# JGI-Bioinformatics/Kmernator

Hardware: AMD Instinct MI355X
Metric: total k-mers/sec at k=31, 150 bp reads (spectrum build, inputs resident in HBM) (higher is better)
Workload: dtype u64

## Files before the change

kmernator_amd/csrc/kmr_api.hip:

```cpp
#include <hip/hip_runtime.h>
#include <dlfcn.h>
#include <unistd.h>
#include <rccl/rccl.h>

#include <algorithm>
#include <atomic>
#include <cmath>
#include <cstdio>
#include <cstdlib>
#include <cstring>
#include <cctype>
#include <memory>
#include <mutex>
#include <string>
#include <type_traits>
#include <vector>

#include "kmr_host.hpp"
#include "kmr_runs.hpp"
#include "kmr_image_layout.hpp"
#include "kmr_kernels.hpp"
#include "kmr_partition.hpp"
#include "kmr_superkmer.hpp"
#include "kmr_buckets.hpp"
// ... 38 lines not shown

namespace {

template <int W, class F> auto with_win(uint32_t win, F &&f) {
	if (W > 1 && win == 32) return f(int_c<(W > 1 ? 32 : 16)>());
	return win == 16 ? f(int_c<16>()) : (win == 8 ? f(int_c<8>()) : f(int_c<4>()));
}

size_t slot_bytes(kmr_handle *h) { return with_w(h, [](auto W) { return sizeof(Slot<W()>); }); }

ReadsView reads_view(const void *bases, const void *quals, const void *offsets, uint64_t n_reads, const void *discarded = nullptr, uint64_t stream_base = 0, uint64_t first_read_idx = 0) {
	ReadsView rv{};
	rv.bases = (const uint8_t *)bases; rv.quals = (const uint8_t *)quals; rv.offsets = (const uint64_t *)offsets; rv.discarded = (const uint8_t *)discarded;
	rv.n_reads = n_reads; rv.stream_base = stream_base; rv.first_read_idx = first_read_idx;
	return rv;
}
ReadsView reads_slice(const ReadsView &all, uint64_t r, uint64_t m) {
	ReadsView rv = all;
	rv.offsets = all.offsets + r; rv.n_reads = m; rv.discarded = all.discarded ? all.discarded + r : nullptr; rv.first_read_idx = all.first_read_idx + r;
	return rv;
}
FinalizeParams finalize_params(kmr_handle *h, uint32_t min_depth) {
	FinalizeParams f{};
	f.kb = h->hkb; f.ext_min_q = h->cfg.ext_min_quality; f.min_depth = min_depth; f.has_singletons = h->cfg.separate_singletons ? 1 : 0; f.nb_weak = h->nb_weak; f.nb_sing = h->nb_sing;
	return f;
}

DevParams dev_params(kmr_handle *h) {
	DevParams p;
	p.k = h->k; p.kb = h->hkb; p.min_weight = h->cfg.min_weight; p.fastq_start = h->cfg.fastq_start_char; p.ext_min_q = h->cfg.ext_min_quality;
	p.qzero = h->cfg.fastq_start_char + std::max<uint32_t>(1u, h->cfg.min_quality_score);
	p.subsample = h->cfg.kmer_subsample; p.rank = h->cfg.rank; p.world = h->cfg.world_size; p.num_parts = h->cfg.num_parts; p.part_idx = h->cfg.part_idx;
	p.count_sender_bad = 0u;
	p.P = h->dP.get<double>(); p.stats = h->dstats.get<DevStats>(); p.err = h->derr.get<uint32_t>();
	p.sub_wstart = p.sub_wkeys = p.sub_sstart = p.sub_skeys = nullptr; p.sub_wvals = nullptr; p.sub_sweight = nullptr; p.sub_wnb = p.sub_snb = 0; p.sub_vw = 0;
	if (h->subtract) {
		const kmr_handle *o = h->subtract;
		if (o->weak.present && o->weak.n) { p.sub_wstart = o->weak.start.get<uint64_t>(); p.sub_wkeys = o->weak.keys.get<uint64_t>(); p.sub_wvals = o->weak.vals.get<uint32_t>(); p.sub_wnb = o->weak.nb; p.sub_vw = o->ext ? 15 : 3; }
		if (o->sing.present && o->sing.n) { p.sub_sstart = o->sing.start.get<uint64_t>(); p.sub_skeys = o->sing.keys.get<uint64_t>(); p.sub_sweight = o->sing.sweight.get<uint8_t>(); p.sub_snb = o->sing.nb; }
	}
	return p;
}


template <int W> Table<W> table_of(kmr_handle *h) { Table<W> t; t.slots = h->slots.get<Slot<W>>(); t.ext = h->extslots.get<ExtSlot>(); t.log2cap = h->log2cap; return t; }

template <int W> int clear_table(kmr_handle *h, void *slots, ExtSlot *ext, uint32_t log2cap) {
	hipLaunchKernelGGL(table_clear_kernel<W>, dim3(grid_for(1ull << log2cap)), dim3(256), 0, h->stream, (Slot<W> *)slots, ext, 1ull << log2cap);
	HIPCHK(h, hipGetLastError());
	return 0;
}
int clear_table_any(kmr_handle *h, void *slots, ExtSlot *ext, uint32_t log2cap) { return with_w(h, [&](auto W) { return clear_table<W()>(h, slots, ext, log2cap); }); }

int alloc_table(kmr_handle *h, uint32_t log2cap, DevBuf &slots, DevBuf &ext) {
	DevBuf s, x;
	HIPCHK(h, s.alloc(slot_bytes(h) << log2cap));
	if (h->ext) HIPCHK(h, x.alloc(sizeof(ExtSlot) << log2cap));
	const int rc = clear_table_any(h, s.get(), x.get<ExtSlot>(), log2cap);
	if (rc) return rc;
	slots = std::move(s); ext = std::move(x);
	return 0;
}

int sync_state(kmr_handle *h, bool with_pool_head = false) {
	h->l1_head_seen = 0;
	if (with_pool_head && h->l1.head) HIPCHK(h, hipMemcpyAsync(&h->l1_head_seen, h->l1.head.get<unsigned int>(), 4, hipMemcpyDeviceToHost, h->stream));
	HIPCHK(h, hipStreamSynchronize(h->stream));
	for (int which = 0; which < KMR_TIME_GROUPS; which++) {
		for (auto &pr : h->pending_events[which]) {
			float ms = 0; hipEventElapsedTime(&ms, pr.first, pr.second);
			h->ms[which] += ms; h->launches[which]++;
			hipEventDestroy(pr.first); hipEventDestroy(pr.second);
		}
		h->pending_events[which].clear();
	}
	uint32_t e = 0; DevStats s;
	HIPCHK(h, hipMemcpy(&e, h->derr.get<uint32_t>(), sizeof(e), hipMemcpyDeviceToHost));
	HIPCHK(h, hipMemcpy(&s, h->dstats.get<DevStats>(), sizeof(s), hipMemcpyDeviceToHost));
#ifdef KMR_DEBUG_HOOKS
	if (h->superkmer_mode) { if (dbg()) fprintf(stderr, "sk_extract windows: %llu general, %llu fast\n", s.claimed, s.inserted); s.claimed = 0; s.inserted = 0; }
#endif
	h->stats.raw_kmers = s.raw + s.inserted + s.sender_bad; h->stats.raw_good_kmers = s.good + s.inserted; h->stats.discarded = s.raw - s.good + s.sender_bad;
	h->occupied = s.claimed; h->pending_kmers = 0; h->subtracted = s.subtracted;
	if (e & ERR_READ_TOO_LONG) return fail(h, KMR_ERR_UNSUPPORTED, "a read is longer than the per-wavefront LDS tile (" + std::to_string(TILE_SPAN) + " bases)");
	if (e & ERR_TABLE_FULL) return fail(h, KMR_ERR_CAPACITY, "device k-mer table is full; raise kmr_config.max_table_entries / estimated_raw_kmers");
	if (e & ERR_SEGMENT_OVERFLOW) return fail(h, KMR_ERR_CAPACITY, "an owner segment overflowed seg_capacity");
	if (e & ERR_POOL_FULL) return fail(h, KMR_ERR_CAPACITY, "record pool overflow (internal sizing error)");
	if (e & ERR_ENTRIES_FULL) return fail(h, KMR_ERR_CAPACITY, "entry buffer overflow (internal sizing error)");
	return 0;
}

template <int W, bool EXT> int grow_table_t(kmr_handle *h, uint32_t newlog) {
	DevBuf ns, ne;
	int rc = alloc_table(h, newlog, ns, ne);
	if (rc) return rc;
	Table<W> src = table_of<W>(h), dst; dst.slots = ns.get<Slot<W>>(); dst.ext = ne.get<ExtSlot>(); dst.log2cap = newlog;
	hipLaunchKernelGGL((rehash_kernel<W, EXT>), dim3(grid_for(1ull << h->log2cap)), dim3(256), 0, h->stream, src, dst, h->hkb, h->derr.get<uint32_t>());
	HIPCHK(h, hipGetLastError());
	HIPCHK(h, hipStreamSynchronize(h->stream));
	h->slots = std::move(ns); h->extslots = std::move(ne); h->log2cap = newlog;
	return 0;
}
int grow_table(kmr_handle *h, uint32_t newlog) { return with_w_ext(h, [&](auto W, auto EXT) { return grow_table_t<W(), EXT()>(h, newlog); }); }

int ensure_capacity(kmr_handle *h, uint64_t incoming) {
	const uint64_t cap = 1ull << h->log2cap;
	if ((double)(h->occupied + h->pending_kmers + incoming) <= 0.85 * (double)cap) { h->pending_kmers += incoming; return 0; }
	int rc = sync_state(h);
	if (rc) return rc;
	if ((double)(h->occupied + incoming) > 0.85 * (double)cap) {
		uint32_t nl = h->log2cap;
		while ((double)(h->occupied + incoming) > 0.6 * (double)(1ull << nl)) nl++;
		rc = grow_table(h, nl);
		if (rc) return rc;
	}
	h->pending_kmers = incoming;
	return 0;
}

const size_t EXTRACT_SMEM = (size_t)WAVES_PER_BLOCK * 2 * TILE_BUF;

int prepare_units(kmr_handle *h, ReadsView &rv, uint32_t span = (uint32_t)TILE_SPAN, const unsigned int *longest = nullptr) {
	rv.u_start = rv.u_end = rv.u_read = nullptr; rv.n_units = 0;
	const uint64_t n = rv.n_reads;
	if (n == 0) return 0;
	int rc = 0;
	unsigned int mx = 0;
	if (longest) mx = *longest;
	else {
		rc = h->umax.reserve(h, "umax", 4); if (rc) return rc;
		HIPCHK(h, hipMemsetAsync(h->umax.get<unsigned int>(), 0, 4, h->stream));
		hipLaunchKernelGGL(unit_max_kernel, dim3(grid_for(n)), dim3(256), 0, h->stream, rv.offsets, n, h->umax.get<unsigned int>());
		HIPCHK(h, hipGetLastError());
		HIPCHK(h, hipMemcpyAsync(&mx, h->umax.get<unsigned int>(), 4, hipMemcpyDeviceToHost, h->stream));
		HIPCHK(h, hipStreamSynchronize(h->stream));
	}
	if (mx <= span) return 0;
	h->unit_batches++;
	rc = h->ucnt.reserve(h, "ucnt", 4 * (n + 1)); if (rc) return rc;
	hipLaunchKernelGGL(unit_count_kernel, dim3(grid_for(n)), dim3(256), 0, h->stream, rv.offsets, n, h->k, span, h->ucnt.get<uint32_t>());
	HIPCHK(h, hipGetLastError());
	rc = h->ufirst.reserve(h, "ufirst", 8 * (n + 1)); if (rc) return rc;
	rc = exclusive_scan_queue(h, h->ucnt.get<uint32_t>(), n, h->ufirst.get<uint64_t>()); if (rc) return rc;
	uint64_t U = 0;
	HIPCHK(h, hipMemcpyAsync(&U, h->ufirst.get<uint64_t>() + n, 8, hipMemcpyDeviceToHost, h->stream));
	HIPCHK(h, hipStreamSynchronize(h->stream));
	if (h->u_read.cap() < 8 * U) {
		h->u_start.reset(); h->u_end.reset(); h->u_read.reset();
		HIPCHK(h, h->u_start.alloc(8 * U)); HIPCHK(h, h->u_end.alloc(8 * U)); HIPCHK(h, h->u_read.alloc(8 * U));
	}
	hipLaunchKernelGGL(unit_fill_kernel, dim3(grid_for(n)), dim3(256), 0, h->stream, rv.offsets, n, h->k, span, h->ufirst.get<uint64_t>(), h->u_start.get<uint64_t>(), h->u_end.get<uint64_t>(), h->u_read.get<uint64_t>());
	HIPCHK(h, hipGetLastError());
	rv.u_start = h->u_start.get<uint64_t>(); rv.u_end = h->u_end.get<uint64_t>(); rv.u_read = h->u_read.get<uint64_t>(); rv.n_units = U;
	return 0;
}

template <int W, bool EXT, class Op> int launch_extract(kmr_handle *h, const ReadsView &rv, const DevParams &dp, const Op &op, uint64_t max_blocks = 0) {
	const bool sub = Op::NEEDS_WEIGHT && (dp.sub_wnb | dp.sub_snb) != 0;
	auto kern = sub ? extract_kernel<W, EXT, Op, true> : extract_kernel<W, EXT, Op, false>;
	HIPCHK(h, hipFuncSetAttribute((const void *)kern, hipFuncAttributeMaxDynamicSharedMemorySize, (int)EXTRACT_SMEM));
	if (dbg()) { int nb = 0; hipOccupancyMaxActiveBlocksPerMultiprocessor(&nb, (const void *)kern, WAVES_PER_BLOCK * 64, EXTRACT_SMEM); fprintf(stderr, "extract: %d blocks of %d waves per CU (dynamic LDS %zu)\n", nb, WAVES_PER_BLOCK, EXTRACT_SMEM);
		for (size_t tr : {(size_t)79872, (size_t)65536, (size_t)52000, (size_t)38000}) { hipOccupancyMaxActiveBlocksPerMultiprocessor(&nb, (const void *)kern, WAVES_PER_BLOCK * 64, tr); fprintf(stderr, "   with %zu bytes: %d blocks\n", tr, nb); } }
	const uint64_t tiles = ((rv.u_start ? rv.n_units : rv.n_reads) + 63) / 64;
	uint64_t blocks = (tiles + WAVES_PER_BLOCK - 1) / WAVES_PER_BLOCK;
	if (blocks == 0) return 0;
	if (max_blocks && blocks > max_blocks) blocks = max_blocks;
// ... 1047 lines not shown
		uint32_t sh = 0; while ((1u << sh) < h->cfg.world_size) sh++;
		if (bits >= 6 + sh) { h->sk_fine_shift = sh; bits -= sh; }
	}
	h->sk_bits = bits;
	if (h->cfg.world_size <= 1 && !h->sk_exchange && h->tune.target_list == 2048 && !h->tune.pow2_lists) {
		const uint64_t aim = h->tune.list_aim ? h->tune.list_aim : (W == 1 ? (h->ext ? 800 : (lean ? 1450 : 1700)) : per_list * 19 / 20);
		const uint64_t nlists = (est / aim + 63) & ~63ull;
		if (nlists > 64 && (nlists < (1ull << bits) || h->tune.list_aim) && nlists < (1ull << 31)) h->sk_bits = (uint32_t)nlists;
	}
	const uint64_t nl0 = sk_list_count(h->sk_bits);
	HIPCHK(h, h->sk_state.alloc(8 * nl0));
	hipLaunchKernelGGL(sk_state_init_kernel, dim3(grid_for(nl0)), dim3(256), 0, h->stream, h->sk_state.get<unsigned long long>(), nl0);
	HIPCHK(h, hipGetLastError());
	return 0;
}
void sk_presize_pool(kmr_handle *h, uint64_t call_bases, uint64_t total_bases, uint64_t avg, bool lean) {
	if (h->l1.base || h->cfg.world_size > 1 || h->sk_exchange || !(h->cfg.estimated_raw_kmers || call_bases > total_bases)) return;
	const double job_bases = h->cfg.estimated_raw_kmers ? (double)h->cfg.estimated_raw_kmers * (double)avg / (double)(avg > h->k ? avg - h->k + 1 : 1) : (double)call_bases;
	const double rest = job_bases - (double)total_bases;
	size_t fr = 0, tot = 0;
	if (rest > 0 && hipMemGetInfo(&fr, &tot) == hipSuccess) {
		const uint64_t want = (uint64_t)(rest * (h->ext ? 2.0 : 1.0) * (lean ? 0.3 : 0.65) / SK_CHUNK_G);
		h->l1.presize = std::min<uint64_t>(want, (uint64_t)(fr / 4) / ((size_t)CH * rec_bytes(h)));
	}
}
uint64_t sk_launch_chunks(kmr_handle *h, uint64_t bases) { return (h->ext ? 2 : 1) * bases / SK_CHUNK_G + ((h->l1.base && !h->sk_exchange) ? 0 : sk_list_count(h->sk_bits)) + (uint64_t)num_cus(h) * SK_EXTRACT_WAVES_PER_CU * 130 + 64; }
template <int W> int sk_launch_extraction(kmr_handle *h, const ReadsView &rv, const SkParams &sp, const DevParams &dp, bool filt, bool lean, float wK, const SkPacked *packed, uint64_t r) {
	if (packed) {
		SkPacked pkd = *packed; pkd.off += r; if (pkd.mk_off) pkd.mk_off += r;
		return with_win<W>(h->sk_win, [&](auto WIN) { return launch_sk_extract_lean<W, WIN(), true>(h, rv, sp, dp, wK, pkd); });
	}
	return with_win<W>(h->sk_win, [&](auto WIN) {
		if (h->ext) return filt ? launch_sk_extract<W, WIN(), true, true>(h, rv, sp, dp) : launch_sk_extract<W, WIN(), false, true>(h, rv, sp, dp);
		if (filt) return launch_sk_extract<W, WIN(), true>(h, rv, sp, dp);
		return lean ? launch_sk_extract_lean<W, WIN()>(h, rv, sp, dp, wK) : launch_sk_extract<W, WIN(), false>(h, rv, sp, dp);
	});
}
template <int W> int sk_track_call(kmr_handle *h, const ReadsView &rvAll, const DevParams &dp) {
	const uint64_t n = rvAll.n_reads;
	std::vector<SkTrackRec> recs(n);
	HIPCHK(h, hipMemcpyAsync(recs.data(), h->trk.get<SkTrackRec>(), n * sizeof(SkTrackRec), hipMemcpyDeviceToHost, h->stream));
	HIPCHK(h, hipStreamSynchronize(h->stream));
	std::vector<SkBoundary> bd; std::vector<uint64_t> good_before;
	const bool walkable = (dp.sub_wnb | dp.sub_snb) == 0;
	for (uint64_t r = 0; r < n; r++) {
		while ((uint64_t)h->trk_next <= h->trk_raw + recs[r].raw) {
			SkBoundary b; b.read = r; b.t = (uint32_t)((uint64_t)h->trk_next - h->trk_raw); b.good = 0; b.ordinal = 0;
			if (!walkable) { b.t = recs[r].raw; b.good = recs[r].good; b.ordinal = recs[r].end_ordinal; }
			bd.push_back(b); good_before.push_back(h->trk_good);
			h->trk_snap_raw.push_back(walkable ? (uint64_t)h->trk_next : h->trk_raw + recs[r].raw);
			h->trk_next = (long)((double)h->trk_next * 1.05);
			if (!walkable) break;
		}
		if (!walkable) while ((uint64_t)h->trk_next <= h->trk_raw + recs[r].raw) h->trk_next = (long)((double)h->trk_next * 1.05);
		h->trk_raw += recs[r].raw; h->trk_good += recs[r].good;
	}
	if (h->trk_bounds.size() + bd.size() > SK_TRACK_MAX) return fail(h, KMR_ERR_UNSUPPORTED, "size tracker: more than 512 elements");
	if (!bd.empty() && walkable) {
		DevBuf dbdb; HIPCHK(h, dbdb.alloc(bd.size() * sizeof(SkBoundary)));
		SkBoundary *dbd = dbdb.get<SkBoundary>();
		auto chk = [&](hipError_t e) { return e == hipSuccess ? 0 : fail(h, KMR_ERR_HIP, std::string("size tracker boundaries: ") + hipGetErrorString(e)); };
		int rc = chk(hipMemcpyAsync(dbd, bd.data(), bd.size() * sizeof(SkBoundary), hipMemcpyHostToDevice, h->stream)); if (rc) return rc;
		ReadsView rv = rvAll; rv.u_start = rv.u_end = rv.u_read = nullptr; rv.n_units = 0;
		hipLaunchKernelGGL(sk_track_boundary_kernel<W>, dim3((unsigned)((bd.size() + 63) / 64)), dim3(64), 0, h->stream, rv, dp, dbd, (uint32_t)bd.size());
		rc = chk(hipGetLastError()); if (rc) return rc;
		rc = chk(hipMemcpyAsync(bd.data(), dbd, bd.size() * sizeof(SkBoundary), hipMemcpyDeviceToHost, h->stream)); if (rc) return rc;
		rc = chk(hipStreamSynchronize(h->stream)); if (rc) return rc;
	}
	for (size_t i = 0; i < bd.size(); i++) { h->trk_bounds.push_back(bd[i].ordinal); h->trk_snap_good.push_back(good_before[i] + bd[i].good); }
	return 0;
}
template <int W> int add_reads_superkmer_t(kmr_handle *h, const ReadsView &rvAll, uint64_t total_bases, const FeedHints &hints) {
	const uint64_t n = rvAll.n_reads;
	const DevParams dp = dev_params(h);
	const bool filt = sk_build_filters(h, dp), tracking = h->cfg.size_tracker && n;
	bool lean = false; float wK = 1.0f; int rc = 0;
	const uint64_t avg = n ? std::max<uint64_t>(1, total_bases / n) : 1;
	const uint64_t sub_bases = h->tune.sub_batch_bases ? h->tune.sub_batch_bases : (1ull << 31);
	const uint64_t chunk = std::max<uint64_t>(64, (sub_bases / avg) & ~63ull);
	unsigned int longest = 0; bool have_longest = false;
	if (!filt && !h->ext && !sp_debug_extract(h)) { rc = sk_uniform_weight(h, rvAll, hints, lean, wK, n <= chunk ? &longest : nullptr, &have_longest); if (rc) return rc; }
	if (hints.packed && (!lean || h->cfg.size_tracker)) return fail(h, KMR_ERR_STATE, "internal: a packed batch handed to an extraction that wants text");
	if (n) sk_note_call_weight(h, lean, wK);
	if (!h->sk_state) { rc = sk_size_lists<W>(h, std::max<uint64_t>(total_bases, hints.call_bases), lean); if (rc) return rc; }
	if (tracking) { h->trk_n = 0; rc = h->trk.reserve(h, "trk", n * sizeof(SkTrackRec)); if (rc) return rc; HIPCHK(h, hipMemsetAsync(h->trk.get<SkTrackRec>(), 0, n * sizeof(SkTrackRec), h->stream)); }
	for (uint64_t r = 0; r < n; r += chunk) {
		const uint64_t m = std::min(chunk, n - r);
		ReadsView rv = reads_slice(rvAll, r, m);
		rc = prepare_units(h, rv, hints.packed ? SK_PACKED_SPAN : (uint32_t)TILE_SPAN, have_longest ? &longest : nullptr); if (rc) return rc;
		if (r == 0) sk_presize_pool(h, hints.call_bases, total_bases, avg, lean);
		rc = pool_reserve(h, h->l1, sk_launch_chunks(h, m * avg + avg), true); if (rc) return rc;
		TimeSpan tb(h, KMR_TIME_BUILD), te(h, KMR_TIME_EXTRACT);
		SkParams sp = sk_params(h);
		if (h->cfg.size_tracker) sp.track = h->trk.get<SkTrackRec>() + r;
		rc = sk_launch_extraction<W>(h, rv, sp, dp, filt, lean, wK, hints.packed, r);
		te.end(); tb.end();
		if (rc) return rc;
	}
	return tracking ? sk_track_call<W>(h, rvAll, dp) : 0;
}
int add_reads_superkmer(kmr_handle *h, const ReadsView &rv, uint64_t total_bases, const FeedHints &hints) { return with_w(h, [&](auto W) { return add_reads_superkmer_t<W()>(h, rv, total_bases, hints); }); }
static const uint64_t SAT_BATCH_BYTES = 1ull << 30;
static const uint64_t SAT_BATCH_KEYS = (1ull << 23) - 1;
static const uint64_t SAT_PAIR_BYTES = 24;
template <int W> int saturated_fix_t(kmr_handle *h, const uint64_t *ls, const uint64_t *lc, uint64_t nl, unsigned long long n_clamped, unsigned long long n_sightings, uint32_t has_singletons) {
	DevMap &wm = h->weak;
	h->last_saturated_keys = 0; h->last_saturated_batches = 0;
	if (!n_clamped || !wm.n) return 0;
	uint32_t list_bits = 0; while ((1ull << list_bits) < nl) list_bits++;
	if ((1ull << list_bits) != nl) list_bits = (uint32_t)nl;
	auto no_mem = [&](const char *what, size_t bytes) { return fail(h, KMR_ERR_OOM, std::string("saturated-key pass (weights of k-mers seen 256 times or more): no device memory for ") + what + " (" + std::to_string(bytes) + " bytes)"); };
	auto dalloc = [](DevBuf &b, size_t bytes) { return b.alloc(std::max<size_t>(bytes, 256)); };
	DevBuf bfound, bentry, blist;
	if (dalloc(bfound, 8) != hipSuccess) return no_mem("a counter", 8);
	unsigned long long *dfound = bfound.get<unsigned long long>(); uint64_t *d_entry = nullptr; uint32_t *d_list = nullptr;
	uint64_t cap = std::min<uint64_t>(wm.n, 4 * n_clamped + 1024);
	unsigned long long found = 0;
	for (;;) {
		if (dalloc(bentry, 8 * cap) != hipSuccess || dalloc(blist, 4 * cap) != hipSuccess) return no_mem("the key list", 12 * cap);
		d_entry = bentry.get<uint64_t>(); d_list = blist.get<uint32_t>();
		HIPCHK(h, hipMemsetAsync(dfound, 0, 8, h->stream));
		hipLaunchKernelGGL(sat_find_kernel<W>, dim3(grid_for(wm.n)), dim3(256), 0, h->stream, (const uint64_t *)wm.keys.get<uint64_t>(), (const uint32_t *)wm.vals.get<uint32_t>(), wm.n, h->sk_m, h->sk_off, h->sk_win, list_bits, dfound, cap, d_entry, d_list, h->ext ? 15u : 3u);
		HIPCHK(h, hipGetLastError());
		HIPCHK(h, hipMemcpyAsync(&found, dfound, 8, hipMemcpyDeviceToHost, h->stream)); HIPCHK(h, hipStreamSynchronize(h->stream));
		if (found <= cap) break;
		cap = found;
	}
	if (!found) return 0;
	std::vector<uint64_t> entry(found); std::vector<uint32_t> lst(found);
	HIPCHK(h, hipMemcpy(entry.data(), d_entry, 8 * found, hipMemcpyDeviceToHost)); HIPCHK(h, hipMemcpy(lst.data(), d_list, 4 * found, hipMemcpyDeviceToHost));
	std::vector<uint64_t> order(found);
	for (uint64_t i = 0; i < found; i++) order[i] = i;
	std::sort(order.begin(), order.end(), [&](uint64_t a, uint64_t b) { return lst[a] != lst[b] ? lst[a] < lst[b] : entry[a] < entry[b]; });
	std::vector<uint64_t> sentry(found); std::vector<uint32_t> dl; std::vector<uint64_t> le0, le1;
	for (uint64_t i = 0; i < found; i++) {
		sentry[i] = entry[order[i]];
		const uint32_t l = lst[order[i]];
		if (dl.empty() || dl.back() != l) { dl.push_back(l); le0.push_back(i); le1.push_back(i + 1); } else le1.back() = i + 1;
	}
	std::vector<uint64_t>().swap(entry); std::vector<uint32_t>().swap(lst); std::vector<uint64_t>().swap(order);
	HIPCHK(h, hipMemcpy(d_entry, sentry.data(), 8 * found, hipMemcpyHostToDevice));
	HIPCHK(h, hipMemcpy(d_list, dl.data(), 4 * dl.size(), hipMemcpyHostToDevice));
	std::vector<uint64_t> c0(dl.size()), c1(dl.size());
	{
		DevBuf bc0, bc1;
		if (dalloc(bc0, 8 * dl.size()) != hipSuccess || dalloc(bc1, 8 * dl.size()) != hipSuccess) return no_mem("the chunk ranges", 16 * dl.size());
		hipLaunchKernelGGL(sat_gather_kernel, dim3(grid_for(dl.size())), dim3(256), 0, h->stream, ls, (const uint32_t *)d_list, (uint64_t)dl.size(), bc0.get<uint64_t>(), bc1.get<uint64_t>());
		HIPCHK(h, hipGetLastError());
		HIPCHK(h, hipMemcpy(c0.data(), bc0.get<uint64_t>(), 8 * dl.size(), hipMemcpyDeviceToHost)); HIPCHK(h, hipMemcpy(c1.data(), bc1.get<uint64_t>(), 8 * dl.size(), hipMemcpyDeviceToHost));
	}
	blist = DevBuf();
	struct Seg { uint32_t li; uint64_t e0, e1, est; };
	std::vector<Seg> segs;
	uint64_t all_chunks = 0;
	for (size_t i = 0; i < dl.size(); i++) all_chunks += c1[i] - c0[i];
	const double per_chunk = all_chunks ? (double)n_sightings / (double)all_chunks : 0.0;
	for (size_t i = 0; i < dl.size(); i++)
		for (uint64_t a = le0[i]; a < le1[i]; a += SAT_BATCH_KEYS) {
			const uint64_t b = std::min<uint64_t>(le1[i], a + SAT_BATCH_KEYS);
			const double share = (double)(b - a) / (double)(le1[i] - le0[i]);
			segs.push_back(Seg{(uint32_t)i, a, b, (uint64_t)(per_chunk * (double)(c1[i] - c0[i]) * share) + 1});
		}
	const uint64_t budget = h->tune.saturated_batch_bytes ? h->tune.saturated_batch_bytes : SAT_BATCH_BYTES;
	uint64_t batches = 0;
	for (size_t s0 = 0; s0 < segs.size(); ) {
		size_t s1 = s0 + 1; uint64_t est = segs[s0].est;
		while (s1 < segs.size() && segs[s1].e1 - segs[s0].e0 <= SAT_BATCH_KEYS && (est + segs[s1].est) * SAT_PAIR_BYTES <= budget) est += segs[s1++].est;
		const uint64_t k0 = segs[s0].e0, nk = segs[s1 - 1].e1 - k0;
		std::vector<uint64_t> items;
		for (size_t g = s0; g < s1; g++)
			for (uint64_t a = c0[segs[g].li]; a < c1[segs[g].li]; a += 256) { items.push_back(a); items.push_back(std::min(c1[segs[g].li], a + 256)); items.push_back(segs[g].e0 - k0); items.push_back(segs[g].e1 - k0); }
		const size_t ni = items.size() / 4;
		std::vector<uint64_t> soa(4 * ni);
		for (size_t i = 0; i < ni; i++) for (int q = 0; q < 4; q++) soa[q * ni + i] = items[4 * i + q];
		uint64_t pcap = est + est / 4 + 1024;
		for (int attempt = 0; ni; attempt++) {
			DevBuf bitems, bk_in, bk_out, bv_in, bv_out, btmp;
			if (dalloc(bitems, 32 * ni) != hipSuccess) return no_mem("its work items", 32 * ni);
			uint64_t *d_items = bitems.get<uint64_t>();
			HIPCHK(h, hipMemcpy(d_items, soa.data(), 32 * ni, hipMemcpyHostToDevice));
			if (dalloc(bk_in, 8 * pcap) != hipSuccess || dalloc(bk_out, 8 * pcap) != hipSuccess || dalloc(bv_in, 4 * pcap) != hipSuccess || dalloc(bv_out, 4 * pcap) != hipSuccess)
				return no_mem("the sightings of one batch", SAT_PAIR_BYTES * pcap);
			unsigned long long *pk_in = bk_in.get<unsigned long long>(), *pk_out = bk_out.get<unsigned long long>(); uint32_t *pv_in = bv_in.get<uint32_t>(), *pv_out = bv_out.get<uint32_t>();
			HIPCHK(h, hipMemsetAsync(dfound, 0, 8, h->stream));
			int rc = zero_work_counter(h); if (rc) return rc;
			hipLaunchKernelGGL(sat_collect_kernel<W>, dim3((unsigned)std::min<uint64_t>(ni, (uint64_t)num_cus(h) * 4)), dim3(256), 0, h->stream, pool_view(h, h->l1), lc, h->k, (const uint64_t *)wm.keys.get<uint64_t>(), (const uint64_t *)(d_entry + k0),
			                   (const uint64_t *)d_items, (const uint64_t *)(d_items + ni), (const uint64_t *)(d_items + 2 * ni), (const uint64_t *)(d_items + 3 * ni), (uint64_t)ni, dfound, pcap, pk_in, pv_in, h->work_counter.get<unsigned int>());
			HIPCHK(h, hipGetLastError());
			unsigned long long n_pairs = 0;
			HIPCHK(h, hipMemcpyAsync(&n_pairs, dfound, 8, hipMemcpyDeviceToHost, h->stream)); HIPCHK(h, hipStreamSynchronize(h->stream));
			if (n_pairs > pcap) {
				if (attempt) return fail(h, KMR_ERR_CAPACITY, "saturated-key pass: sightings of a batch changed between two passes (internal error)");
				pcap = n_pairs;
				continue;
			}
			size_t tmp_bytes = 0;
			if (kmr::sort_pairs_u64_u32(nullptr, &tmp_bytes, pk_in, pk_out, pv_in, pv_out, n_pairs, h->stream) != 0) return fail(h, KMR_ERR_HIP, "saturated-key pass: radix sort (size query)");
			if (dalloc(btmp, tmp_bytes) != hipSuccess) return no_mem("the sort's temporary storage", tmp_bytes);
			if (kmr::sort_pairs_u64_u32(btmp.get(), &tmp_bytes, pk_in, pk_out, pv_in, pv_out, n_pairs, h->stream) != 0) return fail(h, KMR_ERR_HIP, "saturated-key pass: radix sort");
			hipLaunchKernelGGL(sat_reduce_kernel, dim3((unsigned)std::min<uint64_t>(nk, 4096)), dim3(256), 0, h->stream, (const unsigned long long *)pk_out, (const uint32_t *)pv_out, (uint64_t)n_pairs, (const uint64_t *)(d_entry + k0), (uint64_t)nk, has_singletons, wm.vals.get<uint32_t>(), h->ext ? 15u : 3u);
			HIPCHK(h, hipGetLastError());
			HIPCHK(h, hipStreamSynchronize(h->stream));
			break;
		}
		batches++;
		s0 = s1;
	}
	h->last_saturated_keys = found; h->last_saturated_batches = batches;
	return 0;
}


template <int W> int sk_count_uniform(kmr_handle *h, bool tracking, bool &uni, uint32_t &uni_wbits) {
	uni = false; uni_wbits = 0;
	if (tracking || h->ext || h->sk_uni_mixed || h->tune.no_uniform_count) return 0;
	if (W > 1 && (h->k & 31u) == 0) return 0;
	uint32_t w = h->sk_uni_w; bool mixed = false;
	if (h->peer_uni_mixed) mixed = true;
	else if (h->peer_uni_w != SK_UNI_NONE) { if (w == SK_UNI_NONE) w = h->peer_uni_w; else if (w != h->peer_uni_w) mixed = true; }
	if (h->d_uni) {
		uint32_t dv[2] = {SK_UNI_NONE, 0u};
		HIPCHK(h, hipMemcpy(dv, h->d_uni.get<uint32_t>(), 8, hipMemcpyDeviceToHost));
		if (dv[1]) mixed = true;
		else if (dv[0] != SK_UNI_NONE) { if (w == SK_UNI_NONE) w = dv[0]; else if (w != dv[0]) mixed = true; }
	}
	if (!mixed && w != SK_UNI_NONE) { uni = true; uni_wbits = w; }
	return 0;
}
template <int W> SkLong<W> sk_own_lists(kmr_handle *h, bool refined) {
	SkLong<W> lg{};
	lg.list_first = 0; lg.list_stride = 1;
	if (h->sk_exchange && h->cfg.world_size > 1 && !refined) { lg.list_first = h->cfg.rank; lg.list_stride = h->cfg.world_size; }
	return lg;
}
template <int W> struct SkCountLaunch {
	void (*kern)(const uint4 *, const uint64_t *, const uint64_t *, uint64_t, uint32_t, SkCountHot, unsigned int *, uint32_t, const SkCountArgs<W> *);
	size_t smem;
	int blocks;
};
static const int SK_COUNT_BLOCKS_DEFAULT = 5;
template <int W> int sk_count_blocks(kmr_handle *h, bool ext, bool tracking, bool uni, bool item) {
	if (W != 1 || ext || tracking || !uni || item) return 4;
	return h->tune.count_blocks ? h->tune.count_blocks : SK_COUNT_BLOCKS_DEFAULT;
}
template <int W, int LOG2S, bool TRACK, bool EXT, bool UNI, bool ITEM, int BLOCKS = 0> SkCountLaunch<W> sk_count_form() { return {sk_count_kernel<W, LOG2S, TRACK, EXT, UNI, ITEM, BLOCKS>, sk_count_smem_bytes<W, LOG2S, TRACK, EXT, UNI>(), BLOCKS ? BLOCKS : 4}; }
template <int W, bool ITEM> SkCountLaunch<W> sk_count_forms(bool ext, bool tracking, bool uni, int blocks) {
	if constexpr (!ITEM) { if (tracking && !ext) return sk_count_form<W, COUNT_LOG2S, true, false, false, false>(); }
	if constexpr (W == 1 && !ITEM) { if (blocks == 5) return sk_count_form<1, COUNT_LOG2S, false, false, true, false, 5>(); }
	return ext ? sk_count_form<W, COUNT_LOG2S_EXT, false, true, false, ITEM>() :
	    (uni ? sk_count_form<W, COUNT_LOG2S, false, false, true, ITEM>() : sk_count_form<W, COUNT_LOG2S, false, false, false, ITEM>());
}
template <int W> int sk_count_select(kmr_handle *h, bool ext, bool tracking, bool uni, bool item, const CountOut &out, const SkLong<W> &lg, SkCountLaunch<W> &k) {
	if (item && tracking) return fail(h, KMR_ERR_STATE, "internal: the size tracker's count pass has no long-list items");
	if (item != (lg.item_c0 != nullptr) || (item && (!lg.item_c1 || !lg.merge.slots || !lg.merge_used))) return fail(h, KMR_ERR_STATE, "internal: count pass and its work items disagree");
	if (ext ? (!out.wkeys || !out.wvals || !out.weakCount) : !out.wentries) return fail(h, KMR_ERR_STATE, "internal: count pass and its entry buffers disagree");
	const int blocks = sk_count_blocks<W>(h, ext, tracking, uni, item);
	k = item ? sk_count_forms<W, true>(ext, tracking, uni, blocks) : sk_count_forms<W, false>(ext, tracking, uni, blocks);
	if (k.blocks != blocks) return fail(h, KMR_ERR_STATE, "internal: count pass and its blocks per CU disagree");
	if (!item) h->last_count_blocks = k.blocks;
	const auto kern = k.kern; const size_t smem = k.smem;
	HIPCHK(h, hipFuncSetAttribute((const void *)kern, hipFuncAttributeMaxDynamicSharedMemorySize, (int)smem));
	return 0;
}
template <int W> int sk_count_launch(kmr_handle *h, const SkCountLaunch<W> &k, int grid, const uint64_t *ls, const uint64_t *lc, uint64_t nl, const CountOut &out, const FinalizeParams &f, const SkTrackView &tv, const SkLong<W> &lg) {
	SkCountArgs<W> a{out, f, tv, lg};
	SkCountArgs<W> *d = nullptr;
	int rc = arena_get(h, &d, 1); if (rc) return rc;
	hipLaunchKernelGGL(sk_count_args_kernel<W>, dim3(1), dim3(64), 0, h->stream, a, d);
	hipLaunchKernelGGL(k.kern, dim3(grid), dim3(SKC_THREADS), k.smem, h->stream, (const uint4 *)pool_view(h, h->l1).base, ls, lc, nl, h->k, sk_count_hot<W>(a), h->work_counter.get<unsigned int>(), sk_dbg_flags("KMR_SK_COUNT_DBG"), (const SkCountArgs<W> *)d);
	return 0;
}

template <int W> struct SkFinalize : CountPass {
	bool tracking = false, refined = false, uni = false;
	uint64_t nl = 1; uint64_t *ls = nullptr, *lc = nullptr; uint32_t nch = 0;
	SkTrackView tv{};
	SkLong<W> lgMain{}, lgItems{}; uint64_t n_items = 0;
	uint64_t early_slots = 0; FinalizeCounters early_c{};
};

int sk_refine_lists(kmr_handle *h, uint64_t &nl) {
	const uint32_t fine_bits = h->sk_bits + h->sk_fine_shift;
	const uint64_t nlf = 1ull << fine_bits;
	unsigned int head = 0;
	HIPCHK(h, hipStreamSynchronize(h->stream));
	HIPCHK(h, hipMemcpy(&head, h->l1.head.get<unsigned int>(), 4, hipMemcpyDeviceToHost));
	if (head > h->l1.cap) head = h->l1.cap;
	int rc = h->sk_fine_state.reserve(h, "sk_fine_state", 8 * nlf); if (rc) return rc;
	hipLaunchKernelGGL(sk_state_init_kernel, dim3(grid_for(nlf)), dim3(256), 0, h->stream, h->sk_fine_state.get<unsigned long long>(), nlf);
	const int rgrid = (int)std::min<uint64_t>(((uint64_t)head + SK_REFINE_WAVES - 1) / SK_REFINE_WAVES + 1, (uint64_t)num_cus(h) * 8);
	rc = pool_reserve(h, h->l1, (uint64_t)head * 2 + nlf / h->cfg.world_size + (uint64_t)rgrid * SK_REFINE_WAVES * 130 + 64, true); if (rc) return rc;
	if (head) hipLaunchKernelGGL(sk_refine_kernel, dim3(rgrid), dim3(SK_REFINE_WAVES * 64), 0, h->stream, pool_view(h, h->l1), head, fine_bits, h->sk_fine_state.get<unsigned long long>());
	hipLaunchKernelGGL(sk_close_kernel, dim3(grid_for(nlf)), dim3(256), 0, h->stream, h->sk_fine_state.get<unsigned long long>(), nlf, h->l1.chunk_count.get<uint32_t>(), h->l1.cap);
	HIPCHK(h, hipGetLastError());
	nl = nlf;
	return 0;
}
int sk_track_view(kmr_handle *h, SkTrackView &tv) {
	const std::vector<unsigned long long> &bounds = h->trk_bounds;
	if (bounds.size() > SK_TRACK_MAX) return fail(h, KMR_ERR_UNSUPPORTED, "size tracker: more than 512 elements");
	unsigned long long *db = nullptr; unsigned int *dd = nullptr;
	int rc = arena_get(h, &db, bounds.size() + 1); if (rc) return rc;
	rc = arena_get(h, &dd, 2 * (bounds.size() + 1)); if (rc) return rc;
	if (!bounds.empty()) HIPCHK(h, hipMemcpyAsync(db, bounds.data(), 8 * bounds.size(), hipMemcpyHostToDevice, h->stream));
	tv.bounds = db; tv.n = (uint32_t)bounds.size(); tv.d_unique = dd; tv.d_single = dd + bounds.size() + 1;
	return 0;
}
int sk_track_elements(kmr_handle *h, const SkTrackView &tv, uint32_t has_singletons) {
	std::vector<unsigned int> dd(2 * (tv.n + 1), 0);
	HIPCHK(h, hipMemcpy(dd.data(), tv.d_unique, 8 * (tv.n + 1), hipMemcpyDeviceToHost));
	h->trk_elems.clear();
	uint64_t uniq = 0; int64_t single = 0;
	const uint64_t sub = h->cfg.kmer_subsample > 1 ? h->cfg.kmer_subsample : 1;
	for (uint32_t i = 0; i < tv.n; i++) {
		uniq += dd[i]; single += (int32_t)dd[tv.n + 1 + i];
		h->trk_elems.push_back(h->trk_snap_raw[i] * sub); h->trk_elems.push_back(h->trk_snap_good[i] * sub);
		h->trk_elems.push_back(uniq * sub); h->trk_elems.push_back(has_singletons ? (uint64_t)single * sub : 0);
	}
	return 0;
}
template <int W> int sk_early_takeover(kmr_handle *h, SkFinalize<W> &p, uint32_t min_depth, bool &device_error) {
	device_error = false;
	FinalizeCounters &early_c = p.early_c;
	h->last_early_hi = 0; h->last_early_entries = 0; h->last_early_overflowed = false;
	if (!h->early.active) return 0;
	uint32_t eerr = 0;
	HIPCHK(h, hipMemcpy(&eerr, h->early.err.get<uint32_t>(), 4, hipMemcpyDeviceToHost));
	unsigned long long ecur = 0;
	HIPCHK(h, hipMemcpy(&ecur, h->early.cursor.get<unsigned long long>(), 8, hipMemcpyDeviceToHost)); HIPCHK(h, hipMemcpy(&early_c, h->early.fc.get(), sizeof(early_c), hipMemcpyDeviceToHost));
	if (eerr & ~(uint32_t)ERR_ENTRIES_FULL) {
		uint32_t e = 0; HIPCHK(h, hipMemcpy(&e, h->derr.get<uint32_t>(), 4, hipMemcpyDeviceToHost)); e |= eerr & ~(uint32_t)ERR_ENTRIES_FULL;
		HIPCHK(h, hipMemcpy(h->derr.get<uint32_t>(), &e, 4, hipMemcpyHostToDevice)); h->early.active = false;
		device_error = true;
		return 0;
	}
	const bool overflowed = (eerr & ERR_ENTRIES_FULL) || ecur > packed_entries(h, h->early.ue);
	const bool ok = !overflowed && h->early.min_depth == min_depth && !p.tracking && !p.ext && !p.keepSing && !p.refined;
	h->last_early_overflowed = overflowed;
	if (ok) {
		p.early_slots = ecur;
		h->last_early_hi = h->early.hi; h->last_early_entries = early_c.weak_kept;
		const uint64_t stride0 = p.lgMain.list_stride, first0 = p.lgMain.list_first;
		uint64_t first = h->early.hi;
		if (stride0 > 1) first += (first0 + stride0 - first % stride0) % stride0;
		p.lgMain.list_first = first;
	} else { h->early.active = false; memset(&early_c, 0, sizeof(early_c)); }
	return 0;
}
template <int W> int sk_long_items(kmr_handle *h, SkFinalize<W> &p) {
	p.lgItems = p.lgMain; p.n_items = 0;
	const uint64_t LONG_CHUNKS = p.ext ? std::min<uint64_t>(h->tune.long_list_chunks ? h->tune.long_list_chunks : SK_EXT_LONG_CHUNKS, SK_EXT_LONG_CHUNKS) : (h->tune.long_list_chunks ? h->tune.long_list_chunks : 1024), PIECE = std::max<uint64_t>(1, LONG_CHUNKS / 2);
	if (p.tracking || p.nch <= LONG_CHUNKS) return 0;
	const uint64_t cap = (uint64_t)p.nch / PIECE + 2 * 1024 + 16;
	uint64_t *ic0 = nullptr, *ic1 = nullptr; unsigned long long *dn = nullptr;
	int rc = arena_get(h, &ic0, cap); if (rc) return rc; rc = arena_get(h, &ic1, cap); if (rc) return rc; rc = arena_get(h, &dn, 1); if (rc) return rc;
	HIPCHK(h, hipMemsetAsync(dn, 0, 8, h->stream));
	hipLaunchKernelGGL(sk_long_items_kernel, dim3(grid_for(p.nl)), dim3(256), 0, h->stream, p.ls, p.nl, LONG_CHUNKS, PIECE, ic0, ic1, cap, dn);
	HIPCHK(h, hipGetLastError());
	unsigned long long hn = 0;
	HIPCHK(h, hipMemcpyAsync(&hn, dn, 8, hipMemcpyDeviceToHost, h->stream)); HIPCHK(h, hipStreamSynchronize(h->stream));
	if (hn > cap) return fail(h, KMR_ERR_CAPACITY, "long-list work items (internal sizing error)");
	p.n_items = hn;
	if (p.n_items) {
		p.lgMain.long_threshold = LONG_CHUNKS;
		p.lgItems.item_c0 = ic0; p.lgItems.item_c1 = ic1; p.lgItems.n_items = p.n_items; p.lgItems.merge_used = dn;
	}
	return 0;
}
CountOut count_out(kmr_handle *h, bool packed, unsigned long long *cursors, uint32_t *wc, uint32_t *sc, FinalizeCounters *fc) {
	CountOut out{};
	if (packed) { out.wentries = h->ue.get<uint64_t>(); out.wcap = packed_entries(h, h->ue); }
	else { out.wkeys = h->uw_keys.get<uint64_t>(); out.wvals = h->uw_vals.get<uint32_t>(); out.wcap = key_entries(h, h->uw_keys); out.spkt = h->us_pkt.get<uint32_t>(); out.weakCount = wc; }
	out.wcursor = cursors; out.scursor = cursors + 1;
	out.skeys = h->us_keys.get<uint64_t>(); out.sweight = h->us_b8.get<uint8_t>(); out.scap = key_entries(h, h->us_keys);
	out.singCount = sc; out.fc = fc; out.err = h->derr.get<uint32_t>();
	return out;
}
template <int W> int sk_count_pass(kmr_handle *h, SkFinalize<W> &p) {
	const uint64_t nl = p.nl, n_items = p.n_items; const SkTrackView &tv = p.tv;
	uint32_t merge_log2 = 16;
	DevBuf mslots, mext;
	return count_attempts(h, p, [&]() -> int { mslots.reset(); mext.reset(); return 0; }, [&](const CountOut &out, bool repeated, uint32_t &repeat_on) -> int {
		if (repeated) merge_log2 += 3;
		int rc = 0;
		SkCountLaunch<W> k;
		rc = sk_count_select<W>(h, p.ext, p.tracking, p.uni, false, out, p.lgMain, k); if (rc) return rc;
		const int grid = (int)std::min<uint64_t>((uint64_t)num_cus(h) * k.blocks, (nl / p.lgMain.list_stride + SK_LBATCH) / SK_LBATCH);
		if (p.tracking) HIPCHK(h, hipMemsetAsync(tv.d_unique, 0, 8 * (tv.n + 1), h->stream));
		if (dbg()) { int nb = 0; hipOccupancyMaxActiveBlocksPerMultiprocessor(&nb, (const void *)k.kern, SKC_THREADS, k.smem); fprintf(stderr, "sk_count<W=%d>: %d blocks per CU (LDS %zu), %llu lists, %u chunks\n", W, nb, k.smem, (unsigned long long)nl, p.nch); }
		rc = sk_count_launch<W>(h, k, grid, p.ls, p.lc, nl, out, p.f, tv, p.lgMain); if (rc) return rc;
		HIPCHK(h, hipGetLastError());
		if (!n_items) return 0;
		SkLong<W> &lgItems = p.lgItems;
		if (mslots.alloc(sizeof(Slot<W>) << merge_log2) != hipSuccess) return fail(h, KMR_ERR_OOM, "merge table of the long lists");
		if (p.ext && mext.alloc(sizeof(ExtSlot) << merge_log2) != hipSuccess) return fail(h, KMR_ERR_OOM, "merge table of the long lists");
		hipLaunchKernelGGL(table_clear_kernel<W>, dim3(grid_for(1ull << merge_log2)), dim3(256), 0, h->stream, mslots.get<Slot<W>>(), mext.get<ExtSlot>(), 1ull << merge_log2);
		lgItems.merge.slots = mslots.get<Slot<W>>(); lgItems.merge.ext = mext.get<ExtSlot>(); lgItems.merge.log2cap = merge_log2;
		HIPCHK(h, hipMemsetAsync(lgItems.merge_used, 0, 8, h->stream));
		rc = zero_work_counter(h); if (rc) return rc;
		rc = sk_count_select<W>(h, p.ext, p.tracking, p.uni, true, out, lgItems, k); if (rc) return rc;
		const int grid2 = (int)std::min<uint64_t>((uint64_t)num_cus(h) * k.blocks, n_items);
		rc = sk_count_launch<W>(h, k, grid2, p.ls, p.lc, nl, out, p.f, tv, lgItems); if (rc) return rc;
		hipLaunchKernelGGL(sk_merge_emit_kernel<W>, dim3(grid_for(1ull << merge_log2)), dim3(256), 0, h->stream, lgItems.merge, out, p.f);
		if (hipGetLastError() != hipSuccess) return fail(h, KMR_ERR_HIP, "long-list launches");
		if (merge_log2 < 30) repeat_on = ERR_TABLE_FULL;
		return 0;
	});
}
template <int W> int sk_append_early(kmr_handle *h, SkFinalize<W> &p) {
	FinalizeCounters &c = p.c; const FinalizeCounters &early_c = p.early_c; unsigned long long *cur = p.cur; const uint64_t early_slots = p.early_slots;
	const size_t eb = 8ull * (W + 1);
	if (cur[0] + early_slots > packed_entries(h, h->ue)) {
		DevBuf bigger;
		HIPCHK(h, bigger.alloc(eb * (cur[0] + early_slots + 4096)));
		HIPCHK(h, hipMemcpyAsync(bigger.get(), h->ue.get(), eb * cur[0], hipMemcpyDeviceToDevice, h->stream)); HIPCHK(h, hipStreamSynchronize(h->stream));
		h->ue = std::move(bigger);
	}
	HIPCHK(h, hipMemcpyAsync((uint8_t *)h->ue.get<uint64_t>() + eb * cur[0], h->early.ue.get<uint64_t>(), eb * early_slots, hipMemcpyDeviceToDevice, h->stream));
	cur[0] += early_slots;
	c.unique += early_c.unique; c.singletons += early_c.singletons; c.weak_kept += early_c.weak_kept; c.sing_kept += early_c.sing_kept;
	c.saturated += early_c.saturated; c.sat_sightings += early_c.sat_sightings;
	h->stats.unique_kmers = c.unique; h->stats.singleton_kmers = p.f.has_singletons ? c.singletons : 0;
	return 0;
}

template <int W> int finalize_superkmer_t(kmr_handle *h, uint32_t min_depth) {
	int rc = sync_state(h, true);
	if (rc) return rc;
	TimeSpan whole(h, KMR_TIME_FINALIZE);
	const uint64_t G = h->stats.raw_good_kmers;
	SkFinalize<W> p;
	p.f = finalize_params(h, min_depth);
	p.keepSing = p.f.has_singletons && min_depth <= 1;
	p.ext = h->ext; p.packed = !p.ext;
	p.tracking = h->cfg.size_tracker != 0;
	if (!h->l1.head) { rc = pool_reserve(h, h->l1, 0, false); if (rc) return rc; }
	rc = arena_reset(h); if (rc) return rc;
	p.nl = h->sk_state ? sk_list_count(h->sk_bits) : 1;
	if (h->sk_state) {
		hipLaunchKernelGGL(sk_close_kernel, dim3(grid_for(p.nl)), dim3(256), 0, h->stream, h->sk_state.get<unsigned long long>(), p.nl, h->l1.chunk_count.get<uint32_t>(), h->l1.cap);
		HIPCHK(h, hipGetLastError());
	}
	p.refined = h->sk_state && h->sk_fine_shift > 0;
	if (p.refined) { rc = sk_refine_lists(h, p.nl); if (rc) return rc; }
	rc = build_csr(h, h->l1, p.nl, 0, &p.ls, &p.lc, &p.nch, p.refined ? nullptr : &h->l1_head_seen); if (rc) return rc;
	rc = sk_count_uniform<W>(h, p.tracking, p.uni, p.f.uni_wbits); if (rc) return rc;
	h->last_count_uniform = p.uni;
	rc = count_entry_buffers(h, p, G, sk_entry_slack(h, sk_count_blocks<W>(h, p.ext, p.tracking, p.uni, false)), G / (p.f.has_singletons ? 8 : 3), G / 3, h->sk_exchange && h->cfg.world_size > 1); if (rc) return rc;
	if (p.tracking) { rc = sk_track_view(h, p.tv); if (rc) return rc; }
	p.lgMain = sk_own_lists<W>(h, p.refined);
	bool device_error = false;
	rc = sk_early_takeover<W>(h, p, min_depth, device_error); if (rc) return rc;
	if (device_error) { whole.end(); return sync_state(h); }
	rc = sk_long_items<W>(h, p); if (rc) return rc;
	uint32_t *overflow = nullptr;
	auto count_and_bucket = [&](bool fixed_bins) -> int {
		int rc2 = sk_count_pass<W>(h, p); if (rc2) return rc2;
		h->stats.unique_kmers = p.c.unique; h->stats.singleton_kmers = p.f.has_singletons ? p.c.singletons : 0;
		if (p.tracking && !h->last_bb_fallback) { rc2 = sk_track_elements(h, p.tv, p.f.has_singletons); if (rc2) return rc2; }
		if (p.early_slots) { rc2 = sk_append_early<W>(h, p); if (rc2) return rc2; }
		h->early.active = false;
		TimeSpan t(h, KMR_TIME_BUCKETS);
		return finish_maps_from_entries(h, p.wc, p.sc, p.cur[0], p.cur[1], p.c.weak_kept, p.c.sing_kept, p.keepSing, overflow, p.packed, fixed_bins);
	};
	h->last_bb_fallback = false;
	rc = count_and_bucket(h->tune.bb_fixed_bins); if (rc) return rc;
	if (overflow) {
		uint32_t ovf = 0;
		HIPCHK(h, hipMemcpyAsync(&ovf, overflow, 4, hipMemcpyDeviceToHost, h->stream)); HIPCHK(h, hipStreamSynchronize(h->stream));
		if (ovf) {
			if (dbg()) fprintf(stderr, "bucket build: a bin of the radix partition overflowed its capacity, again with measured bins\n");
			h->last_bb_fallback = true;
			rc = count_and_bucket(false); if (rc) return rc;
		}
	}
	h->last_saturated_keys = 0; h->last_saturated_batches = 0;
	if (p.c.saturated) { rc = saturated_fix_t<W>(h, p.ls, p.lc, p.nl, p.c.saturated, p.c.sat_sightings, p.f.has_singletons); if (rc) return rc; }
	whole.end();
	return publish_maps(h, p.keepSing);
}
template <int W> int count_prefix_superkmer_t(kmr_handle *h, uint32_t min_depth, uint64_t hi) {
	int rc = sync_state(h, true); if (rc) return rc;
	FinalizeParams f = finalize_params(h, min_depth);
	const bool keepSing = f.has_singletons && min_depth <= 1;
	h->early.active = false;
	if (h->ext || h->cfg.size_tracker || keepSing || (h->sk_state && h->sk_fine_shift > 0) || !h->sk_state) return KMR_OK;
	const uint64_t nl = sk_list_count(h->sk_bits);
	if (hi > nl) hi = nl;
	if (hi == 0) return KMR_OK;
	rc = arena_reset(h); if (rc) return rc;
	hipLaunchKernelGGL(sk_close_kernel, dim3(grid_for(nl)), dim3(256), 0, h->stream, h->sk_state.get<unsigned long long>(), nl, h->l1.chunk_count.get<uint32_t>(), h->l1.cap);
	HIPCHK(h, hipGetLastError());
	uint64_t *ls = nullptr, *lc = nullptr; uint32_t nch = 0;
	rc = build_csr(h, h->l1, nl, 0, &ls, &lc, &nch, &h->l1_head_seen); if (rc) return rc;
	const uint64_t G = h->stats.raw_good_kmers;
	bool uni = false;
	if (!h->peer_uni_mixed) { rc = sk_count_uniform<W>(h, false, uni, f.uni_wbits); if (rc) return rc; }
	uint64_t want = (uint64_t)((double)G * ((double)hi / (double)nl) / (f.has_singletons ? 6.0 : 2.5)) + sk_entry_slack(h, sk_count_blocks<W>(h, false, false, uni, false));
	if (h->tune.early_entry_share >= 0) { want = (uint64_t)((double)G * h->tune.early_entry_share) + 16384; h->early.ue.reset(); }
	rc = h->early.ue.reserve(h, "early count ue", 8ull * (W + 1) * want); if (rc) return rc;
	rc = h->early.cursor.reserve(h, "early count cursor", 16); if (rc) return rc;
	rc = h->early.fc.reserve(h, "early count fc", sizeof(FinalizeCounters)); if (rc) return rc;
	rc = h->early.err.reserve(h, "early count error word", 4); if (rc) return rc;
	HIPCHK(h, hipMemsetAsync(h->early.cursor.get<unsigned long long>(), 0, 16, h->stream)); HIPCHK(h, hipMemsetAsync(h->early.fc.get(), 0, sizeof(FinalizeCounters), h->stream));
	HIPCHK(h, hipMemsetAsync(h->early.err.get<uint32_t>(), 0, 4, h->stream));
	const SkTrackView tv{};
	SkLong<W> lg = sk_own_lists<W>(h, false);
	lg.long_threshold = h->tune.long_list_chunks ? h->tune.long_list_chunks : 1024;
	uint32_t *sc = nullptr;
	rc = arena_get(h, &sc, h->nb_sing); if (rc) return rc;
	HIPCHK(h, hipMemsetAsync(sc, 0, 4 * h->nb_sing, h->stream));
	CountOut out{};
	out.wentries = h->early.ue.get<uint64_t>(); out.wcursor = h->early.cursor.get<unsigned long long>(); out.wcap = packed_entries(h, h->early.ue);
	out.scursor = h->early.cursor.get<unsigned long long>() + 1;
	out.singCount = sc; out.fc = (FinalizeCounters *)h->early.fc.get(); out.err = h->early.err.get<uint32_t>();
	rc = zero_work_counter(h); if (rc) return rc;
	const uint64_t n_work = hi > lg.list_first ? (hi - lg.list_first + lg.list_stride - 1) / lg.list_stride : 0;
	if (n_work) {
		SkCountLaunch<W> k;
		rc = sk_count_select<W>(h, false, false, uni, false, out, lg, k); if (rc) return rc;
		const int grid = (int)std::min<uint64_t>((uint64_t)num_cus(h) * k.blocks, (n_work + SK_LBATCH) / SK_LBATCH);
		TimeSpan t(h, KMR_TIME_COUNT);
		rc = sk_count_launch<W>(h, k, grid, ls, lc, hi, out, f, tv, lg);
		t.end();
		if (rc) return rc;
		HIPCHK(h, hipGetLastError());
	}
	h->early.active = true; h->early.hi = hi; h->early.min_depth = min_depth;
	return KMR_OK;
}
int count_prefix_superkmer(kmr_handle *h, uint32_t min_depth, uint64_t hi) { return with_w(h, [&](auto W) { return count_prefix_superkmer_t<W()>(h, min_depth, hi); }); }
int finalize_superkmer(kmr_handle *h, uint32_t min_depth) { return with_w(h, [&](auto W) { return finalize_superkmer_t<W()>(h, min_depth); }); }

template <class M> void release(kmr_handle *h) { static_cast<M &>(*h) = M(); }

void free_partition_state(kmr_handle *h) {
	release<BuildMem>(h);
	if (h->tb_copy_stream) { hipStreamDestroy(h->tb_copy_stream); h->tb_copy_stream = nullptr; for (int a = 0; a < 2; a++) { hipEventDestroy(h->tb_ready[a]); hipEventDestroy(h->tb_consumed[a]); h->tb_set_used[a] = false; } }
}

}

extern "C" {

uint32_t kmr_abi_version(void) { return KMR_ABI_VERSION; }

int kmr_config_init(kmr_config *c) {
	if (!c) return KMR_ERR_INVALID_ARG;
	memset(c, 0, sizeof(*c));
	c->struct_size = sizeof(*c);
	c->value_kind = KMR_VALUE_COUNT_DIR; c->min_weight = 0.10f; c->min_quality_score = 3; c->fastq_start_char = 33;
	c->ext_min_quality = 20; c->separate_singletons = 1; c->kmer_subsample = 1; c->device = -1; c->rank = 0; c->world_size = 1;
	c->estimated_depth = 20.0; c->estimated_error_rate = 0.35; c->kmers_per_bucket = 32; c->num_parts = 1; c->part_idx = 0;
	return KMR_OK;
}

const char *kmr_last_error(const kmr_handle *h) { return h ? h->err.c_str() : g_create_error.c_str(); }

int kmr_create(const kmr_config *cfg, kmr_handle **out) {
	if (!cfg || !out) return fail(nullptr, KMR_ERR_INVALID_ARG, "null argument");
	*out = nullptr;
	if (cfg->struct_size != sizeof(kmr_config)) return fail(nullptr, KMR_ERR_INVALID_ARG, "kmr_config.struct_size mismatch (ABI)");
	if (cfg->k < 1 || cfg->k > 128) return fail(nullptr, KMR_ERR_INVALID_ARG, "k must be in 1..128");
	if (cfg->world_size < 1 || cfg->rank >= cfg->world_size) return fail(nullptr, KMR_ERR_INVALID_ARG, "bad rank/world_size");
	if (cfg->value_kind > KMR_VALUE_EXT) return fail(nullptr, KMR_ERR_INVALID_ARG, "bad value_kind");
	if (cfg->hash_kind > KMR_HASH_LOOKUP8) return fail(nullptr, KMR_ERR_INVALID_ARG, "bad hash_kind");
	int ndev = 0;
	if (hipGetDeviceCount(&ndev) != hipSuccess || ndev == 0) return fail(nullptr, KMR_ERR_NO_DEVICE, "no HIP device: this library has no CPU path");
	kmr_handle *h = new kmr_handle();
	h->cfg = *cfg;
	if (h->cfg.kmer_subsample == 0) h->cfg.kmer_subsample = 1;
	if (h->cfg.num_parts == 0) h->cfg.num_parts = 1;
	h->k = cfg->k; h->kb = (cfg->k + 3) / 4; h->W = (h->kb + 7) / 8; h->ext = cfg->value_kind == KMR_VALUE_EXT;
	h->hkb = h->kb | (cfg->hash_kind << 16);
	memset(&h->stats, 0, sizeof(h->stats));
	int rc = 0;
	do {
		if (cfg->device >= 0) { if (hipSetDevice(cfg->device) != hipSuccess) { rc = fail(nullptr, KMR_ERR_NO_DEVICE, "hipSetDevice failed"); break; } }
		if (hipGetDevice(&h->device) != hipSuccess) { rc = fail(nullptr, KMR_ERR_NO_DEVICE, "hipGetDevice failed"); break; }
		if (hipStreamCreate(&h->stream) != hipSuccess) { rc = fail(nullptr, KMR_ERR_HIP, "hipStreamCreate failed"); break; }
		uint64_t w = cfg->num_buckets_weak, s = cfg->num_buckets_singleton;
		const double depth = cfg->estimated_depth > 0 ? cfg->estimated_depth : 20.0;
		const uint32_t kpb = cfg->kmers_per_bucket ? cfg->kmers_per_bucket : 32;
		const uint64_t raw = cfg->estimated_raw_kmers / (cfg->world_size > 1 ? cfg->world_size : 1);
		if (w == 0) { unsigned long est = (unsigned long)(int)(raw / depth); w = est / kpb + 1; }
		if (s == 0) { unsigned long est = cfg->separate_singletons ? (unsigned long)(raw * cfg->estimated_error_rate) : 1; s = est / kpb + 1; }
		h->nb_weak = resize_buckets(w); h->nb_sing = resize_buckets(s);
		h->has_singletons = cfg->separate_singletons != 0;
		uint64_t want = cfg->max_table_entries ? (uint64_t)(cfg->max_table_entries / 0.7) : (uint64_t)(cfg->estimated_raw_kmers * 0.45 / 0.6);
		if (cfg->world_size > 1 && !cfg->max_table_entries) want /= cfg->world_size;
		uint32_t lg = 16; while ((1ull << lg) < want && lg < 40) lg++;
		h->log2cap = lg;
		double P[256]; quality_table(P, cfg->min_quality_score, cfg->fastq_start_char);
		if (h->dP.alloc(sizeof(P)) != hipSuccess || h->dstats.alloc(sizeof(DevStats)) != hipSuccess || h->derr.alloc(4) != hipSuccess) { rc = fail(nullptr, KMR_ERR_OOM, "hipMalloc failed"); break; }
		hipMemcpy(h->dP.get<double>(), P, sizeof(P), hipMemcpyHostToDevice); hipMemset(h->dstats.get<DevStats>(), 0, sizeof(DevStats)); hipMemset(h->derr.get<uint32_t>(), 0, 4);
		if (cfg->build_mode > 3) { rc = fail(nullptr, KMR_ERR_INVALID_ARG, "bad build_mode"); break; }
		h->partition_mode = cfg->build_mode != 1;
		uint32_t wish_w = 0, wish_m = 0, wish_o = 0;
		const bool sk_auto = cfg->build_mode == 0 && cfg->world_size <= 1 && sk_geometry(h->k, 0, wish_w, wish_m, wish_o);
		h->auto_mode = cfg->build_mode == 0;
		const bool sk_ready = sk_geometry(h->k, 0, wish_w, wish_m, wish_o);
		if (cfg->build_mode == 3 || sk_auto || sk_ready) {
			if (!sk_geometry(h->k, 0, h->sk_win, h->sk_m, h->sk_off)) { rc = fail(nullptr, KMR_ERR_UNSUPPORTED, "build_mode 3 (super-k-mer lists) needs k >= 13"); break; }
			h->superkmer_mode = cfg->build_mode == 3 || sk_auto;
			double Pk[256];
			for (int cidx = 0; cidx < 256; cidx++) { double wv = 1.0; for (uint32_t jj = 0; jj < h->k; jj++) wv *= P[cidx]; Pk[cidx] = wv; }
			memcpy(h->hPk, Pk, sizeof(Pk)); memcpy(h->hP, P, sizeof(h->hP));
			if (h->dPk.alloc(2 * sizeof(Pk)) != hipSuccess) { rc = fail(nullptr, KMR_ERR_OOM, "hipMalloc failed"); break; }
			hipMemcpy(h->dPk.get<double>(), Pk, sizeof(Pk), hipMemcpyHostToDevice);
			double Rp[256]; bool fast = true;
			for (int cidx = 0; cidx < 256; cidx++) Rp[cidx] = P[cidx] != 0.0 ? 1.0 / P[cidx] : 0.0;
			for (int a = 0; a < 256 && fast; a++) for (int b = 0; b < 256; b++) {
				if (P[a] == 0.0 || P[b] == 0.0) continue;
				const double q0 = P[a] * Rp[b];
				if (std::fma(std::fma(-q0, P[b], P[a]), Rp[b], q0) != P[a] / P[b]) { fast = false; break; }
			}
			h->sk_fast_div = fast;
			hipMemcpy(h->dPk.get<double>() + 256, Rp, sizeof(Rp), hipMemcpyHostToDevice);
		}
		if (cfg->size_tracker && (!h->superkmer_mode || h->ext || cfg->world_size > 1)) { rc = fail(nullptr, KMR_ERR_UNSUPPORTED, "size_tracker: kept by the super-k-mer build (build_mode 0 / 3, direction-counting values, k >= 13) of a single partition"); break; }
		if (!h->partition_mode) {
			rc = alloc_table(h, h->log2cap, h->slots, h->extslots);
			if (rc) { g_create_error = h->err; break; }
		}
		if (hipStreamSynchronize(h->stream) != hipSuccess) { rc = fail(nullptr, KMR_ERR_HIP, std::string("table clear failed: ") + hipGetErrorString(hipGetLastError())); break; }
	} while (0);
	if (rc) { kmr_destroy(h); return rc; }
	*out = h;
	return KMR_OK;
}

static void exchange_destroy_comm(kmr_handle *h);
void kmr_destroy(kmr_handle *h) {
	if (!h) return;
	if (h->stream) hipStreamSynchronize(h->stream);
	for (int which = 0; which < KMR_TIME_GROUPS; which++) for (auto &pr : h->pending_events[which]) { hipEventDestroy(pr.first); hipEventDestroy(pr.second); }
	release<HandleMem>(h);
	free_partition_state(h);
	exchange_destroy_comm(h);
	release<ExchangeMem>(h);
	if (h->stream) hipStreamDestroy(h->stream);
	delete h;
}

int kmr_num_buckets(const kmr_handle *h, int which, uint64_t *out) {
	if (!h || !out) return KMR_ERR_INVALID_ARG;
	if (which == KMR_MAP_WEAK) *out = h->finalized && h->weak.present ? h->weak.nb : h->nb_weak;
	else if (which == KMR_MAP_SINGLETON) *out = h->finalized && h->sing.present ? h->sing.nb : h->nb_sing;
	else return KMR_ERR_UNSUPPORTED;
	return KMR_OK;
}

int kmr_reset(kmr_handle *h) {
	if (!h) return KMR_ERR_INVALID_ARG;
	hipSetDevice(h->device);
	HIPCHK(h, hipStreamSynchronize(h->stream));
	clear_map(h->weak); clear_map(h->sing);
	int rc = 0;
	if (h->partition_mode) {
		if (h->l1.head) HIPCHK(h, hipMemsetAsync(h->l1.head.get<unsigned int>(), 0, 4, h->stream));
		h->l1.used_ub = 0;
		h->inserted_records = 0;
		h->qual_mixed = false;
		h->sk_uni_w = SK_UNI_NONE; h->sk_uni_mixed = false; h->peer_uni_w = SK_UNI_NONE; h->peer_uni_mixed = false; h->peers_declare = false;
		h->xr_lo = 0; h->xr_hi = ~0ull; h->early.active = false;
		if (h->d_uni) { const uint32_t init[2] = {SK_UNI_NONE, 0u}; HIPCHK(h, hipMemcpyAsync(h->d_uni.get<uint32_t>(), init, 8, hipMemcpyHostToDevice, h->stream)); HIPCHK(h, hipStreamSynchronize(h->stream)); }
		if (h->sk_state) hipLaunchKernelGGL(sk_state_init_kernel, dim3(grid_for(sk_list_count(h->sk_bits))), dim3(256), 0, h->stream, h->sk_state.get<unsigned long long>(), sk_list_count(h->sk_bits));
		if (h->l1_state) {
			hipLaunchKernelGGL(partition_state_init_kernel, dim3(partition_blocks(h)), dim3(256), 0, h->stream, h->l1_state.get<uint8_t>(),
			                   h->l1_state.cap() / (size_t)partition_blocks(h), h->bits1, (uint32_t)partition_blocks(h));
			h->l1_state_dirty = false;
		}
	} else {
		if (!h->slots) rc = alloc_table(h, h->log2cap, h->slots, h->extslots);
		else rc = clear_table_any(h, h->slots.get(), h->extslots.get<ExtSlot>(), h->log2cap);
		if (rc) return rc;
	}
	HIPCHK(h, hipMemsetAsync(h->dstats.get<DevStats>(), 0, sizeof(DevStats), h->stream));
	HIPCHK(h, hipMemsetAsync(h->derr.get<uint32_t>(), 0, 4, h->stream));
	memset(&h->stats, 0, sizeof(h->stats));
	h->occupied = h->pending_kmers = 0; h->stream_base = 0; h->reads = 0; h->subtracted = 0; h->xc_job_bases = 0; h->xc_bytes_to_peers = 0;
	h->trk_n = 0; h->trk_elems.clear();
	h->trk_next = 128; h->trk_raw = h->trk_good = 0; h->trk_bounds.clear(); h->trk_snap_raw.clear(); h->trk_snap_good.clear();
	h->finalized = false; h->map_gen++; h->has_singletons = h->cfg.separate_singletons != 0;
	return KMR_OK;
}
int kmr_release_table(kmr_handle *h) {
	if (!h) return KMR_ERR_INVALID_ARG;
	if (!h->finalized) return fail(h, KMR_ERR_STATE, "kmr_release_table before kmr_finalize");
	hipSetDevice(h->device);
	h->slots.reset(); h->extslots.reset();
	if (h->partition_mode) free_partition_state(h);
	return KMR_OK;
}

void *kmr_stream(kmr_handle *h) { return h ? (void *)h->stream : nullptr; }

int kmr_set_stream_origin(kmr_handle *h, uint64_t ordinal) {
	if (!h) return KMR_ERR_INVALID_ARG;
	if (h->finalized) return fail(h, KMR_ERR_STATE, "kmr_set_stream_origin after kmr_finalize");
	if (ordinal > MAX_STREAM_ORDINAL) return fail(h, KMR_ERR_CAPACITY, "stream ordinals have 40 bits");
	h->stream_base = ordinal;
	return KMR_OK;
}

int kmr_tune(kmr_handle *h, const char *knob, double value) {
	if (!h || !knob) return KMR_ERR_INVALID_ARG;
	const std::string k(knob);
	if (k == "target_list_records") h->tune.target_list = value >= 1 ? (uint64_t)value : 2048;
	else if (k == "sub_batch_bases") h->tune.sub_batch_bases = value >= 1 ? (uint64_t)value : 0;
	else if (k == "recycle_chunks") h->tune.recycle = value < 0 ? -1 : (value != 0 ? 1 : 0);
	else if (k == "partition_blocks") h->tune.part_blocks = value >= 1 ? (int)value : 0;
	else if (k == "entry_share") h->tune.entry_share = value;
	else if (k == "early_entry_share") h->tune.early_entry_share = value;
	else if (k == "saturated_batch_bytes") h->tune.saturated_batch_bytes = value >= 1 ? (uint64_t)value : 0;
	else if (k == "lookup_table") h->tune.no_lut = value == 0;
	else if (k == "stream_lookups") h->tune.no_stream_lookups = value == 0;
	else if (k == "long_list_chunks") h->tune.long_list_chunks = value < 2 ? 2 : (uint64_t)value;
	else if (k == "lean_extract") h->tune.no_lean_extract = value == 0;
	else if (k == "uniform_count") h->tune.no_uniform_count = value == 0;
	else if (k == "count_blocks") { if (value != 0 && value != 4 && value != 5) return fail(h, KMR_ERR_INVALID_ARG, "count_blocks is 0 (default), 4 or 5"); h->tune.count_blocks = (int)value; }
	else if (k == "packed_direct") h->tune.no_packed_direct = value == 0;
	else if (k == "pow2_lists") h->tune.pow2_lists = value != 0;
	else if (k == "list_aim") h->tune.list_aim = value >= 1 ? (uint64_t)value : 0;
	else if (k == "twobit_piece_bases") h->tune.twobit_piece_bases = (uint64_t)value;
	else if (k == "exchange_fail_once") h->tune.exchange_fail_once = value != 0;
	else if (k == "binned_buckets_min") h->tune.binned_min = value >= 0 ? (uint64_t)value : ~0ull;
	else if (k == "bb_fixed_bins") h->tune.bb_fixed_bins = value != 0;
	else if (k == "bb_slack_bins") h->tune.bb_slack_bins = value;
	else if (k == "bb_slack_groups") h->tune.bb_slack_groups = value;
	else if (k == "bb_reload") h->tune.bb_reload = value != 0;
	else if (k == "coarse_lists") h->tune.no_coarse_lists = value == 0;
	else if (k == "select_timing") h->tune.select_timing = value != 0;
	else if (k == "dump_timing") h->tune.dump_timing = value != 0;
	else if (k == "pairs_timing") h->tune.pairs_timing = value != 0;
	else if (k == "dedup_timing") h->tune.dedup_timing = value != 0;
	else if (k == "bimodal_window") h->tune.bimodal_window = value >= 0 && value <= BM_CAP ? (int)value : -1;
	else if (k == "partition_units") h->tune.partition_units = value >= 1 && value <= 8192 ? (uint32_t)value : 0;
	else if (k == "artifact_report_lds") h->tune.artifact_report_lds = value == 0 ? 0 : value == 1 ? 1 : -1;
	else if (k == "pair_hash_bits") h->tune.pair_hash_bits = value >= 1 && value < 64 ? (uint32_t)value : 64;
	else if (k == "dump_piece_bytes") h->tune.dump_piece_bytes = value >= 1 ? (uint64_t)value : 0;
	else if (k == "dump_tiles_per_block") h->tune.dump_tiles_per_block = value >= 1 ? (uint64_t)std::min(value, 4294967296.0) : 0;
	else if (k == "narrow_tallies") h->tune.no_narrow = value == 0;
	else if (k == "keep_level1_state") h->tune.no_l1_state = value == 0;
	else if (k == "csr_partition") h->tune.csr_partition = value != 0;
	else if (k == "compare_lds_kmers") h->tune.compare_lds_kmers = value >= 0 && value <= CMP_CAP_MOST ? (int)value : -1;
	else if (k == "compare_stage_kmers") h->tune.compare_stage_kmers = value >= 1 ? std::min<uint64_t>((uint64_t)value, 1ull << 31) : 0;
	else if (k == "tnf_piece_bases") h->tune.tnf_piece_bases = value >= 1 ? (uint32_t)std::min<double>(value, 1u << 30) : 0;
	else if (k == "match_hit_capacity") h->tune.match_hit_capacity = value >= 1 ? (uint64_t)std::min<double>(value, 4294967294.0) : 0;
	else if (k == "extend_stage_kmers") h->tune.extend_stage_kmers = value >= 1 ? std::min<uint64_t>((uint64_t)value, 1ull << 31) : 0;
	else if (k == "extend_timing") h->tune.extend_timing = value != 0;
	else if (k == "superkmer_window") {
		if (h->superkmer_mode && !h->sk_state) { uint32_t w, m, o; if (!sk_geometry(h->k, 0, w, m, o, (uint32_t)value)) return fail(h, KMR_ERR_INVALID_ARG, "no minimizer geometry under that window"); h->sk_win = w; h->sk_m = m; h->sk_off = o; }
	}
	else if (k == "superkmer_minimizer") {
		if (h->superkmer_mode && !h->sk_state) { uint32_t w, m, o; if (!sk_geometry(h->k, (uint32_t)value, w, m, o)) return fail(h, KMR_ERR_INVALID_ARG, "no minimizer geometry for that length"); h->sk_win = w; h->sk_m = m; h->sk_off = o; }
	}
	else return fail(h, KMR_ERR_INVALID_ARG, "unknown tuning knob '" + k + "'");
	return KMR_OK;
}

int kmr_build_info(kmr_handle *h, const char *what, double *value) {
	if (!h || !what || !value) return KMR_ERR_INVALID_ARG;
	const std::string k(what);
	if (k == "lists") *value = h->sk_state ? (double)sk_list_count(h->sk_bits) : 0.0;
	else if (k == "uniform_count") *value = h->last_count_uniform ? 1.0 : 0.0;
	else if (k == "count_blocks") *value = (double)h->last_count_blocks;
	else if (k == "chunk_pool_chunks") *value = (double)h->l1.cap;
	else if (k == "superkmer_window") *value = (double)h->sk_win;
	else if (k == "early_lists") *value = (double)h->last_early_hi;
	else if (k == "early_entries") *value = (double)h->last_early_entries;
	else if (k == "early_overflowed") *value = h->last_early_overflowed ? 1.0 : 0.0;
	else if (k == "bb_path") *value = (double)h->last_bb_path;
	else if (k == "bb_fallback") *value = h->last_bb_fallback ? 1.0 : 0.0;
	else if (k == "score_path") *value = (double)h->last_score_path;
	else if (k == "saturated_keys") *value = (double)h->last_saturated_keys;
	else if (k == "saturated_batches") *value = (double)h->last_saturated_batches;
	else if (k == "count_attempts") *value = (double)h->last_count_attempts;
	else if (k == "csr_path") *value = (double)h->last_csr_path;
	else if (k == "csr_chunks") *value = (double)h->last_csr_chunks;
	else if (k == "unit_batches") *value = (double)h->unit_batches;
	else if (k == "match_add_attempts") *value = (double)h->last_match_attempts;
	else if (k == "extend_runs") *value = (double)h->last_extend_runs;
	else if (k == "extend_gather_ms") *value = h->last_extend_ms[0];
	else if (k == "extend_extract_ms") *value = h->last_extend_ms[1];
	else if (k == "extend_sort_ms") *value = h->last_extend_ms[2];
	else if (k == "extend_reduce_ms") *value = h->last_extend_ms[3];
	else if (k == "extend_walk_ms") *value = h->last_extend_ms[4];
	else if (k == "device_blocks_live") *value = (double)g_blocks_live.load();
	else if (k == "filter_score_ms") *value = h->last_score_ms;
	else if (k == "select_ms") *value = h->last_select_ms;
	else if (k == "select_write_ms") *value = h->last_write_ms;
	else if (k == "artifact_report_lds") *value = h->last_artifact_report_lds;
	else if (k == "pairs_ms") *value = h->last_pairs_ms;
	else if (k == "pairs_parse_ms") *value = h->last_pairs_parse_ms;
	else if (k == "pairs_sort_ms") *value = h->last_pairs_sort_ms;
	else if (k == "pair_hash_collisions") *value = (double)h->last_pair_hash_collisions;
	else if (k == "dedup_ms") *value = h->last_dedup_ms;
	else if (k == "dedup_key_ms") *value = h->last_dedup_key_ms;
	else if (k == "dedup_sort_ms") *value = h->last_dedup_sort_ms;
	else if (k == "dedup_consensus_ms") *value = h->last_dedup_consensus_ms;
	else if (k == "dump_size_ms") *value = h->last_dump_size_ms;
	else if (k == "dump_write_ms") *value = h->last_dump_write_ms;
	else if (k == "dump_tiles_per_block") *value = (double)h->last_dump_tiles_per_block;
// ... 843 lines not shown
	return add_reads_superkmer(h, reads_view(nullptr, nullptr, nullptr, 0), 0, FeedHints());
}
int kmr_sk_exchange_counts(kmr_handle *h, uint64_t *chunks, uint64_t *granules) {
	if (!h || !chunks || !granules) return KMR_ERR_INVALID_ARG;
	int rc = sk_exchange_ready(h, "kmr_sk_exchange_counts"); if (rc) return rc;
	hipSetDevice(h->device);
	rc = sk_ensure_state(h); if (rc) return rc;
	rc = sync_state(h); if (rc) return rc;
	const uint32_t world = h->cfg.world_size;
	const uint64_t nl = sk_list_count(h->sk_bits);
	unsigned int head = 0;
	HIPCHK(h, hipMemcpy(&head, h->l1.head.get<unsigned int>(), 4, hipMemcpyDeviceToHost));
	if (head > h->l1.cap) head = h->l1.cap;
	DevBuf db; HIPCHK(h, db.alloc(16 * SK_OWNER_MAX));
	unsigned long long *d = db.get<unsigned long long>();
	HIPCHK(h, hipMemsetAsync(d, 0, 16 * SK_OWNER_MAX, h->stream));
	hipLaunchKernelGGL(sk_close_kernel, dim3(grid_for(nl)), dim3(256), 0, h->stream, h->sk_state.get<unsigned long long>(), nl, h->l1.chunk_count.get<uint32_t>(), h->l1.cap);
	if (head) hipLaunchKernelGGL(sk_owner_count_kernel, dim3(grid_for(head)), dim3(256), 0, h->stream, h->l1.chunk_list.get<uint32_t>(), h->l1.chunk_count.get<uint32_t>(), head, world, d, d + SK_OWNER_MAX, h->xr_lo, h->xr_hi);
	hipError_t e = hipGetLastError();
	std::vector<unsigned long long> hv(2 * SK_OWNER_MAX, 0);
	if (e == hipSuccess) e = hipMemcpyAsync(hv.data(), d, 16 * SK_OWNER_MAX, hipMemcpyDeviceToHost, h->stream);
	if (e == hipSuccess) e = hipStreamSynchronize(h->stream);
	HIPCHK(h, e);
	for (uint32_t r = 0; r < world; r++) { chunks[r] = hv[r]; granules[r] = hv[SK_OWNER_MAX + r]; }
	return KMR_OK;
}
int kmr_sk_exchange_pack_dev(kmr_handle *h, void *dev_data, void *dev_meta, const uint64_t *granule_offset, const uint64_t *chunk_offset) {
	if (!h || !dev_data || !dev_meta || !granule_offset || !chunk_offset) return KMR_ERR_INVALID_ARG;
	int rc = sk_exchange_ready(h, "kmr_sk_exchange_pack_dev"); if (rc) return rc;
	hipSetDevice(h->device);
	const uint32_t world = h->cfg.world_size;
	unsigned int head = 0;
	HIPCHK(h, hipMemcpy(&head, h->l1.head.get<unsigned int>(), 4, hipMemcpyDeviceToHost));
	if (head > h->l1.cap) head = h->l1.cap;
	DevBuf db; HIPCHK(h, db.alloc(32 * SK_OWNER_MAX));
	unsigned long long *d = db.get<unsigned long long>();
	std::vector<unsigned long long> hv(4 * SK_OWNER_MAX, 0);
	for (uint32_t r = 0; r < world; r++) { hv[r] = granule_offset[r]; hv[SK_OWNER_MAX + r] = chunk_offset[r]; }
	hipError_t e = hipMemcpyAsync(d, hv.data(), 32 * SK_OWNER_MAX, hipMemcpyHostToDevice, h->stream);
	if (e == hipSuccess && head) {
		hipLaunchKernelGGL(sk_pack_kernel, dim3(grid_for((uint64_t)head * 64, 256, num_cus(h) * 8)), dim3(256), 0, h->stream, pool_view(h, h->l1), head, world, h->cfg.rank,
		                   d, d + SK_OWNER_MAX, d + 2 * SK_OWNER_MAX, d + 3 * SK_OWNER_MAX, (uint4 *)dev_data, (uint2 *)dev_meta, h->xr_lo, h->xr_hi);
		hipLaunchKernelGGL(sk_state_drop_kernel, dim3(grid_for(sk_list_count(h->sk_bits))), dim3(256), 0, h->stream, h->sk_state.get<unsigned long long>(), sk_list_count(h->sk_bits), world, h->cfg.rank, h->xr_lo, h->xr_hi);
		e = hipGetLastError();
	}
	if (e == hipSuccess) e = hipStreamSynchronize(h->stream);
	HIPCHK(h, e);
	return KMR_OK;
}
int kmr_sk_exchange_range(kmr_handle *h, uint64_t list_lo, uint64_t list_hi) {
	if (!h || list_lo > list_hi) return KMR_ERR_INVALID_ARG;
	h->xr_lo = list_lo; h->xr_hi = list_hi;
	return KMR_OK;
}
int kmr_count_lists_prefix(kmr_handle *h, uint32_t min_depth, uint64_t list_hi) {
	if (!h) return KMR_ERR_INVALID_ARG;
	if (h->finalized) return fail(h, KMR_ERR_STATE, "kmr_count_lists_prefix after kmr_finalize");
	if (!h->superkmer_mode) return KMR_OK;
	hipSetDevice(h->device);
	return count_prefix_superkmer(h, min_depth, list_hi);
}
int kmr_sk_exchange_uniform(kmr_handle *h, uint64_t *state) {
	if (!h || !state) return KMR_ERR_INVALID_ARG;
	*state = h->sk_uni_mixed ? (2ull << 32) : (h->sk_uni_w == SK_UNI_NONE ? 0ull : ((1ull << 32) | h->sk_uni_w));
	return KMR_OK;
}
int kmr_sk_exchange_peer_uniform(kmr_handle *h, uint64_t state) {
	if (!h) return KMR_ERR_INVALID_ARG;
	const uint32_t kind = (uint32_t)(state >> 32), w = (uint32_t)state;
	if (kind > 2) return fail(h, KMR_ERR_INVALID_ARG, "bad uniform-weight state");
	h->peers_declare = true;
	if (kind == 2) h->peer_uni_mixed = true;
	else if (kind == 1) { if (h->peer_uni_w == SK_UNI_NONE) h->peer_uni_w = w; else if (h->peer_uni_w != w) h->peer_uni_mixed = true; }
	return KMR_OK;
}
int kmr_sk_exchange_adopt_dev(kmr_handle *h, const void *dev_data, const void *dev_meta, uint64_t n_chunks, uint64_t n_granules) {
	if (!h || (n_chunks && (!dev_data || !dev_meta))) return KMR_ERR_INVALID_ARG;
	int rc = sk_exchange_ready(h, "kmr_sk_exchange_adopt_dev"); if (rc) return rc;
	const bool declared = h->peers_declare;
	h->peers_declare = false;
	if (n_chunks == 0) return KMR_OK;
	hipSetDevice(h->device);
	rc = sk_ensure_state(h); if (rc) return rc;
	const int grid = (int)std::min<uint64_t>((n_chunks + SK_ADOPT_WAVES * SK_ADOPT_GROUP - 1) / (SK_ADOPT_WAVES * SK_ADOPT_GROUP), (uint64_t)num_cus(h) * 8);
	rc = pool_reserve(h, h->l1, n_chunks + n_granules / SK_CHUNK_G + (sk_list_count(h->sk_bits) / h->cfg.world_size) + (uint64_t)grid * SK_ADOPT_WAVES * 130 + 64, true); if (rc) return rc;
	const size_t need = 8 * (n_chunks + 1) + 4 * (n_chunks + 1) + 256;
	rc = h->adopt_buf.reserve(h, "adopt_buf", need, need + need / 4); if (rc) return rc;
	uint64_t *start = (uint64_t *)h->adopt_buf.get<uint8_t>(); uint32_t *cnt = (uint32_t *)(h->adopt_buf.get<uint8_t>() + 8 * (n_chunks + 1));
	hipLaunchKernelGGL(sk_meta_counts_kernel, dim3(grid_for(n_chunks)), dim3(256), 0, h->stream, (const uint2 *)dev_meta, n_chunks, cnt);
	rc = exclusive_scan(h, cnt, n_chunks, start);
	if (!rc && !h->d_uni && !declared) {
		if (h->d_uni.alloc(8) != hipSuccess) rc = fail(h, KMR_ERR_OOM, "uniform-weight flags");
		else { const uint32_t init[2] = {SK_UNI_NONE, 0u}; if (hipMemcpyAsync(h->d_uni.get<uint32_t>(), init, 8, hipMemcpyHostToDevice, h->stream) != hipSuccess) rc = fail(h, KMR_ERR_HIP, "uniform-weight flags"); else hipStreamSynchronize(h->stream); }
	}
	if (!rc && !declared) hipLaunchKernelGGL(sk_uniform_check_kernel, dim3(grid_for(n_chunks)), dim3(256), 0, h->stream, (const uint4 *)dev_data, start, cnt, n_chunks, h->d_uni.get<uint32_t>());
	if (!rc) {
		hipLaunchKernelGGL(sk_adopt_kernel, dim3(grid), dim3(SK_ADOPT_WAVES * 64), 0, h->stream, (const uint4 *)dev_data, (const uint2 *)dev_meta, start, n_chunks, sk_params(h), pool_view(h, h->l1));
		if (hipGetLastError() != hipSuccess) rc = fail(h, KMR_ERR_HIP, "sk_adopt_kernel launch");
	}
	hipStreamSynchronize(h->stream);
	return rc ? rc : sync_state(h);
}

int kmr_size_tracker(kmr_handle *h, int force_last, uint64_t *elements, uint64_t capacity, uint64_t *n_elements) {
	if (!h || !n_elements) return KMR_ERR_INVALID_ARG;
	if (!h->cfg.size_tracker) return fail(h, KMR_ERR_STATE, "kmr_size_tracker: kmr_config.size_tracker was not set");
	if (!h->finalized) return fail(h, KMR_ERR_STATE, "kmr_size_tracker before kmr_finalize");
	const uint64_t n = h->trk_elems.size() / 4 + (force_last ? 1 : 0);
	*n_elements = n;
	if (!elements) return KMR_OK;
	if (capacity < n) return fail(h, KMR_ERR_CAPACITY, "kmr_size_tracker: element buffer too small");
	if (!h->trk_elems.empty()) memcpy(elements, h->trk_elems.data(), 8 * h->trk_elems.size());
	if (force_last) {
		const uint64_t sub = h->cfg.kmer_subsample > 1 ? h->cfg.kmer_subsample : 1;
		uint64_t *e = elements + h->trk_elems.size();
		e[0] = h->stats.raw_kmers * sub; e[1] = h->stats.raw_good_kmers * sub; e[2] = h->stats.unique_kmers * sub; e[3] = h->stats.singleton_kmers * sub;
	}
	return KMR_OK;
}

#include "kmr_exchange_rccl.hpp"

int kmr_kernel_time(kmr_handle *h, int which, double *ms, uint64_t *launches) {
	if (!h || which < 0 || which >= KMR_TIME_GROUPS) return KMR_ERR_INVALID_ARG;
	hipSetDevice(h->device);
	int rc = sync_state(h); if (rc) return rc;
	if (ms) *ms = h->ms[which];
	if (launches) *launches = h->launches[which];
	return KMR_OK;
}
int kmr_kernel_time_reset(kmr_handle *h) {
	if (!h) return KMR_ERR_INVALID_ARG;
	int rc = sync_state(h); if (rc) return rc;
	for (int i = 0; i < KMR_TIME_GROUPS; i++) { h->ms[i] = 0; h->launches[i] = 0; }
	return KMR_OK;
}

}

namespace {

enum { CMP_B_ACC = 0, CMP_B_NK, CMP_B_KOFF, CMP_B_STAGE, CMP_B_CNT, CMP_B_LOFF, CMP_B_SRC, CMP_B_RID, CMP_B_PERM, CMP_B_HSCAN, CMP_B_START, CMP_B_COUNT };
static_assert(CMP_B_COUNT == sizeof(HandleMem::cmp_buf) / sizeof(DevBuf), "kmr_host.hpp's cmp_buf holds one block per CMP_B_ index");

DevParams own_reads_params(kmr_handle *h, bool whole) {
	DevParams dp = dev_params(h);
	dp.sub_wstart = dp.sub_wkeys = dp.sub_sstart = dp.sub_skeys = nullptr; dp.sub_wvals = nullptr; dp.sub_sweight = nullptr; dp.sub_wnb = dp.sub_snb = 0;
	if (whole) { dp.subsample = 1; dp.world = 1; dp.rank = 0; dp.num_parts = 1; dp.part_idx = 0; }
	return dp;
}

int kmer_slots_queue(kmr_handle *h, const uint64_t *offsets, uint64_t n, uint32_t *nk, uint64_t *koff, unsigned int *most_err) {
	hipLaunchKernelGGL(compare_nk_kernel, dim3(grid_for(n)), dim3(256), 0, h->stream, offsets, n, h->k, nk, most_err, most_err + 1);
	HIPCHK(h, hipGetLastError());
	return exclusive_scan_queue(h, nk, n, koff);
}
int kmer_slot_plan(kmr_handle *h, const uint64_t *offsets, uint64_t n, uint64_t **koff, uint64_t *total, unsigned int *most, const char *refusal) {
	DevBuf *B = h->cmp_buf;
	int rc = B[CMP_B_ACC].reserve(h, "compare counters", 256); if (rc) return rc;
	rc = B[CMP_B_NK].reserve(h, "compare k-mer counts", 4 * std::max<uint64_t>(n, 1)); if (rc) return rc;
	rc = B[CMP_B_KOFF].reserve(h, "compare k-mer offsets", 8 * (n + 1)); if (rc) return rc;
	unsigned int *most_err = (unsigned int *)((unsigned long long *)(B[CMP_B_ACC].get<CompareRec>() + 1) + CMP_T_WORDS), hm[2] = {0, 0};
	*koff = B[CMP_B_KOFF].get<uint64_t>(); *total = 0;
	HIPCHK(h, hipMemsetAsync(most_err, 0, 8, h->stream));
	rc = kmer_slots_queue(h, offsets, n, B[CMP_B_NK].get<uint32_t>(), *koff, most_err); if (rc) return rc;
	HIPCHK(h, hipMemcpyAsync(total, *koff + n, 8, hipMemcpyDeviceToHost, h->stream));
// ... 447 lines not shown
```

kmernator_amd/csrc/kmr_host.hpp:

```cpp
#ifndef KMR_HOST_HPP_
#define KMR_HOST_HPP_

#include <hip/hip_runtime.h>
#include <unistd.h>

#include <algorithm>
#include <atomic>
#include <cstdio>
#include <memory>
#include <string>
#include <type_traits>
#include <utility>
#include <vector>

#include "../../include/kmernator_amd.h"

#define KMR_HIDDEN __attribute__((visibility("hidden")))

namespace kmr { struct SkPacked; }

namespace kmr_host KMR_HIDDEN {

inline std::string g_create_error;

// ... 48 lines not shown
struct DevMap {
	uint64_t nb = 0, n = 0;
	DevBuf start;
	DevBuf keys;
	DevBuf vals;
	DevBuf sweight;
	DevBuf spkt;
	DevBuf image;
	bool present = false;
};

struct HostPool {
	DevBuf base, chunk_list, chunk_count, head;
	uint32_t cap = 0; size_t chunk_bytes = 0;
	uint64_t used_ub = 0;
	uint64_t presize = 0;
};

struct HandleMem {
	DevBuf slots, extslots;
	DevBuf dP, dstats, derr;
	DevMap weak, sing;
	DevBuf ix_start, ix_keys, ix_counts;
	DevBuf scratch_stats;
	DevBuf adopt_buf;
	DevBuf trk;
	DevBuf scan_sums;
	DevBuf score_buf;
	DevBuf bimodal_buf;
	DevBuf fasta_buf[2][3];
	DevBuf lut;
	DevBuf dPk;
	DevBuf d_uni;
	DevBuf qrange;
	DevBuf sk_fine_state;
	struct Early { bool active = false; uint64_t hi = 0; uint32_t min_depth = 0; DevBuf ue, cursor, fc, err; } early;
	DevBuf dedup_tab;
	DevBuf xo_dev;
	DevBuf cmp_buf[11];
	SortBufs cmp_sort;
};
struct BuildMem {
	DevBuf sk_state;
	HostPool l1;
	DevBuf work_counter;
	DevBuf l1_state; bool l1_state_dirty = false;
	DevBuf arena; size_t arena_used = 0, arena_want = 0; std::vector<DevBuf> arena_overflow;
	DevBuf linear;
	DevBuf tile_count, kcap, koff;
	DevBuf ucnt, ufirst, u_start, u_end, u_read, umax;
	DevBuf tb_bases, tb_quals, tb_rel, tb_off, tb_len;
	uint64_t tb_quals_filled = 0; int tb_quals_char = -1;
	DevBuf tb_stage[2][8];
	DevBuf uw_keys, uw_vals, us_keys, us_b8, us_pkt;
	DevBuf ue, ue2;
};
struct ExchangeMem {
	DevBuf xc_small, xc_dcounts;
	DevBuf xc_send, xc_send2, xc_recv, xc_recv2;
};

}
using namespace kmr_host;

struct KMR_HIDDEN Tuning {
	uint64_t target_list = 2048;
	uint64_t sub_batch_bases = 0;
	int recycle = -1;
	int part_blocks = 0;
	double entry_share = -1.0;
	double early_entry_share = -1.0;
	uint64_t saturated_batch_bytes = 0;
	bool no_lut = false, no_narrow = false, no_l1_state = false, no_stream_lookups = false;
	uint64_t long_list_chunks = 0;
	uint64_t binned_min = 1ull << 18;
	bool bb_fixed_bins = true;
	double bb_slack_bins = 1.0, bb_slack_groups = 1.0;
	bool bb_reload = false;
	uint64_t twobit_piece_bases = 0;
	uint64_t list_aim = 0;
	bool pow2_lists = false;
	bool no_packed_direct = false;
	bool no_uniform_count = false;
	int count_blocks = 0;
	bool no_lean_extract = false;
	bool exchange_fail_once = false;
	uint64_t dump_piece_bytes = 0;
	uint64_t dump_tiles_per_block = 0;
	bool dump_timing = false;
	bool select_timing = false;
	bool pairs_timing = false;
	bool dedup_timing = false;
	uint32_t partition_units = 0;
	int artifact_report_lds = -1;
	uint32_t pair_hash_bits = 64;
	int bimodal_window = -1;
	bool csr_partition = true;
	int compare_lds_kmers = -1;
	uint64_t compare_stage_kmers = 0;
	uint32_t tnf_piece_bases = 0;
	uint64_t match_hit_capacity = 0;
	uint64_t extend_stage_kmers = 0;
	bool extend_timing = false;
	bool no_coarse_lists = true;
};

struct KMR_HIDDEN FeedHints {
	const kmr::SkPacked *packed = nullptr;
	int uniform_q = -1;
	uint64_t call_bases = 0;
	uint64_t piece_origin = 0;
};

struct KMR_HIDDEN kmr_handle : HandleMem, BuildMem, ExchangeMem {
	kmr_config cfg;
	Tuning tune;
	uint32_t k = 0, kb = 0, hkb = 0, W = 0;
	bool ext = false;
	int device = 0, ncu = 0;
	hipStream_t stream = nullptr;
	std::string err;
	uint32_t log2cap = 0;
	uint64_t occupied = 0;
	uint64_t pending_kmers = 0;
	uint64_t stream_base = 0, reads = 0;
	uint64_t nb_weak = 0, nb_sing = 0;
	bool finalized = false, has_singletons = true;
	kmr_handle *subtract = nullptr;
	uint64_t subtracted = 0;
	kmr_stats stats;
	bool partition_mode = false;
	bool superkmer_mode = false;
	uint64_t ix_lists = 0, ix_gen = ~0ull;
	uint64_t trk_n = 0; std::vector<uint64_t> trk_elems;
	long trk_next = 128; uint64_t trk_raw = 0, trk_good = 0; std::vector<unsigned long long> trk_bounds; std::vector<uint64_t> trk_snap_raw, trk_snap_good;
	bool sk_fast_div = false;
	bool sk_exchange = false;
	bool auto_mode = false;
	int bits1 = 0;
	uint64_t inserted_records = 0;
	uint32_t lut_log2 = 0;
	uint64_t lut_gen = ~0ull, map_gen = 0;
	hipStream_t tb_copy_stream = nullptr; hipEvent_t tb_ready[2] = {nullptr, nullptr}, tb_consumed[2] = {nullptr, nullptr}; bool tb_set_used[2] = {false, false};
	uint32_t sk_bits = 0, sk_m = 0, sk_off = 0, sk_win = 0;
	double hP[256], hPk[256];
	uint32_t sk_uni_w = 0xffffffffu; bool sk_uni_mixed = false; bool last_count_uniform = false;
	uint32_t peer_uni_w = 0xffffffffu; bool peer_uni_mixed = false, peers_declare = false;
	uint64_t xr_lo = 0, xr_hi = ~0ull;
	uint64_t last_early_hi = 0, last_early_entries = 0;
	int last_bb_path = 0; bool last_bb_fallback = false;
	double bimodal_sigmas = -1.0; uint64_t bimodal_n = ~0ull; bool bimodal_on = false;
	std::vector<uint64_t> sel_bimodal; bool sel_bimodal_set = false;
	int last_score_path = 0;
	bool last_early_overflowed = false;
	double last_score_ms = 0, last_select_ms = 0, last_write_ms = 0;
	int last_artifact_report_lds = 0;
	double last_dump_size_ms = 0, last_dump_write_ms = 0;
	uint64_t last_dump_tiles_per_block = 0, last_dump_blocks = 0;
	double last_pairs_ms = 0, last_pairs_parse_ms = 0, last_pairs_sort_ms = 0;
	double last_dedup_ms = 0, last_dedup_key_ms = 0, last_dedup_sort_ms = 0, last_dedup_consensus_ms = 0;
	uint64_t last_pair_hash_collisions = 0;
	uint64_t last_saturated_keys = 0, last_saturated_batches = 0;
	int last_csr_path = -1; uint32_t last_csr_chunks = 0;
	unsigned int l1_head_seen = 0;
	uint64_t unit_batches = 0;
	int last_match_attempts = 0;
	int last_extend_runs = 0; double last_extend_ms[5] = {0, 0, 0, 0, 0};
	int last_count_blocks = 0;
	int last_count_attempts = 0;
	bool qual_mixed = false;
	uint32_t sk_fine_shift = 0;
	uint64_t xo_segcap = 0; std::vector<uint64_t> xo_counts; const void *xo_batch = nullptr; uint64_t xo_first = 0;
	void *xc_comm = nullptr; kmr_transport xc_tr = {nullptr, nullptr, nullptr};
	uint64_t xc_job_bases = 0, xc_bytes_to_peers = 0;
	hipEvent_t ev0 = nullptr, ev1 = nullptr;
	double ms[KMR_TIME_GROUPS] = {0};
	uint64_t launches[KMR_TIME_GROUPS] = {0};
	std::vector<std::pair<hipEvent_t, hipEvent_t> > pending_events[KMR_TIME_GROUPS];
};

struct OnDevice { int device = 0; };

struct KMR_HIDDEN kmr_picks : OnDevice {
	DevBuf text, picked;
	uint64_t n = 0, n_picked = 0, bytes = 0;
	DevBuf read_seg;
	std::vector<uint64_t> seg_table;
	uint32_t n_rounds = 1, n_inputs = 1;
	float round_depth[33] = {};
	uint8_t round_is_remainder[33] = {};
	bool normalized = false;
	uint64_t norm_info[3] = {};
};

struct KMR_HIDDEN kmr_pairs : OnDevice {
	DevBuf mate, read1, read2;
	uint64_t n = 0, n_pairs = 0, n_full = 0, n_seq = 0, n_conflicts = 0;
};

struct KMR_HIDDEN kmr_text : OnDevice {
	DevBuf text;
	uint64_t kept = 0, bytes = 0;
};

struct KMR_HIDDEN kmr_reads : OnDevice {
	DevBuf bases, quals;
	DevBuf offsets;
	DevBuf name_off, name_len;
// ... 141 lines not shown
```

kmernator_amd/csrc/kmr_instances.hpp:

```cpp
#ifndef KMR_INSTANCES_HPP_
#define KMR_INSTANCES_HPP_

#include "kmr_superkmer.hpp"
#include "kmr_compare.hpp"
#include "kmr_match.hpp"
#include "kmr_extend.hpp"

namespace kmr {

static const int COUNT_LOG2S = 10;
static const int COUNT_LOG2S_EXT = 9;
static const int PD_THREADS = 1024, PD_RPT = 8, PD_LINE = 4;

#ifdef KMR_INSTANCES_EXTERN
#define KMR_T extern template
#else
#define KMR_T template
#endif

#define KMR_SKX(W, WIN, FILT) KMR_T __global__ void sk_extract_kernel<W, WIN, FILT, false>(ReadsView, DevParams, SkParams, PoolView); KMR_T __global__ void sk_extract_kernel<W, WIN, FILT, true>(ReadsView, DevParams, SkParams, PoolView);
#define KMR_SKXL(W, WIN) KMR_T __global__ void sk_extract_lean_kernel<W, WIN, false>(ReadsView, DevParams, SkParams, PoolView, float, SkPacked); KMR_T __global__ void sk_extract_lean_kernel<W, WIN, true>(ReadsView, DevParams, SkParams, PoolView, float, SkPacked);
#define KMR_SKX_W(W) KMR_SKX(W, 16, false) KMR_SKX(W, 16, true) KMR_SKX(W, 8, false) KMR_SKX(W, 8, true) KMR_SKX(W, 4, false) KMR_SKX(W, 4, true) KMR_SKXL(W, 16) KMR_SKXL(W, 8) KMR_SKXL(W, 4)

#define KMR_SKX_W32(W) KMR_SKX(W, 32, false) KMR_SKX(W, 32, true) KMR_SKXL(W, 32)

#define KMR_SKC(W, TRACK) KMR_SKCX(W, TRACK, false)
#define KMR_SKCB(W, TRACK, EXT, UNI, ITEM, BLOCKS) KMR_T __global__ void sk_count_kernel<W, EXT ? COUNT_LOG2S_EXT : COUNT_LOG2S, TRACK, EXT, UNI, ITEM, BLOCKS>(const uint4 *, const uint64_t *, const uint64_t *, uint64_t, uint32_t, SkCountHot, unsigned int *, uint32_t, const SkCountArgs<W> *);
#define KMR_SKCI(W, TRACK, EXT, UNI, ITEM) KMR_SKCB(W, TRACK, EXT, UNI, ITEM, 0)
#define KMR_SKC5 KMR_SKCB(1, false, false, true, false, 5)
#define KMR_SKCX(W, TRACK, EXT) KMR_SKCI(W, TRACK, EXT, false, false)
#define KMR_SKL(W) KMR_T __global__ void sk_lookup_kernel<W>(PoolView, const uint64_t *, const uint64_t *, uint64_t, uint32_t, const uint64_t *, const uint64_t *, const uint32_t *, uint32_t *, uint64_t, unsigned int *, const uint64_t *, const uint64_t *, const uint32_t *, uint64_t, uint64_t);
#define KMR_SKCU(W) KMR_SKCI(W, false, false, true, false)
#define KMR_SKC_W(W) KMR_SKC(W, false) KMR_SKCU(W) KMR_SKC(W, true) KMR_SKCX(W, false, true) \
	KMR_SKCI(W, false, false, false, true) KMR_SKCI(W, false, false, true, true) KMR_SKCI(W, false, true, false, true) KMR_SKL(W)

#define KMR_EX(W, EXT, OP, SUB) KMR_T __global__ void extract_kernel<W, EXT, OP, SUB>(ReadsView, DevParams, OP);
#define KMR_EX_OP(W, EXT, ...) KMR_T __global__ void extract_kernel<W, EXT, __VA_ARGS__, false>(ReadsView, DevParams, __VA_ARGS__); KMR_T __global__ void extract_kernel<W, EXT, __VA_ARGS__, true>(ReadsView, DevParams, __VA_ARGS__);
#define KMR_EX_W(W) \
	KMR_EX_OP(W, false, InsertOp<W, false>) KMR_EX_OP(W, true, InsertOp<W, true>) \
	KMR_EX_OP(W, false, LinearOp<W, false, false>) KMR_EX_OP(W, false, LinearOp<W, false, true>) \
	KMR_EX_OP(W, true, LinearOp<W, true, false>) KMR_EX_OP(W, true, LinearOp<W, true, true>) \
	KMR_T __global__ void extract_kernel<W, false, LookupOp<W>, false>(ReadsView, DevParams, LookupOp<W>); \
	KMR_T __global__ void extract_kernel<W, false, LookupWeightOp<W>, false>(ReadsView, DevParams, LookupWeightOp<W>); \
	KMR_EX_OP(W, false, CompareOp<W>) KMR_EX_OP(W, false, MatchOp<W>) KMR_EX_OP(W, false, ExtendOp<W>)

#define KMR_PD(W, EXT, LEVEL) KMR_T __global__ void partition_direct_kernel<W, EXT, LEVEL, PD_THREADS, PD_RPT, PD_LINE>(PartSource<W>, PoolView, unsigned int *, const int, const int);
#define KMR_OS(W, EXT, REQ) KMR_T __global__ void owner_scatter_kernel<W, EXT, REQ>(const typename PoolRec<W, EXT>::type *, const uint64_t *, const uint32_t *, uint64_t, uint32_t, uint32_t, uint32_t *, uint64_t, unsigned long long *, unsigned int *, uint32_t *, uint32_t *, OwnerFn);
#define KMR_CK(W, EXT, LOG2S, NARROW) KMR_T __global__ void count_kernel<W, EXT, LOG2S, NARROW>(PoolView, const uint64_t *, const uint64_t *, uint64_t, CountOut, FinalizeParams, unsigned int *, int);
#define KMR_PART_W(W) \
	KMR_PD(W, false, 1) KMR_PD(W, false, 2) KMR_PD(W, true, 1) KMR_PD(W, true, 2) \
	KMR_OS(W, false, false) KMR_OS(W, false, true) KMR_OS(W, true, false) KMR_OS(W, true, true) \
	KMR_CK(W, false, COUNT_LOG2S, false) KMR_CK(W, false, 11, false) KMR_CK(W, true, COUNT_LOG2S, false)

#if defined(KMR_INSTANCES_EXTERN)
KMR_SKX_W(1) KMR_SKX_W(2) KMR_SKX_W(3) KMR_SKX_W(4)
KMR_SKX_W32(2) KMR_SKX_W32(3) KMR_SKX_W32(4)
KMR_SKC_W(1) KMR_SKC_W(2) KMR_SKC_W(3) KMR_SKC_W(4) KMR_SKC5
KMR_EX_W(1) KMR_EX_W(2) KMR_EX_W(3) KMR_EX_W(4)
KMR_PART_W(1) KMR_PART_W(2) KMR_PART_W(3) KMR_PART_W(4)
KMR_CK(1, true, COUNT_LOG2S, true)
#else
#ifdef KMR_INST_SKX
KMR_SKX_W(KMR_INST_W)
#if KMR_INST_W > 1
KMR_SKX_W32(KMR_INST_W)
#endif
#endif
#ifdef KMR_INST_SKC
KMR_SKC_W(KMR_INST_W)
#if KMR_INST_W == 1
KMR_SKC5
#endif
#endif
#ifdef KMR_INST_EX
KMR_EX_W(KMR_INST_W)
#endif
#ifdef KMR_INST_PART
KMR_PART_W(KMR_INST_W)
#if KMR_INST_W == 1
KMR_CK(1, true, COUNT_LOG2S, true)
#endif
#endif
#endif

}
#endif
```

kmernator_amd/csrc/kmr_kernels.hpp:

```cpp
#ifndef KMR_KERNELS_HPP_
#define KMR_KERNELS_HPP_

#include <hip/hip_runtime.h>
#include <stdint.h>
#include <string.h>

#include "kmr_key.hpp"

namespace kmr {

static const uint64_t EMPTY_KEY = ~0ull;
static const uint64_t NO_FIRST = ~0ull;

static const int FIRST_ORD_SHIFT = 24;
static const uint64_t MAX_STREAM_ORDINAL = (1ull << 40) - 1;
__host__ __device__ __forceinline__ uint32_t first_weight_bits(float w) {
#if defined(__HIP_DEVICE_COMPILE__)
	const uint32_t bits = __float_as_uint(w);
#else
	uint32_t bits; memcpy(&bits, &w, 4);
#endif
	const uint32_t ex = (bits >> 23) & 0xffu;
	if (ex == 0 || ex > 127u) return ex > 127u ? (254u << 15) : 0u;
	const uint32_t prod = ((bits & 0x7fffffu) | 0x800000u) * 254u;
	const uint32_t sh = 8u + (127u - ex);
	return sh < 32u ? prod >> sh : 0u;
}
__host__ __device__ __forceinline__ unsigned long long first_pack(uint64_t ordinal, bool forward, float w) {
	return ((unsigned long long)ordinal << FIRST_ORD_SHIFT) | ((unsigned long long)(forward ? 1u : 0u) << 23) | (unsigned long long)(first_weight_bits(w) & 0x7fffffu);
}
__host__ __device__ __forceinline__ bool first_forward(unsigned long long f) { return ((f >> 23) & 1ull) != 0; }
__host__ __device__ __forceinline__ double first_weight_shift(unsigned long long f) {
	const uint32_t q8 = (uint32_t)(f >> 15) & 0xffu, r15 = (uint32_t)f & 0x7fffu;
	const double w1 = ((double)q8 + ((double)r15 + 0.5) / 32768.0) / 254.0;
	return (double)(float)((double)q8 / 254.0) - w1;
}
static const int WAVES_PER_BLOCK = 4;
#ifndef KMR_TILE_BUF
#define KMR_TILE_BUF 9856
#endif
static const int TILE_BUF = KMR_TILE_BUF;
static const int TILE_SPAN = TILE_BUF - 32;

enum { ERR_READ_TOO_LONG = 1, ERR_TABLE_FULL = 2, ERR_SEGMENT_OVERFLOW = 4 };

struct DevStats {
	unsigned long long raw, good, claimed;
	unsigned long long inserted;
	unsigned long long subtracted;
	unsigned long long sender_bad;
};

struct DevParams {
	uint32_t k, kb;
	float min_weight;
	uint32_t fastq_start, ext_min_q;
	uint32_t qzero;
	uint32_t subsample, rank, world, num_parts, part_idx;
	uint32_t count_sender_bad;
	const double *P;
	DevStats *stats;
	uint32_t *err;
	const uint64_t *sub_wstart, *sub_wkeys; const uint32_t *sub_wvals; uint64_t sub_wnb; uint32_t sub_vw;
	const uint64_t *sub_sstart, *sub_skeys; const uint8_t *sub_sweight; uint64_t sub_snb;
};

struct ReadsView {
	const uint8_t *bases;
	const uint8_t *quals;
	const uint64_t *offsets;
	const uint8_t *discarded;
	uint64_t n_reads;
	uint64_t stream_base;
	uint64_t first_read_idx;
	const uint64_t *u_start, *u_end, *u_read;
	uint64_t n_units;
};

static const uint32_t UNIT_KMERS = 9216;
#ifndef KMR_INSTANCE_TU
__global__ void unit_max_kernel(const uint64_t *offsets, uint64_t n, unsigned int *maxLen) {
	unsigned int mx = 0;
	for (uint64_t r = blockIdx.x * (uint64_t)blockDim.x + threadIdx.x; r < n; r += (uint64_t)gridDim.x * blockDim.x) {
		const uint64_t L = offsets[r + 1] - offsets[r];
		mx = L > mx ? (unsigned int)(L > 0xffffffffull ? 0xffffffffu : L) : mx;
	}
#pragma unroll
	for (int off = 32; off > 0; off >>= 1) { unsigned int o = __shfl_xor(mx, off, 64); mx = o > mx ? o : mx; }
	if ((threadIdx.x & 63) == 0 && mx > __hip_atomic_load(maxLen, __ATOMIC_RELAXED, __HIP_MEMORY_SCOPE_AGENT)) atomicMax(maxLen, mx);
}
__global__ void unit_count_kernel(const uint64_t *offsets, uint64_t n, uint32_t k, uint32_t span, uint32_t *counts) {
	for (uint64_t r = blockIdx.x * (uint64_t)blockDim.x + threadIdx.x; r < n; r += (uint64_t)gridDim.x * blockDim.x) {
		const uint64_t L = offsets[r + 1] - offsets[r];
		counts[r] = L <= span ? 1u : (uint32_t)((L - k + 1 + UNIT_KMERS - 1) / UNIT_KMERS);
	}
}
#endif
#ifndef KMR_INSTANCE_TU
__global__ void unit_fill_kernel(const uint64_t *offsets, uint64_t n, uint32_t k, uint32_t span, const uint64_t *ufirst,
                                 uint64_t *u_start, uint64_t *u_end, uint64_t *u_read) {
	for (uint64_t r = blockIdx.x * (uint64_t)blockDim.x + threadIdx.x; r < n; r += (uint64_t)gridDim.x * blockDim.x) {
		const uint64_t b = offsets[r], e = offsets[r + 1], L = e - b;
		const uint64_t u0 = ufirst[r], nu = ufirst[r + 1] - u0;
		if (L <= span) { u_start[u0] = b; u_end[u0] = e; u_read[u0] = r; continue; }
		for (uint64_t g = 0; g < nu; g++) {
			const uint64_t s0 = b + g * UNIT_KMERS, e0 = s0 + UNIT_KMERS + k - 1;
			u_start[u0 + g] = s0; u_end[u0 + g] = e0 < e ? e0 : e; u_read[u0 + g] = r;
		}
	}
}
#endif

template <int W> struct Slot;
template <> struct Slot<1> {
	uint64_t key;
	unsigned long long cntfwd;
	double wsum;
	unsigned long long first;
};
template <int W> struct Slot {
	uint64_t key[W];
	unsigned long long cntfwd;
	double wsum;
	unsigned long long first;
	uint32_t state;
	uint32_t pad;
};
struct ExtSlot {
	uint32_t tally[12];
	uint32_t pkt;
	uint32_t pad[3];
};

// ... 1298 lines not shown
```

kmernator_amd/csrc/kmr_superkmer.hpp:

```cpp
#ifndef KMR_SUPERKMER_HPP_
#define KMR_SUPERKMER_HPP_

#include "kmr_partition.hpp"
#include "kmr_buckets.hpp"

namespace kmr {

#ifndef KMR_SK_MAX_N
#define KMR_SK_MAX_N 128
#endif
static const uint32_t SK_CHUNK_G = 64;
static const uint32_t SK_MAX_N = KMR_SK_MAX_N;
static const int SK_WAVES = 3;
static const int SK_WINDOW = 16;
static const int SK_RR = 3, SKL_RR = 4;

#ifdef KMR_DEBUG_HOOKS
#define SK_DBG(flags, bit) (((flags) & (bit)) != 0)
#else
#define SK_DBG(flags, bit) false
#endif
struct SkTrackRec { uint32_t raw, good; unsigned long long end_ordinal; };
static const uint32_t SK_TRACK_MAX = 512;
struct SkTrackView { const unsigned long long *bounds; uint32_t n; unsigned int *d_unique, *d_single; };

struct SkParams {
	uint32_t dbg;
	uint32_t m;
	uint32_t off;
	uint32_t list_bits;
	uint32_t fast_div;
	const double *Rp;
	uint32_t keep_all_owners;
	unsigned long long *state;
	struct SkTrackRec *track;
	const double *Pk;
};

struct SkBoundary { uint64_t read; uint32_t t, good; unsigned long long ordinal; };
template <int W>
__global__ __launch_bounds__(64)
void sk_track_boundary_kernel(ReadsView rv, DevParams p, SkBoundary *bd, uint32_t n_bd) {
	const uint32_t i = blockIdx.x * blockDim.x + threadIdx.x;
	if (i >= n_bd) return;
	const uint64_t r = bd[i].read, b0 = rv.offsets[r], L = rv.offsets[r + 1] - b0;
	const uint32_t k = p.k, target = bd[i].t;
	const uint8_t *bs = rv.bases + b0, *qs = rv.quals ? rv.quals + b0 : nullptr;
	const bool isRef = !qs || (L > 0 && qs[0] == 127);
	const bool filt = p.subsample > 1 || p.num_parts > 1 || p.world > 1;
	Roller<W> roll; roll.init(k);
	double w = 0.0;
	uint32_t raw = 0, good = 0, nN = 0;
	unsigned long long ord = rv.stream_base + b0 + L;
	for (uint64_t j = 0; j < L; j++) {
		const uint32_t code = base_code(bs[j]);
		nN += code >> 2;
		if (j >= k) nN -= base_code(bs[j - k]) >> 2;
		if (filt) roll.push(code & 3u);
		if (j + 1 < k) continue;
		const uint64_t x = j + 1 - k;
		if (isRef) w = 1.0;
		else if (x % 1024 == 0 || w == 0.0) { w = 1.0; for (uint32_t jj = 0; jj < k; jj++) w *= p.P[qs[x + jj]]; }
		else w *= p.P[qs[x + k - 1]] / p.P[qs[x - 1]];
		if (nN) w = 0.0;
		bool mine = true;
		if (filt) {
			const Key<W> kf = roll.getFwd(), kr = roll.getRc();
			const Key<W> canon = key_le<W>(kf, kr) ? kf : kr;
			const uint64_t hash = key_hash<W>(canon, p.kb);
			if (p.subsample > 1 && hash % p.subsample != 0) mine = false;
			if (p.world > 1 && distributed_thread_id(hash, p.world) != p.rank) mine = false;
			if (p.num_parts > 1 && distributed_thread_id(hash, p.num_parts) != p.part_idx) mine = false;
		}
		if (!mine) continue;
		raw++;
		if ((float)w > p.min_weight) good++;
		if (raw == target) { ord = rv.stream_base + b0 + x + 1; break; }
	}
	bd[i].good = good; bd[i].ordinal = ord;
}

static const uint32_t SK_EXT_X = 5u;
__host__ __device__ __forceinline__ uint32_t sk_base_granules(uint32_t n, uint32_t k) { return (n + k - 1 + 63) / 64; }
__host__ __device__ __forceinline__ uint32_t sk_ext_granules(uint32_t n) { return (n + 7) / 8; }
__host__ __device__ __forceinline__ uint32_t sk_rec_granules(uint32_t n, uint32_t k, bool uniform, bool ext) { return 1 + sk_base_granules(n, k) + (uniform ? 0u : (n + 3) / 4) + (ext ? sk_ext_granules(n) : 0u); }
__device__ __forceinline__ uint32_t sk_hdr_n(uint32_t y) { return (y >> 8) & 0xffu; }
__device__ __forceinline__ bool sk_hdr_uniform(uint32_t y) { return ((y >> 16) & 1u) != 0; }
__device__ __forceinline__ uint32_t sk_hdr_granules(uint32_t y) { return (y >> 17) & 0x7fu; }
__device__ __forceinline__ uint64_t sk_hdr_ordinal(uint32_t x, uint32_t y) { return (uint64_t)x | ((uint64_t)(y & 0xffu) << 32); }
__device__ __forceinline__ bool sk_hdr_is_ext(uint32_t y) { return ((y >> 30) & 1u) != 0; }
__device__ __forceinline__ uint32_t sk_hdr_ext_left(uint32_t y) { return (y >> 24) & 7u; }
__device__ __forceinline__ uint32_t sk_hdr_ext_right(uint32_t y) { return (y >> 27) & 7u; }
__device__ __forceinline__ uint32_t sk_hdr_ext(uint32_t left, uint32_t right) { return (left << 24) | (right << 27) | (1u << 30); }
__device__ __forceinline__ uint4 sk_make_header(unsigned long long ord, uint32_t n, bool uniform, uint32_t granules, uint32_t ext, uint32_t mhash, uint32_t wbits) {
	return make_uint4((uint32_t)ord, (uint32_t)(ord >> 32) | (n << 8) | ((uniform ? 1u : 0u) << 16) | (granules << 17) | ext, mhash, wbits);
}
__device__ __forceinline__ uint32_t sk_pend_make(uint32_t start, uint32_t n, bool uniform, uint32_t pos) { return (1u << 31) | (pos << 25) | ((uniform ? 1u : 0u) << 24) | (n << 16) | start; }
static const uint32_t SK_PEND_ADDRESS = 1u << 30;
__device__ __forceinline__ uint32_t sk_pend_start(uint32_t q) { return q & 0xffffu; }
__device__ __forceinline__ uint32_t sk_pend_n(uint32_t q) { return (q >> 16) & 0xffu; }
__device__ __forceinline__ bool sk_pend_uniform(uint32_t q) { return ((q >> 24) & 1u) != 0; }
__device__ __forceinline__ uint32_t sk_pend_pos(uint32_t q) { return (q >> 25) & 15u; }
__device__ __forceinline__ bool sk_pend_is_address(uint32_t q) { return ((q >> 30) & 1u) != 0; }
__device__ __forceinline__ bool sk_pend_live(uint32_t q) { return (q >> 31) != 0; }

#ifndef KMR_INSTANCE_TU
__global__ void sk_state_init_kernel(unsigned long long *state, uint64_t n) {
	for (uint64_t i = blockIdx.x * (uint64_t)blockDim.x + threadIdx.x; i < n; i += (uint64_t)gridDim.x * blockDim.x) state[i] = ((unsigned long long)NO_CHUNK << 32) | SK_CHUNK_G;
}
#endif
#ifndef KMR_INSTANCE_TU
__global__ void sk_close_kernel(const unsigned long long *state, uint64_t n, uint32_t *chunk_count, uint32_t cap) {
	for (uint64_t i = blockIdx.x * (uint64_t)blockDim.x + threadIdx.x; i < n; i += (uint64_t)gridDim.x * blockDim.x) {
		const unsigned long long s = state[i];
		const uint32_t c = (uint32_t)(s >> 32), f = (uint32_t)s;
		if (c != NO_CHUNK && c < cap) chunk_count[c] = f < SK_CHUNK_G ? f : SK_CHUNK_G;
	}
}
#endif

__device__ __forceinline__ void sk_wave_lds_order() { asm volatile("" ::: "memory"); __builtin_amdgcn_wave_barrier(); asm volatile("" ::: "memory"); }

__device__ __forceinline__ uint32_t sk_wave_scan_u32(uint32_t x) {
	x += (uint32_t)__builtin_amdgcn_update_dpp(0, (int)x, 0x111, 0xf, 0xf, true);
	x += (uint32_t)__builtin_amdgcn_update_dpp(0, (int)x, 0x112, 0xf, 0xf, true);
	x += (uint32_t)__builtin_amdgcn_update_dpp(0, (int)x, 0x114, 0xf, 0xf, true);
	x += (uint32_t)__builtin_amdgcn_update_dpp(0, (int)x, 0x118, 0xf, 0xf, true);
	x += (uint32_t)__builtin_amdgcn_update_dpp(0, (int)x, 0x142, 0xa, 0xf, false);
	x += (uint32_t)__builtin_amdgcn_update_dpp(0, (int)x, 0x143, 0xc, 0xf, false);
	return x;
}

struct SkSlab { uint32_t base[2]; uint32_t next; uint32_t hot_list; unsigned long long hot_state; };
static const uint32_t SK_NO_LIST = 0xffffffffu, SK_LIST_LOCKED = 0xfffffffeu;
static const int SK_HOT_AFTER = 3;
__device__ __forceinline__ uint32_t sk_alloc_chunk(SkSlab *slab, const PoolView &pool) {
	const uint32_t idx = atomicAdd(&slab->next, 1u);
	uint32_t c;
	if (idx < 128u) c = slab->base[idx >> 6] + (idx & 63u);
	else c = atomicAdd(pool.head, 1u);
	if (c >= pool.cap) { atomicOr(pool.err, (uint32_t)ERR_POOL_FULL); return NO_CHUNK; }
	return c;
}
__device__ __forceinline__ uint64_t sk_append_settle(unsigned long long *state, uint32_t list, uint32_t g, unsigned long long old, SkSlab *slab, const PoolView &pool, bool &waits) {
	const uint32_t c = (uint32_t)(old >> 32), f = (uint32_t)old;
	if (f + g <= SK_CHUNK_G) return (uint64_t)c * SK_CHUNK_G + f;
	if (f <= SK_CHUNK_G) {
		if (c != NO_CHUNK) pool.chunk_count[c] = f;
		const uint32_t c2 = sk_alloc_chunk(slab, pool);
		if (c2 == NO_CHUNK) { atomicExch(state + list, ((unsigned long long)NO_CHUNK << 32) | (SK_CHUNK_G + 1)); return ~0ull; }
		pool.chunk_list[c2] = list;
		atomicExch(state + list, ((unsigned long long)c2 << 32) | g);
		return (uint64_t)c2 * SK_CHUNK_G;
	}
	waits = true;
	return ~0ull;
}
__device__ __forceinline__ uint64_t sk_append_hot(SkSlab *slab, uint32_t list, uint32_t g, const PoolView &pool) {
	for (int spin = 0; spin < 4096; spin++) {
		const unsigned long long old = atomicAdd(&slab->hot_state, (unsigned long long)g);
		const uint32_t c = (uint32_t)(old >> 32), f = (uint32_t)old;
		if (f + g <= SK_CHUNK_G) return (uint64_t)c * SK_CHUNK_G + f;
		if (f <= SK_CHUNK_G) {
			pool.chunk_count[c] = f;
			const uint32_t c2 = sk_alloc_chunk(slab, pool);
			if (c2 == NO_CHUNK) return ~0ull;
			pool.chunk_list[c2] = list; pool.chunk_count[c2] = 0;
			atomicExch(&slab->hot_state, ((unsigned long long)c2 << 32) | g);
			return (uint64_t)c2 * SK_CHUNK_G;
		}
	}
	atomicOr(pool.err, (uint32_t)ERR_POOL_FULL);
	return ~0ull;
}
__device__ __forceinline__ uint64_t sk_append(unsigned long long *state, uint32_t list, uint32_t g, SkSlab *slab, const PoolView &pool) {
	unsigned long long *word = state + list;
	for (int spin = 0; spin < (1 << 22); spin++) {
		if (spin >= SK_HOT_AFTER) {
			uint32_t hl = slab->hot_list;
			if (hl == SK_NO_LIST && atomicCAS(&slab->hot_list, SK_NO_LIST, SK_LIST_LOCKED) == SK_NO_LIST) {
				const uint32_t c2 = sk_alloc_chunk(slab, pool);
				if (c2 == NO_CHUNK) { slab->hot_list = SK_NO_LIST; return ~0ull; }
				pool.chunk_list[c2] = list; pool.chunk_count[c2] = 0;
				slab->hot_state = ((unsigned long long)c2 << 32) | g;
				__builtin_amdgcn_fence(__ATOMIC_RELEASE, "workgroup");
				__hip_atomic_store(&slab->hot_list, list, __ATOMIC_RELEASE, __HIP_MEMORY_SCOPE_WORKGROUP);
				return (uint64_t)c2 * SK_CHUNK_G;
			}
			hl = __hip_atomic_load(&slab->hot_list, __ATOMIC_ACQUIRE, __HIP_MEMORY_SCOPE_WORKGROUP);
			if (hl == list) return sk_append_hot(slab, list, g, pool);
		}
// ... 991 lines not shown
struct SkRec { uint32_t n; const uint32_t *bases, *weights; bool uniform; uint64_t ord0; };
__device__ __forceinline__ SkRec sk_enter_record(const uint4 *wstage, uint32_t rs, uint32_t x, uint32_t y, uint32_t k) {
	SkRec r;
	r.n = sk_hdr_n(y);
	r.bases = (const uint32_t *)(wstage + rs + 1);
	r.weights = r.bases + 4 * sk_base_granules(r.n, k);
	r.uniform = sk_hdr_uniform(y);
	r.ord0 = sk_hdr_ordinal(x, y);
	return r;
}

template <int W> __device__ __forceinline__ Key<W> sk_cut_kmer(const uint32_t *bases, uint32_t j) {
	Key<W> kf;
	const uint32_t d0 = j >> 4, sft = 2u * (j & 15u);
#pragma unroll
	for (int wi = 0; wi < W; wi++) {
		const uint32_t a = bases[d0 + 2 * wi], b = bases[d0 + 2 * wi + 1], c = bases[d0 + 2 * wi + 2];
		const uint64_t hi = ((uint64_t)a << 32) | b;
		kf.w[wi] = sft ? (hi << sft) | ((uint64_t)c >> (32 - sft)) : hi;
	}
	return kf;
}
template <int W> __device__ __forceinline__ void key_clip_tail(Key<W> &kf, uint32_t k) {
	const uint32_t kbits = 2u * k;
#pragma unroll
	for (int wi = 0; wi < W; wi++) {
		const uint32_t lo = 64u * wi;
		if (kbits <= lo) kf.w[wi] = 0;
		else if (kbits < lo + 64u) kf.w[wi] &= ~0ull << (lo + 64u - kbits);
	}
}
template <int W> __device__ __forceinline__ Key<W> key_canonical(const Key<W> &kf, uint32_t k, bool &fwd) {
	const Key<W> kr = key_revcomp<W>(kf, k);
	fwd = key_le<W>(kf, kr);
	return fwd ? kf : kr;
}

template <int W, int LOG2S> struct SkKeySet {
	static constexpr int S = 1 << LOG2S;
	uint64_t *tkeys; uint32_t *tval, *tstate;
	__device__ __forceinline__ void clear(int t, int threads) const { for (int i = t; i < S; i += threads) tstate[i] = 0; }
	__device__ __forceinline__ void put(const uint64_t *key, uint32_t value) const {
		uint64_t kw[W];
#pragma unroll
		for (int q = 0; q < W; q++) kw[q] = key[q];
		uint32_t sl = (uint32_t)(slot_hash<W>(kw) >> (64 - LOG2S));
		while (atomicCAS(&tstate[sl], 0u, 1u) != 0u) sl = (sl + 1) & (S - 1);
#pragma unroll
		for (int q = 0; q < W; q++) tkeys[(size_t)sl * W + q] = kw[q];
		tval[sl] = value;
	}
	__device__ __forceinline__ uint32_t find(const Key<W> &key, uint32_t miss) const {
		uint32_t sl = (uint32_t)(slot_hash<W>(key.w) >> (64 - LOG2S));
		uint32_t value = miss;
		for (int probe = 0; probe < S; probe++) {
			if (tstate[sl] == 0) break;
			bool eq = true;
#pragma unroll
			for (int q = 0; q < W; q++) eq = eq && tkeys[(size_t)sl * W + q] == key.w[q];
			if (eq) { value = tval[sl]; break; }
			sl = (sl + 1) & (S - 1);
		}
		return value;
	}
};

static const int SK_STAGE_CHUNKS = 4;
static const int SK_STAGE_G = SK_STAGE_CHUNKS * SK_CHUNK_G;
static const uint32_t SK_LBATCH = 24;
static const uint32_t SK_DESC_CAP = 160;

template <int W> struct SkLong {
	const uint64_t *item_c0, *item_c1;
	uint64_t n_items;
	uint64_t long_threshold;
	uint32_t list_first, list_stride;
	Table<W> merge;
	unsigned long long *merge_used;
};

struct SkCountHot {
	uint64_t *wout;
	uint32_t *wvals; unsigned long long *wcursor; uint64_t wcap;
	uint32_t min_depth, has_singletons, uni_wbits, ext_min_q;
};
template <int W> struct SkCountArgs { CountOut out; FinalizeParams f; SkTrackView tv; SkLong<W> lg; };
template <int W> __host__ inline SkCountHot sk_count_hot(const SkCountArgs<W> &a) {
	return {a.out.wentries ? a.out.wentries : a.out.wkeys, a.out.wvals, a.out.wcursor, a.out.wcap, a.f.min_depth, a.f.has_singletons, a.f.uni_wbits, a.f.ext_min_q};
}
template <int W> __global__ void sk_count_args_kernel(SkCountArgs<W> a, SkCountArgs<W> *dst) { if (threadIdx.x == 0 && blockIdx.x == 0) *dst = a; }

template <int W, int LOG2S, bool TRACK = false, bool EXT = false, bool UNI = false>
__host__ __device__ constexpr size_t sk_count_smem_bytes() { return (size_t)(1 << LOG2S) * (8 * W + 24 + (W > 1 ? 4 : 0) - (UNI ? 8 : 0) - (UNI && W > 1 ? 4 : 0) + (TRACK ? 8 : 0) + (EXT ? 28 : 0)) + (size_t)SK_STAGE_G * 16 + 256 + 64 + (TRACK ? 8 * (SK_TRACK_MAX + 1) : 0); }
static const uint64_t SK_EXT_LONG_CHUNKS = 128;
static const int SK_EXT_BLOCKS = 3;
__device__ __forceinline__ uint32_t sk_ext_char(uint32_t code) { return (uint32_t)((0x584e54474341ull >> (8 * code)) & 0xffu); }

#ifndef KMR_SKC_WAVES
#define KMR_SKC_WAVES 4
#endif
static const int SKC_WAVES = KMR_SKC_WAVES, SKC_THREADS = SKC_WAVES * 64;
static const unsigned long long SK_KEY_PENDING = ~0ull;
static const uint32_t SK_ORDERED_FROM = 256;
static const unsigned long long SK_OSLAB = 2048;

template <int BLOCKS> __device__ __forceinline__ uint32_t skc_uni(uint32_t x) { if constexpr (BLOCKS == 5) return (uint32_t)__builtin_amdgcn_readfirstlane((int)x); else return x; }
template <int BLOCKS> __device__ __forceinline__ unsigned long long skc_uni64(unsigned long long x) { if constexpr (BLOCKS == 5) return ((unsigned long long)skc_uni<5>((uint32_t)(x >> 32)) << 32) | skc_uni<5>((uint32_t)x); else return x; }
template <int BLOCKS> __device__ __forceinline__ unsigned long long skc_slab_base(unsigned long long g) {
	if constexpr (BLOCKS == 5) return skc_uni64<5>(g);
	else return ((unsigned long long)(uint32_t)__shfl((int)(g >> 32), 0, 64) << 32) | (uint32_t)__shfl((int)(uint32_t)g, 0, 64);
}
template <int W, int LOG2S, bool TRACK, bool EXT, bool UNI, bool ITEM>
__host__ __device__ constexpr int sk_count_default_blocks() { return EXT ? (W == 1 ? (LOG2S <= 9 ? SK_EXT_BLOCKS : 2) : 1) : ((W == 1 && LOG2S <= 10 && !TRACK) ? 4 : (W == 2 && LOG2S <= 10 && !TRACK ? (UNI ? 4 : 3) : 1)); }
template <int W, int LOG2S, bool TRACK = false, bool EXT = false, bool UNI = false, bool ITEM = false, int BLOCKS = 0>
__global__ __launch_bounds__(SKC_THREADS, (BLOCKS ? BLOCKS : sk_count_default_blocks<W, LOG2S, TRACK, EXT, UNI, ITEM>()))
void sk_count_kernel(const uint4 *poolg, const uint64_t *list_start, const uint64_t *list_chunks, uint64_t n_lists, uint32_t k,
                     SkCountHot hot, unsigned int *work_counter, uint32_t dbgFlags, const SkCountArgs<W> *__restrict__ args) {
	const CountOut &out = args->out; const FinalizeParams &f = args->f; const SkTrackView &tv = args->tv; const SkLong<W> &lg = args->lg;
	static_assert(!UNI || (!TRACK && !EXT), "the one-weight count pass is the plain one's");
	static_assert(BLOCKS == 0 || (BLOCKS == 5 && W == 1 && UNI && !ITEM), "only the one-weight, one-word pass over lists has a five-block instance");
	constexpr int S = 1 << LOG2S;
	constexpr bool LEAN = UNI && W > 1;
	constexpr bool WSUM = !UNI;
	constexpr bool PACKED = !EXT;
	static_assert(!ITEM || !TRACK, "the size tracker's pass has no long-list items");
#ifndef KMR_SKC_LIMIT_PCT
#define KMR_SKC_LIMIT_PCT 80
#endif
	constexpr uint32_t LIMIT = (uint32_t)(S * (KMR_SKC_LIMIT_PCT / 100.0));
	constexpr int WSLOTS = S / SKC_WAVES;
	extern __shared__ __attribute__((aligned(16))) uint8_t csm[];
	uint64_t *tkeys = (uint64_t *)csm;
	unsigned long long *tcnt = (unsigned long long *)(tkeys + (size_t)S * W);
	double *twsum = (double *)(tcnt + S);
	unsigned long long *tfirst = (unsigned long long *)(twsum + (WSUM ? S : 0));
	uint32_t *tstate = (uint32_t *)(tfirst + S);
	uint32_t *ttally = tstate + (W > 1 && !LEAN ? S : 0);
	uint32_t *tpkt = ttally + (EXT ? 6 * S : 0);
	uint4 *stage = (uint4 *)(tpkt + (EXT ? S : 0));
	uint8_t *recOf = (uint8_t *)(stage + SK_STAGE_G);
	unsigned long long *tsecond = (unsigned long long *)(csm + (size_t)S * (8 * W + 24 + (W > 1 ? 4 : 0) + (EXT ? 28 : 0)) + (size_t)SK_STAGE_G * 16 + 256 + 64);
	unsigned int *trkU = (unsigned int *)(tsecond + (TRACK ? S : 0)), *trkS = trkU + (SK_TRACK_MAX + 1);
	__shared__ uint32_t s_list, s_sp;
	__shared__ uint32_t s_claimed[2], s_overflow[2];
	__shared__ unsigned long long s_sat[2];
	__shared__ uint32_t s_stackBits[40], s_stackVal[40];
	__shared__ unsigned long long s_c0[SK_LBATCH + 1], s_c1[SK_LBATCH + 1];
	__shared__ uint32_t s_dchunk[SK_DESC_CAP];
	__shared__ uint8_t s_dcount[SK_DESC_CAP];
	const int t = threadIdx.x, lane = t & 63, wv = (int)skc_uni<BLOCKS>((uint32_t)(t >> 6));
	if (TRACK) for (int i = t; i < 2 * (int)(SK_TRACK_MAX + 1); i += SKC_THREADS) trkU[i] = 0;
	const uint32_t vw = EXT ? 15 : 3;
	unsigned long long uniqW = 0, singleW = 0, keptW = 0, keptS = 0;
	unsigned long long wpos = 0, wend = 0, spos = 0, send = 0;
	bool outFull = false;
	if (t == 0) { s_claimed[0] = s_claimed[1] = 0; s_overflow[0] = s_overflow[1] = 0; s_sp = 0; s_sat[0] = s_sat[1] = 0; }
	for (int i = t; i < S; i += SKC_THREADS) { tkeys[(size_t)i * W] = EMPTY_KEY; if (W > 1) tkeys[(size_t)i * W + W - 1] = SK_KEY_PENDING; tcnt[i] = 0; if constexpr (WSUM) twsum[i] = 0.0; tfirst[i] = NO_FIRST; if constexpr (W > 1 && !LEAN) tstate[i] = 0; if (TRACK) tsecond[i] = NO_FIRST; }
	if (EXT) for (int i = t; i < 6 * S; i += SKC_THREADS) ttally[i] = 0;
	lds_barrier();
	const uint32_t singC = hot.has_singletons ? (hot.min_depth > 1 ? 0u : 2u) : 3u;
	const uint32_t weakMin = ((!hot.has_singletons || hot.min_depth > 2) && hot.min_depth != 1) ? hot.min_depth : 0u;
	const uint32_t uniFirst = UNI ? (first_weight_bits(__uint_as_float(hot.uni_wbits)) & 0x7fffffu) : 0u;
	uint4 pre = make_uint4(0, 0, 0, 0); uint32_t preCount = 0; uint64_t preList = ~0ull;
	uint32_t gen = 0;

	constexpr bool itemMode = ITEM;
	constexpr uint32_t grab = itemMode ? 1u : SK_LBATCH;
	for (;;) {
		if (t == 0) s_list = atomicAdd(work_counter, grab);
		lds_barrier();
		const uint64_t lfirst = skc_uni<BLOCKS>(s_list);
		const uint64_t stride = lg.list_stride ? lg.list_stride : 1u;
		const uint64_t n_work = itemMode ? lg.n_items : (n_lists > lg.list_first ? (n_lists - lg.list_first + stride - 1) / stride : 0);
		if (lfirst >= n_work) break;
		const uint32_t nl = (uint32_t)(n_work - lfirst < (uint64_t)grab ? n_work - lfirst : (uint64_t)grab);
		if ((uint32_t)t < nl) {
			uint64_t a, b;
			if (itemMode) { a = lg.item_c0[lfirst + t]; b = lg.item_c1[lfirst + t]; }
			else { const uint64_t l = lg.list_first + (lfirst + t) * stride; a = list_start[l]; b = list_start[l + 1]; if (lg.long_threshold && b - a > lg.long_threshold) b = a; }
			s_c0[t] = a; s_c1[t] = b;
		}
		lds_barrier();
		const uint64_t dbase = skc_uni64<BLOCKS>(itemMode ? s_c0[0] : list_start[lg.list_first + lfirst * stride]), dend = skc_uni64<BLOCKS>(itemMode ? s_c1[0] : list_start[lg.list_first + (lfirst + nl - 1) * stride + 1]);
		const uint64_t dcached = dend - dbase < (uint64_t)SK_DESC_CAP ? dend - dbase : (uint64_t)SK_DESC_CAP;
		for (uint64_t i = (uint64_t)t; i < dcached; i += SKC_THREADS) { const uint64_t d = list_chunks[dbase + i]; s_dchunk[i] = (uint32_t)d; s_dcount[i] = (uint8_t)(d >> 32); }
		lds_barrier();
		auto describe = [&](uint64_t ci, uint32_t &chunk, uint32_t &count) {
			if (ci - dbase < dcached) { chunk = s_dchunk[ci - dbase]; count = s_dcount[ci - dbase]; }
			else { const uint64_t d = list_chunks[ci]; chunk = (uint32_t)d; count = (uint32_t)(d >> 32); }
			if constexpr (BLOCKS == 5) { chunk = skc_uni<BLOCKS>(chunk); count = skc_uni<BLOCKS>(count); }
		};
		auto fetch = [&](uint64_t ci, uint4 &v, uint32_t &count) {
			uint32_t chunk;
			describe(ci, chunk, count);
			v = make_uint4(0, 0, 0, 0);
			if ((uint32_t)lane < count) v = poolg[(size_t)chunk * SK_CHUNK_G + lane];
		};
		for (uint32_t lj = 0; lj < nl; lj++) {
			const uint64_t c0 = skc_uni64<BLOCKS>(s_c0[lj]), c1 = skc_uni64<BLOCKS>(s_c1[lj]);
			if (c0 == c1) continue;
			if (itemMode && (__hip_atomic_load(out.err, __ATOMIC_RELAXED, __HIP_MEMORY_SCOPE_AGENT) & ERR_TABLE_FULL)) continue;
			uint32_t fl = gen & 1u;
			gen++;
			auto insert_pass = [&](const uint32_t bits, const uint32_t val, const bool firstPass) {
				const uint32_t subMask = bits ? ((1u << bits) - 1) : 0;
				const bool padded = W > 1 && (LEAN || (k & 31u) != 0);
				uint4 *wstage = stage + wv * SK_CHUNK_G;
				uint8_t *wrecOf = recOf + wv * 64;
				uint4 cur = make_uint4(0, 0, 0, 0); uint32_t curCount = 0;
				if (firstPass && preList == lfirst + lj) { cur = pre; curCount = preCount; }
				else if (c0 + wv < c1) fetch(c0 + wv, cur, curCount);
				bool wantPre = firstPass;
				if (firstPass) preList = ~0ull;
				for (uint64_t ci = c0 + wv; ci < c1 && !skc_uni<BLOCKS>(s_overflow[fl]) && skc_uni<BLOCKS>(s_claimed[fl]) <= LIMIT; ci += SKC_WAVES) {
					wstage[lane] = cur;
					uint32_t claimedHere = 0;
					const unsigned long long starts = sk_record_starts<true, EXT>(cur.y, curCount, lane, k);
					const SkDeal deal = sk_deal(starts, cur, lane, wrecOf);
					const uint32_t Lk = deal.Lk;
					uint32_t left = deal.left, rs = deal.rs, j = deal.j, hx = deal.hx, hy = deal.hy, hw = deal.hw;
					if (SK_DBG(dbgFlags, 4)) left = 0;
					uint4 nxt = make_uint4(0, 0, 0, 0); uint32_t nxtCount = 0, nxtChunk = 0, preChunk = 0;
					const bool wantNxt = ci + SKC_WAVES < c1;
					bool havePre = false;
					if (wantNxt) describe(ci + SKC_WAVES, nxtChunk, nxtCount);
					if (wantPre) {
						wantPre = false;
						if (lj + 1 < nl) { const uint64_t n0 = skc_uni64<BLOCKS>(s_c0[lj + 1]), n1 = skc_uni64<BLOCKS>(s_c1[lj + 1]); if (n0 + wv < n1) { describe(n0 + wv, preChunk, preCount); havePre = true; preList = lfirst + lj + 1; } }
					}
					if (wantNxt && (uint32_t)lane < nxtCount) nxt = poolg[(size_t)nxtChunk * SK_CHUNK_G + lane];
					if (havePre) { pre = make_uint4(0, 0, 0, 0); if ((uint32_t)lane < preCount) pre = poolg[(size_t)preChunk * SK_CHUNK_G + lane]; }
					uint32_t n = 0; const uint32_t *ww = nullptr; bool uniformW = true; uint64_t ord0 = 0;
					const uint8_t *xq = nullptr;
					uint32_t leftCarry = 0;
					auto enter_record = [&]() {
						const SkRec rec = sk_enter_record(wstage, rs, hx, hy, k);
						n = rec.n; ww = rec.weights; uniformW = rec.uniform; ord0 = rec.ord0;
						if (EXT) xq = (const uint8_t *)(ww + (uniformW ? 0u : 4u * ((n + 3) / 4)));
					};
					constexpr int NWD = 2 * W + 2;
					uint32_t win[NWD], sb = 0;
#pragma unroll
					for (int i = 0; i < NWD; i++) win[i] = 0;
					auto seed_window = [&]() {
						const uint32_t *bw = (const uint32_t *)(wstage + rs + 1) + (j >> 4);
#pragma unroll
						for (int i = 0; i < NWD; i++) win[i] = bw[i];
						sb = 2u * (j & 15u);
					};
					struct KState { Key<W> key; bool fwd, mine; uint32_t slot, step, w; uint64_t ord; uint32_t x; };
					KState kA, kB;
#pragma unroll
					for (int wi = 0; wi < W; wi++) { kA.key.w[wi] = 0; kB.key.w[wi] = 0; }
					kA.fwd = kB.fwd = true; kA.mine = kB.mine = false; kA.slot = kB.slot = 0; kA.step = kB.step = 1; kA.w = kB.w = 0; kA.ord = kB.ord = 0; kA.x = kB.x = 0;
					auto prepare = [&](KState &st) {
						Key<W> kf;
						const bool up = sb >= 32u; const uint32_t r = sb & 31u;
#pragma unroll
						for (int wi = 0; wi < W; wi++) {
							const uint32_t d0 = up ? win[2 * wi + 1] : win[2 * wi], d1 = up ? win[2 * wi + 2] : win[2 * wi + 1], d2 = up ? win[2 * wi + 3] : win[2 * wi + 2];
							const uint32_t hi = (uint32_t)(((((uint64_t)d0) << 32 | d1) << r) >> 32), lo = (uint32_t)(((((uint64_t)d1) << 32 | d2) << r) >> 32);
							kf.w[wi] = ((uint64_t)hi << 32) | lo;
						}
						uint32_t rcIn = 0; uint64_t kfFirst = 0;
						if constexpr (EXT) {
							kfFirst = kf.w[0];
							if ((k >> 5) < (uint32_t)W) { uint64_t wsel = kf.w[0];
#pragma unroll
								for (int wi = 1; wi < W; wi++) if ((k >> 5) == (uint32_t)wi) wsel = kf.w[wi];
								rcIn = (uint32_t)(wsel >> (62u - 2u * (k & 31u))) & 3u; }
							else { const uint32_t b = j + k; rcIn = (((const uint32_t *)(wstage + rs + 1))[b >> 4] >> (30 - 2 * (b & 15u))) & 3u; }
						}
						if constexpr (W == 1) {
							const uint32_t padBits = 64u - 2u * k;
							kf.w[0] &= ~0ull << padBits;
							uint32_t rh = __builtin_bitreverse32((uint32_t)kf.w[0]), rl = __builtin_bitreverse32((uint32_t)(kf.w[0] >> 32));
							rh = ((rh >> 1) & 0x55555555u) | ((rh & 0x55555555u) << 1);
							rl = ((rl >> 1) & 0x55555555u) | ((rl & 0x55555555u) << 1);
							const uint64_t kr = (((uint64_t)~rh << 32) | (uint32_t)~rl) << padBits;
							st.fwd = kf.w[0] <= kr;
							st.key.w[0] = st.fwd ? kf.w[0] : kr;
						} else {
							key_clip_tail<W>(kf, k);
							st.key = key_canonical<W>(kf, k, st.fwd);
						}
						const uint64_t h = slot_hash<W>(st.key.w);
						st.slot = (uint32_t)(h >> (64 - LOG2S));
						st.step = ((uint32_t)(h >> (64 - 2 * LOG2S)) & (uint32_t)(S - 1)) | 1u;
						st.mine = ((uint32_t)(h >> 20) & subMask) == val;
						if constexpr (!UNI) st.w = uniformW ? hw : ww[j];
						st.ord = ord0 + j;
						if constexpr (EXT) {
							uint32_t lc = j > 0 ? leftCarry : sk_hdr_ext_left(hy), rc = sk_hdr_ext_right(hy);
							if (j + 1 < n) rc = rcIn;
							leftCarry = (uint32_t)(kfFirst >> 62);
							const uint32_t q2 = ((const uint16_t *)xq)[j];
							uint32_t lq = q2 & 0xffu, rq = q2 >> 8;
							if (!st.fwd) {
								const uint32_t tl = rc < 4u ? 3u - rc : rc, tr = lc < 4u ? 3u - lc : lc, tq = rq;
								lc = tl; rc = tr; rq = lq; lq = tq;
							}
							st.x = lc | (rc << 8) | (lq << 16) | (rq << 24);
						}
					};
					if (left) {
						enter_record(); seed_window();
						if (EXT && j > 0) { const uint32_t b = j - 1; leftCarry = (((const uint32_t *)(wstage + rs + 1))[b >> 4] >> (30 - 2 * (b & 15u))) & 3u; }
						prepare(kA);
					}
					uint32_t dbgSink = 0;
					auto step_one = [&](KState &cur, KState &nxt) {
						if (left) {
							uint32_t s = cur.slot;
							const float wa = __uint_as_float(UNI ? hot.uni_wbits : cur.w);
							unsigned long long old = EMPTY_KEY;
							const bool tableOn = !SK_DBG(dbgFlags, 1) && cur.mine;
							if (W == 1 || padded) { if (tableOn) old = atomicCAS((unsigned long long *)&tkeys[(size_t)s * W], (unsigned long long)EMPTY_KEY, (unsigned long long)cur.key.w[0]); }
							j++; left--; sb += 2;
							if (left) {
								if (j >= n) {
									rs = rs + sk_hdr_granules(hy);
									{ const uint32_t g0 = rs < SK_CHUNK_G - 1 ? rs : SK_CHUNK_G - 1; const uint4 hh = wstage[g0]; hx = hh.x; hy = hh.y; hw = hh.w; }
									j = 0;
									seed_window();
									enter_record();
								} else if (sb > 62u) seed_window();
								prepare(nxt);
							}
							if (SK_DBG(dbgFlags, 1)) { dbgSink ^= (uint32_t)cur.key.w[0] ^ s; }
							else if (cur.mine) {
								bool placed = false;
								const uint32_t claimedBefore = claimedHere;
								if constexpr (W == 1) {
									if (old == EMPTY_KEY) { claimedHere++; placed = true; }
									else if (old == cur.key.w[0]) placed = true;
									else s = (s + cur.step) & (S - 1);
								}
								if (W > 1 && padded) {
									bool poll = false;
									for (int probe = 0; probe < 8 * S; probe++) {
										const bool active = !placed;
										if (probe > 0 && active && !poll) old = atomicCAS((unsigned long long *)&tkeys[(size_t)s * W], (unsigned long long)EMPTY_KEY, (unsigned long long)cur.key.w[0]);
										const bool won = active && !poll && old == EMPTY_KEY;
										if (won) {
#pragma unroll
											for (int qq = 1; qq < W - 1; qq++) tkeys[(size_t)s * W + qq] = cur.key.w[qq];
											__hip_atomic_store(&tkeys[(size_t)s * W + W - 1], cur.key.w[W - 1], __ATOMIC_RELEASE, __HIP_MEMORY_SCOPE_WORKGROUP);
											claimedHere++; placed = true;
										}
										sk_wave_lds_order();
										if (active && !won) {
											bool moveOn = true;
											if (old == cur.key.w[0]) {
												const unsigned long long last = __hip_atomic_load(&tkeys[(size_t)s * W + W - 1], __ATOMIC_ACQUIRE, __HIP_MEMORY_SCOPE_WORKGROUP);
												if (last == SK_KEY_PENDING) { poll = true; moveOn = false; }
												else {
													bool eq = last == cur.key.w[W - 1];
#pragma unroll
													for (int qq = 1; qq < W - 1; qq++) eq = eq && (tkeys[(size_t)s * W + qq] == cur.key.w[qq]);
													if (eq) { placed = true; moveOn = false; }
												}
											}
											if (moveOn) { poll = false; s = (s + cur.step) & (S - 1); }
										}
										if (!__any(!placed)) break;
									}
								}
								for (int probe = 0; probe < S && !placed && !(W > 1 && padded); probe++) {
									if constexpr (W == 1) {
										const unsigned long long o2 = atomicCAS((unsigned long long *)&tkeys[s], (unsigned long long)EMPTY_KEY, (unsigned long long)cur.key.w[0]);
										if (o2 == EMPTY_KEY) { claimedHere++; placed = true; break; }
										if (o2 == cur.key.w[0]) { placed = true; break; }
									} else if constexpr (!LEAN) {
										uint32_t st = __hip_atomic_load(&tstate[s], __ATOMIC_ACQUIRE, __HIP_MEMORY_SCOPE_WORKGROUP);
										if (st == 0) {
											const uint32_t old2 = atomicCAS(&tstate[s], 0u, 1u);
											if (old2 == 0) {
#pragma unroll
												for (int qq = 0; qq < W; qq++) tkeys[(size_t)s * W + qq] = cur.key.w[qq];
												__hip_atomic_store(&tstate[s], 2u, __ATOMIC_RELEASE, __HIP_MEMORY_SCOPE_WORKGROUP);
												claimedHere++;
												placed = true; break;
											}
											st = old2;
										}
										if (st == 1) { probe--; continue; }
										bool eq = true;
#pragma unroll
										for (int qq = 0; qq < W; qq++) eq = eq && (tkeys[(size_t)s * W + qq] == cur.key.w[qq]);
										if (eq) { placed = true; break; }
									}
									s = (s + cur.step) & (S - 1);
								}
								if (!placed) s_overflow[fl] = 1;
								else {
									atomicAdd(&tcnt[s], 1ull | ((unsigned long long)(cur.fwd ? 1 : 0) << 32));
									if constexpr (!UNI) atomicAdd(&twsum[s], (double)wa);
									const unsigned long long fp = UNI ? (((unsigned long long)cur.ord << FIRST_ORD_SHIFT) | ((unsigned long long)(cur.fwd ? 1u : 0u) << 23) | (unsigned long long)uniFirst) : first_pack(cur.ord, cur.fwd, wa);
									if (TRACK) {
										const unsigned long long was = atomicMin(&tfirst[s], fp);
										const unsigned long long cand = was > fp ? was : fp;
										if (cand != NO_FIRST) atomicMin(&tsecond[s], cand);
									} else atomicMin(&tfirst[s], fp);
									if constexpr (EXT) {
										const uint32_t lc = cur.x & 0xffu, rc = (cur.x >> 8) & 0xffu, lq = (cur.x >> 16) & 0xffu, rq = cur.x >> 24;
										if (lq >= hot.ext_min_q || lc > 3u) atomicAdd(&ttally[(size_t)s * 6 + (lc >> 1)], 1u << (16 * (lc & 1u)));
										if (rq >= hot.ext_min_q || rc > 3u) atomicAdd(&ttally[(size_t)s * 6 + 3 + (rc >> 1)], 1u << (16 * (rc & 1u)));
										if (claimedHere != claimedBefore) tpkt[s] = sk_ext_char(lc) | (sk_ext_char(rc) << 8) | (cur.x & 0xffff0000u);
									}
								}
							}
						}
					};
					for (uint32_t it = 0; it < Lk; it += 2) { step_one(kA, kB); step_one(kB, kA); }
					if (SK_DBG(dbgFlags, 1) && dbgSink == 0x12345u) s_overflow[fl] = 2;
					claimedHere = (uint32_t)__builtin_amdgcn_readlane((int)sk_wave_scan_u32(claimedHere), 63);
					if (lane == 0 && claimedHere) atomicAdd(&s_claimed[fl], claimedHere);
					sk_wave_lds_order();
					cur = nxt; curCount = nxtCount;
				}
				if (wantPre && lj + 1 < nl) { const uint64_t n0 = skc_uni64<BLOCKS>(s_c0[lj + 1]), n1 = skc_uni64<BLOCKS>(s_c1[lj + 1]); if (n0 + wv < n1) { fetch(n0 + wv, pre, preCount); preList = lfirst + lj + 1; } }
			};
			auto emit_pass = [&]() {
				uint16_t *wsel = (uint16_t *)(stage + wv * SK_CHUNK_G);
				static_assert(WSLOTS * 2 <= (int)SK_CHUNK_G * 16, "the selected slots' indices live in one staging quarter");
				uint32_t nsel = 0;
				unsigned long long usedMask[WSLOTS / 64];
				const unsigned long long below = (1ull << lane) - 1;
#pragma unroll
				for (int i = 0; i < WSLOTS / 64; i++) {
					const int s = wv * WSLOTS + i * 64 + lane;
					const uint32_t count = (uint32_t)tcnt[s];
					const bool used = count != 0;
					const unsigned long long um = __ballot(used);
					usedMask[i] = um;
					if (!itemMode) { uniqW += (uint32_t)__builtin_popcountll(um); singleW += (uint32_t)__builtin_popcountll(__ballot(count == 1)); }
					uint32_t cls = !used ? 0u : ((count == 1 && singC != 3u) ? singC : (count < weakMin ? 0u : 1u));
					if (SK_DBG(dbgFlags, 2)) cls = 0;
					const bool need = (itemMode || TRACK) ? used : cls != 0;
					const unsigned long long nm = __ballot(need);
					if (need) wsel[nsel + (uint32_t)__builtin_popcountll(nm & below)] = (uint16_t)s;
					nsel += (uint32_t)__builtin_popcountll(nm);
				}
				sk_wave_lds_order();
#pragma unroll 1
				for (uint32_t sb0 = 0; sb0 < nsel; sb0 += 64) {
					const bool used = sb0 + (uint32_t)lane < nsel;
					const int s = used ? (int)wsel[sb0 + lane] : wv * WSLOTS;
					const unsigned long long cf = used ? tcnt[s] : 0ull;
					const uint32_t count = (uint32_t)cf;
					uint32_t cls = !used ? 0u : ((count == 1 && singC != 3u) ? singC : (count < weakMin ? 0u : 1u));
					if (SK_DBG(dbgFlags, 2)) cls = 0;
					Key<W> key;
#pragma unroll
					for (int q = 0; q < W; q++) key.w[q] = used ? tkeys[(size_t)s * W + q] : 0ull;
					const unsigned long long fst = used ? tfirst[s] : NO_FIRST;
					const double wsum = UNI ? (double)count * (double)__uint_as_float(hot.uni_wbits) : (used ? twsum[s] : 0.0);
					if (TRACK && used) {
						auto behind = [&](unsigned long long ord) -> uint32_t {
							uint32_t lo = 0, hi = tv.n;
							while (lo < hi) { const uint32_t mid = (lo + hi) >> 1; if (tv.bounds[mid] <= ord) lo = mid + 1; else hi = mid; }
							return lo;
						};
						const uint32_t iu = behind(fst >> 24);
						atomicAdd(&trkU[iu], 1u);
						atomicAdd(&trkS[iu], 1u);
						const unsigned long long sec = tsecond[s];
						if (sec != NO_FIRST) atomicAdd(&trkS[behind(sec >> 24)], 0xffffffffu);
					}
					if (itemMode) {
						cls = 0;
						for (int turn = 0; turn < (W == 1 ? 1 : 64); turn++) {
							if (used && (W == 1 || lane == turn) && !(__hip_atomic_load(out.err, __ATOMIC_RELAXED, __HIP_MEMORY_SCOPE_AGENT) & ERR_TABLE_FULL)) {
								bool claimed;
								const uint64_t ms = table_find_or_insert<W>(lg.merge, key, part_hash<W>(key.w), claimed);
								if (claimed && atomicAdd(lg.merge_used, 1ull) > (5ull << lg.merge.log2cap) / 8) atomicOr(out.err, (uint32_t)ERR_TABLE_FULL);
								if (ms == ~0ull) atomicOr(out.err, (uint32_t)ERR_TABLE_FULL);
								else {
									Slot<W> *sl = &lg.merge.slots[ms];
									atomicAdd(&sl->cntfwd, cf);
									atomicAdd(&sl->wsum, wsum);
									atomicMin(&sl->first, fst);
									if constexpr (EXT) {
										ExtSlot *es = &lg.merge.ext[ms];
#pragma unroll
										for (int j = 0; j < 12; j++) { const uint32_t v = (ttally[(size_t)s * 6 + (j >> 1)] >> (16 * (j & 1))) & 0xffffu; if (v) atomicAdd(&es->tally[j], v); }
										es->pkt = tpkt[s];
									}
								}
							}
						}
					}
					const unsigned long long mw = __ballot(cls == 1), ms = __ballot(cls == 2);
					if (mw) {
						const uint32_t cnt = (uint32_t)__builtin_popcountll(mw);
						if (wpos + cnt > wend) {
							for (unsigned long long e = wpos + lane; e < wend && e < hot.wcap; e += 64) { if (PACKED) hot.wout[e * (W + 1) + W] = 0; else hot.wvals[e * vw] = 0; }
							unsigned long long g = 0;
							if (lane == 0) g = atomicAdd(hot.wcursor, SK_OSLAB);
							wpos = skc_slab_base<BLOCKS>(g);
							wend = wpos + SK_OSLAB;
							if (wend > hot.wcap) { if (lane == 0) atomicOr(out.err, (uint32_t)ERR_ENTRIES_FULL); outFull = true; wend = wpos; }
						}
						if (!outFull) {
							if (cls == 1) {
								const uint64_t pos = wpos + (uint32_t)__builtin_popcountll(mw & below);
								uint32_t fwdc = (uint32_t)(cf >> 32), cnt16 = count;
								if (hot.has_singletons && first_forward(fst)) fwdc -= 1;
								if (cnt16 >= SK_ORDERED_FROM) { atomicAdd(&s_sat[0], 1ull); atomicAdd(&s_sat[1], (unsigned long long)count); if (cnt16 > 65535u) { cnt16 = 65535u; if (fwdc > 65534u) fwdc = 65534u; } }
								if (fwdc > 65535u) fwdc = 65535u;
								const uint32_t wbits = __float_as_uint((float)(hot.has_singletons ? wsum + first_weight_shift(fst) : wsum));
								if constexpr (PACKED) {
									uint64_t ew[W + 1];
#pragma unroll
									for (int q = 0; q < W; q++) ew[q] = key.w[q];
									ew[W] = bb_pack_value(cnt16, wbits, fwdc);
									bb_store_entry<W>(hot.wout, pos, ew);
								} else {
#pragma unroll
									for (int q = 0; q < W; q++) hot.wout[pos * W + q] = key.w[q];
									uint32_t *v = hot.wvals + pos * vw;
									v[0] = cnt16; v[1] = wbits; v[2] = fwdc;
									if constexpr (EXT) {
#pragma unroll
										for (int j = 0; j < 12; j++) v[3 + j] = (ttally[(size_t)s * 6 + (j >> 1)] >> (16 * (j & 1))) & 0xffffu;
									}
								}
							}
							wpos += cnt; keptW += cnt;
						}
					}
					if constexpr (!PACKED) {
						const uint64_t bucket = cls == 1 ? key_hash<W>(key, f.kb) & (f.nb_weak - 1) : 0;
						bucket_count_add(out.weakCount, bucket, cls == 1 && !outFull);
					}
					if (ms) {
						const uint32_t cnt = (uint32_t)__builtin_popcountll(ms);
						if (spos + cnt > send) {
							for (unsigned long long e = spos + lane; e < send && e < out.scap; e += 64) out.sweight[e] = 0;
							unsigned long long g = 0;
							if (lane == 0) g = atomicAdd(out.scursor, SK_OSLAB);
							spos = skc_slab_base<BLOCKS>(g);
							send = spos + SK_OSLAB;
							if (send > out.scap) { if (lane == 0) atomicOr(out.err, (uint32_t)ERR_ENTRIES_FULL); outFull = true; send = spos; }
						}
						uint64_t bucket = 0;
						if (!outFull && cls == 2) {
							const uint64_t pos = spos + (uint32_t)__builtin_popcountll(ms & below);
							bucket = key_hash<W>(key, f.kb) & (f.nb_sing - 1);
#pragma unroll
							for (int q = 0; q < W; q++) out.skeys[pos * W + q] = key.w[q];
							const float wf = (float)wsum;
							out.sweight[pos] = (uint8_t)((unsigned char)(((double)wf * 254.0)) + 1);
							if constexpr (EXT) out.spkt[pos] = tpkt[s];
						}
						bucket_count_add(out.singCount, bucket, cls == 2 && !outFull);
						if (!outFull) { spos += cnt; keptS += cnt; }
					}
				}
				sk_wave_lds_order();
#pragma unroll
				for (int i = 0; i < WSLOTS / 64; i++) {
					const int s = wv * WSLOTS + i * 64 + lane;
					if ((usedMask[i] >> lane) & 1ull) {
						tkeys[(size_t)s * W] = EMPTY_KEY; if (W > 1) tkeys[(size_t)s * W + W - 1] = SK_KEY_PENDING; tcnt[s] = 0; if constexpr (WSUM) twsum[s] = 0.0; tfirst[s] = NO_FIRST; if constexpr (W > 1 && !LEAN) tstate[s] = 0; if (TRACK) tsecond[s] = NO_FIRST;
						if constexpr (EXT) {
#pragma unroll
							for (int q = 0; q < 6; q++) ttally[(size_t)s * 6 + q] = 0;
						}
					}
				}
			};
			auto clear_table = [&]() {
				for (int i = t; i < S; i += SKC_THREADS) { tkeys[(size_t)i * W] = EMPTY_KEY; if (W > 1) tkeys[(size_t)i * W + W - 1] = SK_KEY_PENDING; tcnt[i] = 0; if constexpr (WSUM) twsum[i] = 0.0; tfirst[i] = NO_FIRST; if constexpr (W > 1 && !LEAN) tstate[i] = 0; if (TRACK) tsecond[i] = NO_FIRST; }
				if (EXT) for (int i = t; i < 6 * S; i += SKC_THREADS) ttally[i] = 0;
			};

			insert_pass(0, 0, true);
			lds_barrier();
			const bool ovf = skc_uni<BLOCKS>(s_overflow[fl]) != 0 || skc_uni<BLOCKS>(s_claimed[fl]) > LIMIT;
			if (t == 0) { s_claimed[fl ^ 1u] = 0; s_overflow[fl ^ 1u] = 0; }
			if (!ovf) {
				emit_pass();
				lds_barrier();
				continue;
			}
			clear_table();
			if (t == 0) { s_sp = 2; s_stackBits[0] = 1; s_stackVal[0] = 0; s_stackBits[1] = 1; s_stackVal[1] = 1; }
			lds_barrier();
			while (skc_uni<BLOCKS>(s_sp) > 0) {
				const uint32_t bits = skc_uni<BLOCKS>(s_stackBits[s_sp - 1]), val = skc_uni<BLOCKS>(s_stackVal[s_sp - 1]);
				lds_barrier();
				if (t == 0) { s_sp--; s_claimed[fl] = 0; s_overflow[fl] = 0; }
				lds_barrier();
				insert_pass(bits, val, false);
				lds_barrier();
				if (skc_uni<BLOCKS>(s_overflow[fl]) || skc_uni<BLOCKS>(s_claimed[fl]) > LIMIT) {
					lds_barrier();
					clear_table();
					if (t == 0) {
						if (bits >= 20) atomicOr(out.err, (uint32_t)ERR_TABLE_FULL);
						else {
							s_stackBits[s_sp] = bits + 1; s_stackVal[s_sp] = val; s_sp++;
							s_stackBits[s_sp] = bits + 1; s_stackVal[s_sp] = val | (1u << bits); s_sp++;
						}
					}
					lds_barrier();
					continue;
				}
				emit_pass();
				lds_barrier();
			}
			if (t == 0) { s_claimed[0] = s_claimed[1] = 0; s_overflow[0] = s_overflow[1] = 0; }
			lds_barrier();
		}
	}
	for (unsigned long long e = wpos + lane; e < wend && e < hot.wcap; e += 64) { if (PACKED) hot.wout[e * (W + 1) + W] = 0; else hot.wvals[e * vw] = 0; }
	for (unsigned long long e = spos + lane; e < send && e < out.scap; e += 64) out.sweight[e] = 0;
	if (lane == 0) {
		if (uniqW) atomicAdd(&out.fc->unique, uniqW); if (singleW) atomicAdd(&out.fc->singletons, singleW);
		if (keptW) atomicAdd(&out.fc->weak_kept, keptW); if (keptS) atomicAdd(&out.fc->sing_kept, keptS);
	}
	if (t == 0 && s_sat[0]) { atomicAdd(&out.fc->saturated, s_sat[0]); atomicAdd(&out.fc->sat_sightings, s_sat[1]); }
	if (TRACK) {
		lds_barrier();
		for (uint32_t i = (uint32_t)t; i <= tv.n && i <= SK_TRACK_MAX; i += SKC_THREADS) { if (trkU[i]) atomicAdd(&tv.d_unique[i], trkU[i]); if (trkS[i]) atomicAdd(&tv.d_single[i], trkS[i]); }
	}
}


template <int W>
__global__ __launch_bounds__(256)
void sk_merge_emit_kernel(Table<W> tbl, CountOut out, FinalizeParams f) {
	const uint32_t vw = tbl.ext ? 15 : 3;
	const uint32_t singC = f.has_singletons ? (f.min_depth > 1 ? 0u : 2u) : 3u;
	const uint32_t weakMin = ((!f.has_singletons || f.min_depth > 2) && f.min_depth != 1) ? f.min_depth : 0u;
	const uint64_t cap = 1ull << tbl.log2cap;
	unsigned long long uniq = 0, single = 0, keptW = 0, keptS = 0;
	for (uint64_t i0 = (uint64_t)blockIdx.x * blockDim.x; i0 < cap; i0 += (uint64_t)gridDim.x * blockDim.x) {
		const uint64_t i = i0 + threadIdx.x;
		const bool used = i < cap && slot_used<W>(tbl.slots[i]);
		uint32_t cls = 0; uint64_t bucket = 0;
		if (used) {
			const Slot<W> sl = tbl.slots[i];
			const Key<W> key = slot_key<W>(sl);
			uint32_t cnt = (uint32_t)sl.cntfwd, fwdc = (uint32_t)(sl.cntfwd >> 32);
			uniq++; if (cnt == 1) single++;
			cls = (cnt == 1 && singC != 3u) ? singC : (cnt < weakMin ? 0u : 1u);
			if (cls == 1) {
				const unsigned long long pos = atomicAdd(out.wcursor, 1ull);
				if (pos >= out.wcap) { atomicOr(out.err, (uint32_t)ERR_ENTRIES_FULL); cls = 0; }
				else {
					if (out.weakCount) bucket = key_hash<W>(key, f.kb) & (f.nb_weak - 1);
					if (f.has_singletons && first_forward(sl.first)) fwdc -= 1;
					if (cnt >= SK_ORDERED_FROM) { atomicAdd(&out.fc->saturated, 1ull); atomicAdd(&out.fc->sat_sightings, (unsigned long long)cnt); if (cnt > 65535u) { cnt = 65535u; if (fwdc > 65534u) fwdc = 65534u; } }
					if (fwdc > 65535u) fwdc = 65535u;
					const uint32_t wbits = __float_as_uint((float)(f.has_singletons ? sl.wsum + first_weight_shift(sl.first) : sl.wsum));
					if (out.wentries) {
						uint64_t ew[W + 1];
#pragma unroll
						for (int q = 0; q < W; q++) ew[q] = key.w[q];
						ew[W] = bb_pack_value(cnt, wbits, fwdc);
						bb_store_entry<W>(out.wentries, pos, ew);
					} else {
#pragma unroll
						for (int q = 0; q < W; q++) out.wkeys[pos * W + q] = key.w[q];
						uint32_t *v = out.wvals + pos * vw;
						v[0] = cnt; v[1] = wbits; v[2] = fwdc;
						if (tbl.ext) for (int j = 0; j < 12; j++) v[3 + j] = tbl.ext[i].tally[j];
					}
					keptW++;
				}
			} else if (cls == 2) {
				const unsigned long long pos = atomicAdd(out.scursor, 1ull);
				if (pos >= out.scap) { atomicOr(out.err, (uint32_t)ERR_ENTRIES_FULL); cls = 0; }
				else {
					bucket = key_hash<W>(key, f.kb) & (f.nb_sing - 1);
#pragma unroll
					for (int q = 0; q < W; q++) out.skeys[pos * W + q] = key.w[q];
					const float wf = (float)sl.wsum;
					out.sweight[pos] = (uint8_t)((unsigned char)(((double)wf * 254.0)) + 1);
					if (tbl.ext && out.spkt) out.spkt[pos] = tbl.ext[i].pkt;
					keptS++;
				}
			}
		}
		if (out.weakCount) bucket_count_add(out.weakCount, bucket, cls == 1);
		bucket_count_add(out.singCount, bucket, cls == 2);
	}
	uniq = wave_sum(uniq); single = wave_sum(single); keptW = wave_sum(keptW); keptS = wave_sum(keptS);
	if ((threadIdx.x & 63) == 0) {
		if (uniq) atomicAdd(&out.fc->unique, uniq); if (single) atomicAdd(&out.fc->singletons, single);
		if (keptW) atomicAdd(&out.fc->weak_kept, keptW); if (keptS) atomicAdd(&out.fc->sing_kept, keptS);
	}
}
#ifndef KMR_INSTANCE_TU
__global__ void sk_long_items_kernel(const uint64_t *list_start, uint64_t n_lists, uint64_t threshold, uint64_t piece, uint64_t *item_c0, uint64_t *item_c1, uint64_t cap, unsigned long long *n_items, uint32_t *item_list = nullptr) {
	for (uint64_t l = blockIdx.x * (uint64_t)blockDim.x + threadIdx.x; l < n_lists; l += (uint64_t)gridDim.x * blockDim.x) {
		const uint64_t a = list_start[l], b = list_start[l + 1];
		if (b - a <= threshold) continue;
		const uint64_t n = (b - a + piece - 1) / piece;
// ... 434 lines not shown
```

Measured before the change: 65.17 billion.

## Add six-blocks-per-CU count kernel with 32-bit rebased first-ordinals in LDS

Adds a kernel that records the min and max read-ordinal span of each call into device stats. When that span fits in 31 bits and no foreign chunks were adopted, the uniform W=1 count pass can use a new BLOCKS=6 variant. This variant stores first-occurrence ordinals as 32-bit values rebased on ord_base, which shrinks the LDS table so six blocks fit per CU. It also drops prefetching of the next list in that variant and adds register-rematerialization helpers. The goal is higher occupancy in the count kernel, at the cost of extra host plumbing, a union reuse of ext_min_q, and the loss of the prefetch.

```diff
diff --git a/kmernator_amd/csrc/kmr_api.hip b/kmernator_amd/csrc/kmr_api.hip
--- a/kmernator_amd/csrc/kmr_api.hip
+++ b/kmernator_amd/csrc/kmr_api.hip
@@ -144,6 +144,7 @@
 #endif
 	h->stats.raw_kmers = s.raw + s.inserted + s.sender_bad; h->stats.raw_good_kmers = s.good + s.inserted; h->stats.discarded = s.raw - s.good + s.sender_bad;
 	h->occupied = s.claimed; h->pending_kmers = 0; h->subtracted = s.subtracted;
+	h->ord_seen = s.ord_nlo != 0; h->ord_lo = ~s.ord_nlo; h->ord_hi = s.ord_hi;
 	if (e & ERR_READ_TOO_LONG) return fail(h, KMR_ERR_UNSUPPORTED, "a read is longer than the per-wavefront LDS tile (" + std::to_string(TILE_SPAN) + " bases)");
 	if (e & ERR_TABLE_FULL) return fail(h, KMR_ERR_CAPACITY, "device k-mer table is full; raise kmr_config.max_table_entries / estimated_raw_kmers");
 	if (e & ERR_SEGMENT_OVERFLOW) return fail(h, KMR_ERR_CAPACITY, "an owner segment overflowed seg_capacity");
@@ -1357,6 +1358,10 @@
 	if (!filt && !h->ext && !sp_debug_extract(h)) { rc = sk_uniform_weight(h, rvAll, hints, lean, wK, n <= chunk ? &longest : nullptr, &have_longest); if (rc) return rc; }
 	if (hints.packed && (!lean || h->cfg.size_tracker)) return fail(h, KMR_ERR_STATE, "internal: a packed batch handed to an extraction that wants text");
 	if (n) sk_note_call_weight(h, lean, wK);
+	if (n) {
+		hipLaunchKernelGGL(sk_ord_span_kernel, dim3(1), dim3(64), 0, h->stream, rvAll.offsets, n, rvAll.stream_base, h->dstats.get<DevStats>());
+		HIPCHK(h, hipGetLastError());
+	}
 	if (!h->sk_state) { rc = sk_size_lists<W>(h, std::max<uint64_t>(total_bases, hints.call_bases), lean); if (rc) return rc; }
 	if (tracking) { h->trk_n = 0; rc = h->trk.reserve(h, "trk", n * sizeof(SkTrackRec)); if (rc) return rc; HIPCHK(h, hipMemsetAsync(h->trk.get<SkTrackRec>(), 0, n * sizeof(SkTrackRec), h->stream)); }
 	for (uint64_t r = 0; r < n; r += chunk) {
@@ -1514,22 +1519,30 @@
 	int blocks;
 };
 static const int SK_COUNT_BLOCKS_DEFAULT = 5;
-template <int W> int sk_count_blocks(kmr_handle *h, bool ext, bool tracking, bool uni, bool item) {
+static const bool SK_COUNT_SIX_DEFAULT = true;
+template <int W> int sk_count_blocks(kmr_handle *h, bool ext, bool tracking, bool uni, bool item, uint64_t n_lists) {
 	if (W != 1 || ext || tracking || !uni || item) return 4;
-	return h->tune.count_blocks ? h->tune.count_blocks : SK_COUNT_BLOCKS_DEFAULT;
-}
-template <int W, int LOG2S, bool TRACK, bool EXT, bool UNI, bool ITEM, int BLOCKS = 0> SkCountLaunch<W> sk_count_form() { return {sk_count_kernel<W, LOG2S, TRACK, EXT, UNI, ITEM, BLOCKS>, sk_count_smem_bytes<W, LOG2S, TRACK, EXT, UNI>(), BLOCKS ? BLOCKS : 4}; }
+	if (h->tune.count_blocks) return h->tune.count_blocks;
+	const bool ordinals = h->ord_seen && !h->ord_foreign && h->ord_hi >= h->ord_lo && h->ord_hi - h->ord_lo < (1ull << 31);
+	const bool fed = n_lists >= (uint64_t)num_cus(h) * 6 * SK_LBATCH;
+	if (ordinals && (h->tune.count_six == 1 || (h->tune.count_six == 0 && SK_COUNT_SIX_DEFAULT && fed))) return 6;
+	return SK_COUNT_BLOCKS_DEFAULT;
+}
+template <int W, int LOG2S, bool TRACK, bool EXT, bool UNI, bool ITEM, int BLOCKS = 0> SkCountLaunch<W> sk_count_form() { return {sk_count_kernel<W, LOG2S, TRACK, EXT, UNI, ITEM, BLOCKS>, sk_count_smem_bytes<W, LOG2S, TRACK, EXT, UNI, BLOCKS == 6>(), BLOCKS ? BLOCKS : 4}; }
 template <int W, bool ITEM> SkCountLaunch<W> sk_count_forms(bool ext, bool tracking, bool uni, int blocks) {
 	if constexpr (!ITEM) { if (tracking && !ext) return sk_count_form<W, COUNT_LOG2S, true, false, false, false>(); }
-	if constexpr (W == 1 && !ITEM) { if (blocks == 5) return sk_count_form<1, COUNT_LOG2S, false, false, true, false, 5>(); }
+	if constexpr (W == 1 && !ITEM) {
+		if (blocks == 5) return sk_count_form<1, COUNT_LOG2S, false, false, true, false, 5>();
+		if (blocks == 6) return sk_count_form<1, COUNT_LOG2S, false, false, true, false, 6>();
+	}
 	return ext ? sk_count_form<W, COUNT_LOG2S_EXT, false, true, false, ITEM>() :
 	    (uni ? sk_count_form<W, COUNT_LOG2S, false, false, true, ITEM>() : sk_count_form<W, COUNT_LOG2S, false, false, false, ITEM>());
 }
-template <int W> int sk_count_select(kmr_handle *h, bool ext, bool tracking, bool uni, bool item, const CountOut &out, const SkLong<W> &lg, SkCountLaunch<W> &k) {
+template <int W> int sk_count_select(kmr_handle *h, bool ext, bool tracking, bool uni, bool item, uint64_t n_lists, const CountOut &out, const SkLong<W> &lg, SkCountLaunch<W> &k) {
 	if (item && tracking) return fail(h, KMR_ERR_STATE, "internal: the size tracker's count pass has no long-list items");
 	if (item != (lg.item_c0 != nullptr) || (item && (!lg.item_c1 || !lg.merge.slots || !lg.merge_used))) return fail(h, KMR_ERR_STATE, "internal: count pass and its work items disagree");
 	if (ext ? (!out.wkeys || !out.wvals || !out.weakCount) : !out.wentries) return fail(h, KMR_ERR_STATE, "internal: count pass and its entry buffers disagree");
-	const int blocks = sk_count_blocks<W>(h, ext, tracking, uni, item);
+	const int blocks = sk_count_blocks<W>(h, ext, tracking, uni, item, n_lists);
 	k = item ? sk_count_forms<W, true>(ext, tracking, uni, blocks) : sk_count_forms<W, false>(ext, tracking, uni, blocks);
 	if (k.blocks != blocks) return fail(h, KMR_ERR_STATE, "internal: count pass and its blocks per CU disagree");
 	if (!item) h->last_count_blocks = k.blocks;
@@ -1542,7 +1555,9 @@
 	SkCountArgs<W> *d = nullptr;
 	int rc = arena_get(h, &d, 1); if (rc) return rc;
 	hipLaunchKernelGGL(sk_count_args_kernel<W>, dim3(1), dim3(64), 0, h->stream, a, d);
-	hipLaunchKernelGGL(k.kern, dim3(grid), dim3(SKC_THREADS), k.smem, h->stream, (const uint4 *)pool_view(h, h->l1).base, ls, lc, nl, h->k, sk_count_hot<W>(a), h->work_counter.get<unsigned int>(), sk_dbg_flags("KMR_SK_COUNT_DBG"), (const SkCountArgs<W> *)d);
+	SkCountHot hot = sk_count_hot<W>(a);
+	if (k.blocks == 6) hot.ord_base = (uint32_t)h->ord_lo;
+	hipLaunchKernelGGL(k.kern, dim3(grid), dim3(SKC_THREADS), k.smem, h->stream, (const uint4 *)pool_view(h, h->l1).base, ls, lc, nl, h->k, hot, h->work_counter.get<unsigned int>(), sk_dbg_flags("KMR_SK_COUNT_DBG"), (const SkCountArgs<W> *)d);
 	return 0;
 }
 
@@ -1659,7 +1674,7 @@
 		if (repeated) merge_log2 += 3;
 		int rc = 0;
 		SkCountLaunch<W> k;
-		rc = sk_count_select<W>(h, p.ext, p.tracking, p.uni, false, out, p.lgMain, k); if (rc) return rc;
+		rc = sk_count_select<W>(h, p.ext, p.tracking, p.uni, false, nl, out, p.lgMain, k); if (rc) return rc;
 		const int grid = (int)std::min<uint64_t>((uint64_t)num_cus(h) * k.blocks, (nl / p.lgMain.list_stride + SK_LBATCH) / SK_LBATCH);
 		if (p.tracking) HIPCHK(h, hipMemsetAsync(tv.d_unique, 0, 8 * (tv.n + 1), h->stream));
 		if (dbg()) { int nb = 0; hipOccupancyMaxActiveBlocksPerMultiprocessor(&nb, (const void *)k.kern, SKC_THREADS, k.smem); fprintf(stderr, "sk_count<W=%d>: %d blocks per CU (LDS %zu), %llu lists, %u chunks\n", W, nb, k.smem, (unsigned long long)nl, p.nch); }
@@ -1673,7 +1688,7 @@
 		lgItems.merge.slots = mslots.get<Slot<W>>(); lgItems.merge.ext = mext.get<ExtSlot>(); lgItems.merge.log2cap = merge_log2;
 		HIPCHK(h, hipMemsetAsync(lgItems.merge_used, 0, 8, h->stream));
 		rc = zero_work_counter(h); if (rc) return rc;
-		rc = sk_count_select<W>(h, p.ext, p.tracking, p.uni, true, out, lgItems, k); if (rc) return rc;
+		rc = sk_count_select<W>(h, p.ext, p.tracking, p.uni, true, n_items, out, lgItems, k); if (rc) return rc;
 		const int grid2 = (int)std::min<uint64_t>((uint64_t)num_cus(h) * k.blocks, n_items);
 		rc = sk_count_launch<W>(h, k, grid2, p.ls, p.lc, nl, out, p.f, tv, lgItems); if (rc) return rc;
 		hipLaunchKernelGGL(sk_merge_emit_kernel<W>, dim3(grid_for(1ull << merge_log2)), dim3(256), 0, h->stream, lgItems.merge, out, p.f);
@@ -1721,7 +1736,7 @@
 	rc = build_csr(h, h->l1, p.nl, 0, &p.ls, &p.lc, &p.nch, p.refined ? nullptr : &h->l1_head_seen); if (rc) return rc;
 	rc = sk_count_uniform<W>(h, p.tracking, p.uni, p.f.uni_wbits); if (rc) return rc;
 	h->last_count_uniform = p.uni;
-	rc = count_entry_buffers(h, p, G, sk_entry_slack(h, sk_count_blocks<W>(h, p.ext, p.tracking, p.uni, false)), G / (p.f.has_singletons ? 8 : 3), G / 3, h->sk_exchange && h->cfg.world_size > 1); if (rc) return rc;
+	rc = count_entry_buffers(h, p, G, sk_entry_slack(h, sk_count_blocks<W>(h, p.ext, p.tracking, p.uni, false, p.nl)), G / (p.f.has_singletons ? 8 : 3), G / 3, h->sk_exchange && h->cfg.world_size > 1); if (rc) return rc;
 	if (p.tracking) { rc = sk_track_view(h, p.tv); if (rc) return rc; }
 	p.lgMain = sk_own_lists<W>(h, p.refined);
 	bool device_error = false;
@@ -1771,7 +1786,7 @@
 	const uint64_t G = h->stats.raw_good_kmers;
 	bool uni = false;
 	if (!h->peer_uni_mixed) { rc = sk_count_uniform<W>(h, false, uni, f.uni_wbits); if (rc) return rc; }
-	uint64_t want = (uint64_t)((double)G * ((double)hi / (double)nl) / (f.has_singletons ? 6.0 : 2.5)) + sk_entry_slack(h, sk_count_blocks<W>(h, false, false, uni, false));
+	uint64_t want = (uint64_t)((double)G * ((double)hi / (double)nl) / (f.has_singletons ? 6.0 : 2.5)) + sk_entry_slack(h, sk_count_blocks<W>(h, false, false, uni, false, hi));
 	if (h->tune.early_entry_share >= 0) { want = (uint64_t)((double)G * h->tune.early_entry_share) + 16384; h->early.ue.reset(); }
 	rc = h->early.ue.reserve(h, "early count ue", 8ull * (W + 1) * want); if (rc) return rc;
 	rc = h->early.cursor.reserve(h, "early count cursor", 16); if (rc) return rc;
@@ -1793,7 +1808,7 @@
 	const uint64_t n_work = hi > lg.list_first ? (hi - lg.list_first + lg.list_stride - 1) / lg.list_stride : 0;
 	if (n_work) {
 		SkCountLaunch<W> k;
-		rc = sk_count_select<W>(h, false, false, uni, false, out, lg, k); if (rc) return rc;
+		rc = sk_count_select<W>(h, false, false, uni, false, hi, out, lg, k); if (rc) return rc;
 		const int grid = (int)std::min<uint64_t>((uint64_t)num_cus(h) * k.blocks, (n_work + SK_LBATCH) / SK_LBATCH);
 		TimeSpan t(h, KMR_TIME_COUNT);
 		rc = sk_count_launch<W>(h, k, grid, ls, lc, hi, out, f, tv, lg);
@@ -1954,7 +1969,7 @@
 	HIPCHK(h, hipMemsetAsync(h->dstats.get<DevStats>(), 0, sizeof(DevStats), h->stream));
 	HIPCHK(h, hipMemsetAsync(h->derr.get<uint32_t>(), 0, 4, h->stream));
 	memset(&h->stats, 0, sizeof(h->stats));
-	h->occupied = h->pending_kmers = 0; h->stream_base = 0; h->reads = 0; h->subtracted = 0; h->xc_job_bases = 0; h->xc_bytes_to_peers = 0;
+	h->occupied = h->pending_kmers = 0; h->stream_base = 0; h->reads = 0; h->ord_lo = h->ord_hi = 0; h->ord_seen = h->ord_foreign = false; h->subtracted = 0; h->xc_job_bases = 0; h->xc_bytes_to_peers = 0;
 	h->trk_n = 0; h->trk_elems.clear();
 	h->trk_next = 128; h->trk_raw = h->trk_good = 0; h->trk_bounds.clear(); h->trk_snap_raw.clear(); h->trk_snap_good.clear();
 	h->finalized = false; h->map_gen++; h->has_singletons = h->cfg.separate_singletons != 0;
@@ -1995,6 +2010,7 @@
 	else if (k == "lean_extract") h->tune.no_lean_extract = value == 0;
 	else if (k == "uniform_count") h->tune.no_uniform_count = value == 0;
 	else if (k == "count_blocks") { if (value != 0 && value != 4 && value != 5) return fail(h, KMR_ERR_INVALID_ARG, "count_blocks is 0 (default), 4 or 5"); h->tune.count_blocks = (int)value; }
+	else if (k == "count_six") { if (value != 0 && value != 1 && value != 2) return fail(h, KMR_ERR_INVALID_ARG, "count_six is 0 (default), 1 (wherever the ordinals allow) or 2 (never)"); h->tune.count_six = (int)value; }
 	else if (k == "packed_direct") h->tune.no_packed_direct = value == 0;
 	else if (k == "pow2_lists") h->tune.pow2_lists = value != 0;
 	else if (k == "list_aim") h->tune.list_aim = value >= 1 ? (uint64_t)value : 0;
@@ -3004,6 +3020,7 @@
 	if (n_chunks == 0) return KMR_OK;
 	hipSetDevice(h->device);
 	rc = sk_ensure_state(h); if (rc) return rc;
+	h->ord_foreign = true;
 	const int grid = (int)std::min<uint64_t>((n_chunks + SK_ADOPT_WAVES * SK_ADOPT_GROUP - 1) / (SK_ADOPT_WAVES * SK_ADOPT_GROUP), (uint64_t)num_cus(h) * 8);
 	rc = pool_reserve(h, h->l1, n_chunks + n_granules / SK_CHUNK_G + (sk_list_count(h->sk_bits) / h->cfg.world_size) + (uint64_t)grid * SK_ADOPT_WAVES * 130 + 64, true); if (rc) return rc;
 	const size_t need = 8 * (n_chunks + 1) + 4 * (n_chunks + 1) + 256;
diff --git a/kmernator_amd/csrc/kmr_host.hpp b/kmernator_amd/csrc/kmr_host.hpp
--- a/kmernator_amd/csrc/kmr_host.hpp
+++ b/kmernator_amd/csrc/kmr_host.hpp
@@ -154,6 +154,7 @@
 	bool pow2_lists = false;
 	bool no_packed_direct = false;
 	bool no_uniform_count = false;
+	int count_six = 0;
 	int count_blocks = 0;
 	bool no_lean_extract = false;
 	bool exchange_fail_once = false;
@@ -196,6 +197,7 @@
 	uint64_t occupied = 0;
 	uint64_t pending_kmers = 0;
 	uint64_t stream_base = 0, reads = 0;
+	uint64_t ord_lo = 0, ord_hi = 0; bool ord_seen = false, ord_foreign = false;
 	uint64_t nb_weak = 0, nb_sing = 0;
 	bool finalized = false, has_singletons = true;
 	kmr_handle *subtract = nullptr;
diff --git a/kmernator_amd/csrc/kmr_instances.hpp b/kmernator_amd/csrc/kmr_instances.hpp
--- a/kmernator_amd/csrc/kmr_instances.hpp
+++ b/kmernator_amd/csrc/kmr_instances.hpp
@@ -28,6 +28,7 @@
 #define KMR_SKCB(W, TRACK, EXT, UNI, ITEM, BLOCKS) KMR_T __global__ void sk_count_kernel<W, EXT ? COUNT_LOG2S_EXT : COUNT_LOG2S, TRACK, EXT, UNI, ITEM, BLOCKS>(const uint4 *, const uint64_t *, const uint64_t *, uint64_t, uint32_t, SkCountHot, unsigned int *, uint32_t, const SkCountArgs<W> *);
 #define KMR_SKCI(W, TRACK, EXT, UNI, ITEM) KMR_SKCB(W, TRACK, EXT, UNI, ITEM, 0)
 #define KMR_SKC5 KMR_SKCB(1, false, false, true, false, 5)
+#define KMR_SKC6 KMR_SKCB(1, false, false, true, false, 6)
 #define KMR_SKCX(W, TRACK, EXT) KMR_SKCI(W, TRACK, EXT, false, false)
 #define KMR_SKL(W) KMR_T __global__ void sk_lookup_kernel<W>(PoolView, const uint64_t *, const uint64_t *, uint64_t, uint32_t, const uint64_t *, const uint64_t *, const uint32_t *, uint32_t *, uint64_t, unsigned int *, const uint64_t *, const uint64_t *, const uint32_t *, uint64_t, uint64_t);
 #define KMR_SKCU(W) KMR_SKCI(W, false, false, true, false)
@@ -55,7 +56,7 @@
 #if defined(KMR_INSTANCES_EXTERN)
 KMR_SKX_W(1) KMR_SKX_W(2) KMR_SKX_W(3) KMR_SKX_W(4)
 KMR_SKX_W32(2) KMR_SKX_W32(3) KMR_SKX_W32(4)
-KMR_SKC_W(1) KMR_SKC_W(2) KMR_SKC_W(3) KMR_SKC_W(4) KMR_SKC5
+KMR_SKC_W(1) KMR_SKC_W(2) KMR_SKC_W(3) KMR_SKC_W(4) KMR_SKC5 KMR_SKC6
 KMR_EX_W(1) KMR_EX_W(2) KMR_EX_W(3) KMR_EX_W(4)
 KMR_PART_W(1) KMR_PART_W(2) KMR_PART_W(3) KMR_PART_W(4)
 KMR_CK(1, true, COUNT_LOG2S, true)
@@ -69,7 +70,7 @@
 #ifdef KMR_INST_SKC
 KMR_SKC_W(KMR_INST_W)
 #if KMR_INST_W == 1
-KMR_SKC5
+KMR_SKC5 KMR_SKC6
 #endif
 #endif
 #ifdef KMR_INST_EX
diff --git a/kmernator_amd/csrc/kmr_kernels.hpp b/kmernator_amd/csrc/kmr_kernels.hpp
--- a/kmernator_amd/csrc/kmr_kernels.hpp
+++ b/kmernator_amd/csrc/kmr_kernels.hpp
@@ -49,6 +49,7 @@
 	unsigned long long inserted;
 	unsigned long long subtracted;
 	unsigned long long sender_bad;
+	unsigned long long ord_nlo, ord_hi;
 };
 
 struct DevParams {
diff --git a/kmernator_amd/csrc/kmr_superkmer.hpp b/kmernator_amd/csrc/kmr_superkmer.hpp
--- a/kmernator_amd/csrc/kmr_superkmer.hpp
+++ b/kmernator_amd/csrc/kmr_superkmer.hpp
@@ -1,6 +1,7 @@
 #ifndef KMR_SUPERKMER_HPP_
 #define KMR_SUPERKMER_HPP_
 
+#include <type_traits>
 #include "kmr_partition.hpp"
 #include "kmr_buckets.hpp"
 
@@ -107,6 +108,14 @@
 #ifndef KMR_INSTANCE_TU
 __global__ void sk_state_init_kernel(unsigned long long *state, uint64_t n) {
 	for (uint64_t i = blockIdx.x * (uint64_t)blockDim.x + threadIdx.x; i < n; i += (uint64_t)gridDim.x * blockDim.x) state[i] = ((unsigned long long)NO_CHUNK << 32) | SK_CHUNK_G;
+}
+#endif
+#ifndef KMR_INSTANCE_TU
+__global__ void sk_ord_span_kernel(const uint64_t *offsets, uint64_t n_reads, uint64_t stream_base, DevStats *st) {
+	if (blockIdx.x == 0 && threadIdx.x == 0 && offsets[n_reads] > offsets[0]) {
+		atomicMax(&st->ord_nlo, ~(unsigned long long)(stream_base + offsets[0]));
+		atomicMax(&st->ord_hi, (unsigned long long)(stream_base + offsets[n_reads] - 1));
+	}
 }
 #endif
 #ifndef KMR_INSTANCE_TU
@@ -1264,16 +1273,17 @@
 struct SkCountHot {
 	uint64_t *wout;
 	uint32_t *wvals; unsigned long long *wcursor; uint64_t wcap;
-	uint32_t min_depth, has_singletons, uni_wbits, ext_min_q;
+	uint32_t min_depth, has_singletons, uni_wbits;
+	union { uint32_t ext_min_q; uint32_t ord_base; };
 };
 template <int W> struct SkCountArgs { CountOut out; FinalizeParams f; SkTrackView tv; SkLong<W> lg; };
 template <int W> __host__ inline SkCountHot sk_count_hot(const SkCountArgs<W> &a) {
-	return {a.out.wentries ? a.out.wentries : a.out.wkeys, a.out.wvals, a.out.wcursor, a.out.wcap, a.f.min_depth, a.f.has_singletons, a.f.uni_wbits, a.f.ext_min_q};
+	return {a.out.wentries ? a.out.wentries : a.out.wkeys, a.out.wvals, a.out.wcursor, a.out.wcap, a.f.min_depth, a.f.has_singletons, a.f.uni_wbits, {a.f.ext_min_q}};
 }
 template <int W> __global__ void sk_count_args_kernel(SkCountArgs<W> a, SkCountArgs<W> *dst) { if (threadIdx.x == 0 && blockIdx.x == 0) *dst = a; }
 
-template <int W, int LOG2S, bool TRACK = false, bool EXT = false, bool UNI = false>
-__host__ __device__ constexpr size_t sk_count_smem_bytes() { return (size_t)(1 << LOG2S) * (8 * W + 24 + (W > 1 ? 4 : 0) - (UNI ? 8 : 0) - (UNI && W > 1 ? 4 : 0) + (TRACK ? 8 : 0) + (EXT ? 28 : 0)) + (size_t)SK_STAGE_G * 16 + 256 + 64 + (TRACK ? 8 * (SK_TRACK_MAX + 1) : 0); }
+template <int W, int LOG2S, bool TRACK = false, bool EXT = false, bool UNI = false, bool FIRST32 = false>
+__host__ __device__ constexpr size_t sk_count_smem_bytes() { return (size_t)(1 << LOG2S) * (8 * W + 24 + (W > 1 ? 4 : 0) - (UNI ? 8 : 0) - (UNI && W > 1 ? 4 : 0) + (TRACK ? 8 : 0) + (EXT ? 28 : 0) - (FIRST32 ? 4 : 0)) + (size_t)SK_STAGE_G * 16 + 256 + 64 + (TRACK ? 8 * (SK_TRACK_MAX + 1) : 0); }
 static const uint64_t SK_EXT_LONG_CHUNKS = 128;
 static const int SK_EXT_BLOCKS = 3;
 __device__ __forceinline__ uint32_t sk_ext_char(uint32_t code) { return (uint32_t)((0x584e54474341ull >> (8 * code)) & 0xffu); }
@@ -1286,11 +1296,17 @@
 static const uint32_t SK_ORDERED_FROM = 256;
 static const unsigned long long SK_OSLAB = 2048;
 
-template <int BLOCKS> __device__ __forceinline__ uint32_t skc_uni(uint32_t x) { if constexpr (BLOCKS == 5) return (uint32_t)__builtin_amdgcn_readfirstlane((int)x); else return x; }
-template <int BLOCKS> __device__ __forceinline__ unsigned long long skc_uni64(unsigned long long x) { if constexpr (BLOCKS == 5) return ((unsigned long long)skc_uni<5>((uint32_t)(x >> 32)) << 32) | skc_uni<5>((uint32_t)x); else return x; }
+template <int BLOCKS> __device__ __forceinline__ uint32_t skc_uni(uint32_t x) { if constexpr (BLOCKS >= 5) return (uint32_t)__builtin_amdgcn_readfirstlane((int)x); else return x; }
+template <int BLOCKS> __device__ __forceinline__ unsigned long long skc_uni64(unsigned long long x) { if constexpr (BLOCKS >= 5) return ((unsigned long long)skc_uni<5>((uint32_t)(x >> 32)) << 32) | skc_uni<5>((uint32_t)x); else return x; }
 template <int BLOCKS> __device__ __forceinline__ unsigned long long skc_slab_base(unsigned long long g) {
-	if constexpr (BLOCKS == 5) return skc_uni64<5>(g);
+	if constexpr (BLOCKS >= 5) return skc_uni64<5>(g);
 	else return ((unsigned long long)(uint32_t)__shfl((int)(g >> 32), 0, 64) << 32) | (uint32_t)__shfl((int)(uint32_t)g, 0, 64);
+}
+template <bool F32> __device__ __forceinline__ void skc_first_clear(unsigned long long *tfirst, int s) { if constexpr (F32) ((uint32_t *)tfirst)[s] = ~0u; else tfirst[s] = NO_FIRST; }
+template <typename ORD> __device__ __forceinline__ void skc_first_min32(unsigned long long *tfirst, uint32_t s, ORD ord, bool fwd) { atomicMin(&((uint32_t *)tfirst)[s], ((uint32_t)ord << 1) | (fwd ? 1u : 0u)); }
+template <int BLOCKS> __device__ __forceinline__ int skc_afresh(int x) { if constexpr (BLOCKS == 6) asm volatile("" : "+v"(x)); return x; }
+__device__ __forceinline__ unsigned long long skc_first_word32(const unsigned long long *tfirst, int s, uint32_t uniFirst) {
+	return ((unsigned long long)(((const uint32_t *)tfirst)[s] & 1u) << 23) | (unsigned long long)uniFirst;
 }
 template <int W, int LOG2S, bool TRACK, bool EXT, bool UNI, bool ITEM>
 __host__ __device__ constexpr int sk_count_default_blocks() { return EXT ? (W == 1 ? (LOG2S <= 9 ? SK_EXT_BLOCKS : 2) : 1) : ((W == 1 && LOG2S <= 10 && !TRACK) ? 4 : (W == 2 && LOG2S <= 10 && !TRACK ? (UNI ? 4 : 3) : 1)); }
@@ -1300,7 +1316,10 @@
                      SkCountHot hot, unsigned int *work_counter, uint32_t dbgFlags, const SkCountArgs<W> *__restrict__ args) {
 	const CountOut &out = args->out; const FinalizeParams &f = args->f; const SkTrackView &tv = args->tv; const SkLong<W> &lg = args->lg;
 	static_assert(!UNI || (!TRACK && !EXT), "the one-weight count pass is the plain one's");
-	static_assert(BLOCKS == 0 || (BLOCKS == 5 && W == 1 && UNI && !ITEM), "only the one-weight, one-word pass over lists has a five-block instance");
+	static_assert(BLOCKS == 0 || ((BLOCKS == 5 || BLOCKS == 6) && W == 1 && UNI && !ITEM), "only the one-weight, one-word pass over lists has a five- and a six-block instance");
+	constexpr bool F32 = BLOCKS == 6;
+	constexpr bool XPRE = BLOCKS != 6;
+	using Ord = std::conditional_t<F32, uint32_t, uint64_t>;
 	constexpr int S = 1 << LOG2S;
 	constexpr bool LEAN = UNI && W > 1;
 	constexpr bool WSUM = !UNI;
@@ -1316,7 +1335,7 @@
 	unsigned long long *tcnt = (unsigned long long *)(tkeys + (size_t)S * W);
 	double *twsum = (double *)(tcnt + S);
 	unsigned long long *tfirst = (unsigned long long *)(twsum + (WSUM ? S : 0));
-	uint32_t *tstate = (uint32_t *)(tfirst + S);
+	uint32_t *tstate = F32 ? (uint32_t *)tfirst + S : (uint32_t *)(tfirst + S);
 	uint32_t *ttally = tstate + (W > 1 && !LEAN ? S : 0);
 	uint32_t *tpkt = ttally + (EXT ? 6 * S : 0);
 	uint4 *stage = (uint4 *)(tpkt + (EXT ? S : 0));
@@ -1337,7 +1356,7 @@
 	unsigned long long wpos = 0, wend = 0, spos = 0, send = 0;
 	bool outFull = false;
 	if (t == 0) { s_claimed[0] = s_claimed[1] = 0; s_overflow[0] = s_overflow[1] = 0; s_sp = 0; s_sat[0] = s_sat[1] = 0; }
-	for (int i = t; i < S; i += SKC_THREADS) { tkeys[(size_t)i * W] = EMPTY_KEY; if (W > 1) tkeys[(size_t)i * W + W - 1] = SK_KEY_PENDING; tcnt[i] = 0; if constexpr (WSUM) twsum[i] = 0.0; tfirst[i] = NO_FIRST; if constexpr (W > 1 && !LEAN) tstate[i] = 0; if (TRACK) tsecond[i] = NO_FIRST; }
+	for (int i = skc_afresh<BLOCKS>(t); i < S; i += SKC_THREADS) { tkeys[(size_t)i * W] = EMPTY_KEY; if (W > 1) tkeys[(size_t)i * W + W - 1] = SK_KEY_PENDING; tcnt[i] = 0; if constexpr (WSUM) twsum[i] = 0.0; skc_first_clear<F32>(tfirst, i); if constexpr (W > 1 && !LEAN) tstate[i] = 0; if (TRACK) tsecond[i] = NO_FIRST; }
 	if (EXT) for (int i = t; i < 6 * S; i += SKC_THREADS) ttally[i] = 0;
 	lds_barrier();
 	const uint32_t singC = hot.has_singletons ? (hot.min_depth > 1 ? 0u : 2u) : 3u;
@@ -1357,20 +1376,21 @@
 		if (lfirst >= n_work) break;
 		const uint32_t nl = (uint32_t)(n_work - lfirst < (uint64_t)grab ? n_work - lfirst : (uint64_t)grab);
 		if ((uint32_t)t < nl) {
+			const int tb = skc_afresh<BLOCKS>(t);
 			uint64_t a, b;
-			if (itemMode) { a = lg.item_c0[lfirst + t]; b = lg.item_c1[lfirst + t]; }
-			else { const uint64_t l = lg.list_first + (lfirst + t) * stride; a = list_start[l]; b = list_start[l + 1]; if (lg.long_threshold && b - a > lg.long_threshold) b = a; }
-			s_c0[t] = a; s_c1[t] = b;
+			if (itemMode) { a = lg.item_c0[lfirst + tb]; b = lg.item_c1[lfirst + tb]; }
+			else { const uint64_t l = lg.list_first + (lfirst + tb) * stride; a = list_start[l]; b = list_start[l + 1]; if (lg.long_threshold && b - a > lg.long_threshold) b = a; }
+			s_c0[tb] = a; s_c1[tb] = b;
 		}
 		lds_barrier();
 		const uint64_t dbase = skc_uni64<BLOCKS>(itemMode ? s_c0[0] : list_start[lg.list_first + lfirst * stride]), dend = skc_uni64<BLOCKS>(itemMode ? s_c1[0] : list_start[lg.list_first + (lfirst + nl - 1) * stride + 1]);
 		const uint64_t dcached = dend - dbase < (uint64_t)SK_DESC_CAP ? dend - dbase : (uint64_t)SK_DESC_CAP;
-		for (uint64_t i = (uint64_t)t; i < dcached; i += SKC_THREADS) { const uint64_t d = list_chunks[dbase + i]; s_dchunk[i] = (uint32_t)d; s_dcount[i] = (uint8_t)(d >> 32); }
+		for (uint64_t i = (uint64_t)skc_afresh<BLOCKS>(t); i < dcached; i += SKC_THREADS) { const uint64_t d = list_chunks[dbase + i]; s_dchunk[i] = (uint32_t)d; s_dcount[i] = (uint8_t)(d >> 32); }
 		lds_barrier();
 		auto describe = [&](uint64_t ci, uint32_t &chunk, uint32_t &count) {
 			if (ci - dbase < dcached) { chunk = s_dchunk[ci - dbase]; count = s_dcount[ci - dbase]; }
 			else { const uint64_t d = list_chunks[ci]; chunk = (uint32_t)d; count = (uint32_t)(d >> 32); }
-			if constexpr (BLOCKS == 5) { chunk = skc_uni<BLOCKS>(chunk); count = skc_uni<BLOCKS>(count); }
+			if constexpr (BLOCKS >= 5) { chunk = skc_uni<BLOCKS>(chunk); count = skc_uni<BLOCKS>(count); }
 		};
 		auto fetch = [&](uint64_t ci, uint4 &v, uint32_t &count) {
 			uint32_t chunk;
@@ -1392,7 +1412,7 @@
 				uint4 cur = make_uint4(0, 0, 0, 0); uint32_t curCount = 0;
 				if (firstPass && preList == lfirst + lj) { cur = pre; curCount = preCount; }
 				else if (c0 + wv < c1) fetch(c0 + wv, cur, curCount);
-				bool wantPre = firstPass;
+				bool wantPre = firstPass && XPRE;
 				if (firstPass) preList = ~0ull;
 				for (uint64_t ci = c0 + wv; ci < c1 && !skc_uni<BLOCKS>(s_overflow[fl]) && skc_uni<BLOCKS>(s_claimed[fl]) <= LIMIT; ci += SKC_WAVES) {
 					wstage[lane] = cur;
@@ -1412,12 +1432,13 @@
 					}
 					if (wantNxt && (uint32_t)lane < nxtCount) nxt = poolg[(size_t)nxtChunk * SK_CHUNK_G + lane];
 					if (havePre) { pre = make_uint4(0, 0, 0, 0); if ((uint32_t)lane < preCount) pre = poolg[(size_t)preChunk * SK_CHUNK_G + lane]; }
-					uint32_t n = 0; const uint32_t *ww = nullptr; bool uniformW = true; uint64_t ord0 = 0;
+					uint32_t n = 0; const uint32_t *ww = nullptr; bool uniformW = true; Ord ord0 = 0;
 					const uint8_t *xq = nullptr;
 					uint32_t leftCarry = 0;
 					auto enter_record = [&]() {
 						const SkRec rec = sk_enter_record(wstage, rs, hx, hy, k);
-						n = rec.n; ww = rec.weights; uniformW = rec.uniform; ord0 = rec.ord0;
+						n = rec.n; ww = rec.weights; uniformW = rec.uniform;
+						if constexpr (F32) ord0 = (uint32_t)rec.ord0 - hot.ord_base; else ord0 = rec.ord0;
 						if (EXT) xq = (const uint8_t *)(ww + (uniformW ? 0u : 4u * ((n + 3) / 4)));
 					};
 					constexpr int NWD = 2 * W + 2;
@@ -1430,7 +1451,7 @@
 						for (int i = 0; i < NWD; i++) win[i] = bw[i];
 						sb = 2u * (j & 15u);
 					};
-					struct KState { Key<W> key; bool fwd, mine; uint32_t slot, step, w; uint64_t ord; uint32_t x; };
+					struct KState { Key<W> key; bool fwd, mine; uint32_t slot, step, w; Ord ord; uint32_t x; };
 					KState kA, kB;
 #pragma unroll
 					for (int wi = 0; wi < W; wi++) { kA.key.w[wi] = 0; kB.key.w[wi] = 0; }
@@ -1578,12 +1599,15 @@
 								else {
 									atomicAdd(&tcnt[s], 1ull | ((unsigned long long)(cur.fwd ? 1 : 0) << 32));
 									if constexpr (!UNI) atomicAdd(&twsum[s], (double)wa);
-									const unsigned long long fp = UNI ? (((unsigned long long)cur.ord << FIRST_ORD_SHIFT) | ((unsigned long long)(cur.fwd ? 1u : 0u) << 23) | (unsigned long long)uniFirst) : first_pack(cur.ord, cur.fwd, wa);
-									if (TRACK) {
-										const unsigned long long was = atomicMin(&tfirst[s], fp);
-										const unsigned long long cand = was > fp ? was : fp;
-										if (cand != NO_FIRST) atomicMin(&tsecond[s], cand);
-									} else atomicMin(&tfirst[s], fp);
+									if constexpr (F32) skc_first_min32(tfirst, s, cur.ord, cur.fwd);
+									else {
+										const unsigned long long fp = UNI ? (((unsigned long long)cur.ord << FIRST_ORD_SHIFT) | ((unsigned long long)(cur.fwd ? 1u : 0u) << 23) | (unsigned long long)uniFirst) : first_pack(cur.ord, cur.fwd, wa);
+										if (TRACK) {
+											const unsigned long long was = atomicMin(&tfirst[s], fp);
+											const unsigned long long cand = was > fp ? was : fp;
+											if (cand != NO_FIRST) atomicMin(&tsecond[s], cand);
+										} else atomicMin(&tfirst[s], fp);
+									}
 									if constexpr (EXT) {
 										const uint32_t lc = cur.x & 0xffu, rc = (cur.x >> 8) & 0xffu, lq = (cur.x >> 16) & 0xffu, rq = cur.x >> 24;
 										if (lq >= hot.ext_min_q || lc > 3u) atomicAdd(&ttally[(size_t)s * 6 + (lc >> 1)], 1u << (16 * (lc & 1u)));
@@ -1636,7 +1660,8 @@
 					Key<W> key;
 #pragma unroll
 					for (int q = 0; q < W; q++) key.w[q] = used ? tkeys[(size_t)s * W + q] : 0ull;
-					const unsigned long long fst = used ? tfirst[s] : NO_FIRST;
+					unsigned long long fst = NO_FIRST;
+					if constexpr (F32) { if (used) fst = skc_first_word32(tfirst, s, uniFirst); } else fst = used ? tfirst[s] : NO_FIRST;
 					const double wsum = UNI ? (double)count * (double)__uint_as_float(hot.uni_wbits) : (used ? twsum[s] : 0.0);
 					if (TRACK && used) {
 						auto behind = [&](unsigned long long ord) -> uint32_t {
@@ -1745,7 +1770,7 @@
 				for (int i = 0; i < WSLOTS / 64; i++) {
 					const int s = wv * WSLOTS + i * 64 + lane;
 					if ((usedMask[i] >> lane) & 1ull) {
-						tkeys[(size_t)s * W] = EMPTY_KEY; if (W > 1) tkeys[(size_t)s * W + W - 1] = SK_KEY_PENDING; tcnt[s] = 0; if constexpr (WSUM) twsum[s] = 0.0; tfirst[s] = NO_FIRST; if constexpr (W > 1 && !LEAN) tstate[s] = 0; if (TRACK) tsecond[s] = NO_FIRST;
+						tkeys[(size_t)s * W] = EMPTY_KEY; if (W > 1) tkeys[(size_t)s * W + W - 1] = SK_KEY_PENDING; tcnt[s] = 0; if constexpr (WSUM) twsum[s] = 0.0; skc_first_clear<F32>(tfirst, s); if constexpr (W > 1 && !LEAN) tstate[s] = 0; if (TRACK) tsecond[s] = NO_FIRST;
 						if constexpr (EXT) {
 #pragma unroll
 							for (int q = 0; q < 6; q++) ttally[(size_t)s * 6 + q] = 0;
@@ -1754,7 +1779,7 @@
 				}
 			};
 			auto clear_table = [&]() {
-				for (int i = t; i < S; i += SKC_THREADS) { tkeys[(size_t)i * W] = EMPTY_KEY; if (W > 1) tkeys[(size_t)i * W + W - 1] = SK_KEY_PENDING; tcnt[i] = 0; if constexpr (WSUM) twsum[i] = 0.0; tfirst[i] = NO_FIRST; if constexpr (W > 1 && !LEAN) tstate[i] = 0; if (TRACK) tsecond[i] = NO_FIRST; }
+				for (int i = skc_afresh<BLOCKS>(t); i < S; i += SKC_THREADS) { tkeys[(size_t)i * W] = EMPTY_KEY; if (W > 1) tkeys[(size_t)i * W + W - 1] = SK_KEY_PENDING; tcnt[i] = 0; if constexpr (WSUM) twsum[i] = 0.0; skc_first_clear<F32>(tfirst, i); if constexpr (W > 1 && !LEAN) tstate[i] = 0; if (TRACK) tsecond[i] = NO_FIRST; }
 				if (EXT) for (int i = t; i < 6 * S; i += SKC_THREADS) ttally[i] = 0;
 			};
 
@@ -1797,8 +1822,9 @@
 			lds_barrier();
 		}
 	}
-	for (unsigned long long e = wpos + lane; e < wend && e < hot.wcap; e += 64) { if (PACKED) hot.wout[e * (W + 1) + W] = 0; else hot.wvals[e * vw] = 0; }
-	for (unsigned long long e = spos + lane; e < send && e < out.scap; e += 64) out.sweight[e] = 0;
+	const int laneT = skc_afresh<BLOCKS>(lane);
+	for (unsigned long long e = wpos + laneT; e < wend && e < hot.wcap; e += 64) { if (PACKED) hot.wout[e * (W + 1) + W] = 0; else hot.wvals[e * vw] = 0; }
+	for (unsigned long long e = spos + laneT; e < send && e < out.scap; e += 64) out.sweight[e] = 0;
 	if (lane == 0) {
 		if (uniqW) atomicAdd(&out.fc->unique, uniqW); if (singleW) atomicAdd(&out.fc->singletons, singleW);
 		if (keptW) atomicAdd(&out.fc->weak_kept, keptW); if (keptS) atomicAdd(&out.fc->sing_kept, keptS);
```

After: 68.26 billion (median of 6 runs). 1.05x the previous value.
